# NVIDIA-RTX/RTXPT

Measured on AMD Instinct MI355X. Metric: Mrays/s at 4K 4spp 8-bounce bistro-like (extend + shadow rays / wall time of pt_render), higher is better.
Workload: dtype f32; 1 GPU; C3 bistro-like street canyon, 2808008 triangles, 64 materials, 32 textures 1024^2, 7368 emissive-triangle + env-quad lights, 3840x2160, 4 spp, 8 bounces, NEE 5 candidates + RR, lp types binary16 (reference default), environment cube 2048 BC6H (reference default on D3D12); BVH builder=PLOC + parallel re-insertion + cost-driven wide nodes, built on device, buildMs 77.8 (host part 0.0), 275780 wide n; parallelism=pixel-tile shard x1 + 1 gather, gather=none (1 GPU), transport=none, rehearsal=False

## Files before the change

### rtxpt_amd/csrc/pt_api.hip

```cpp
#include <cstring>
#include <rocprim/rocprim.hpp>
#include "pt_context.h"
#ifdef MI355PT_TEST_HOOKS
#include "../../include/mi355pt_testhooks.h"
#endif
#include "pt_denoiser.h"
#include <dlfcn.h>
#include <algorithm>
#include <cmath>
#include <cstdio>
#include <chrono>

using namespace ptk;

static_assert(sizeof(::PTMaterialData) == sizeof(ptk::PTMaterialData), "material ABI");
static_assert(sizeof(::PathTracerCameraData) == sizeof(ptk::PathTracerCameraData), "camera ABI");
static_assert(sizeof(::PtSettings) == sizeof(ptk::PtSettings), "settings ABI");
static_assert(sizeof(::PtGeometryDesc) == sizeof(ptk::GeometryDesc), "geometry ABI");
static_assert(sizeof(::PtInstanceDesc) == sizeof(ptk::InstanceDesc), "instance ABI");
static_assert(sizeof(::PolymorphicLightInfo) == sizeof(ptk::PolymorphicLightInfo), "light ABI");

namespace {

void build_mips(HostTexture& t) {
// ... 354 lines not shown
    return PT_OK;
}
int bake_env_cube(pt_context* c) {
    ptk::EnvCube& e = c->envCube; memset(&e, 0, sizeof(e)); e.dim = c->envCubeDim; e.mipLevels = ptk::env_cube_mip_levels(e.dim);
    size_t total = 0; for (uint l = 0; l < e.mipLevels; l++) { e.mipOffset[l] = (uint)total; total += 6ull * (e.dim >> l) * (e.dim >> l); }
    PT_CHECK_HIP(c, c->dEnvCube.resize(total));
    std::vector<ptk::EnvDirectionalLight> dirLights = c->envDirLights;
    if (!c->sceneDirLights.empty()) {
        PtEnvMapSceneParams prm; memset(&prm, 0, sizeof(prm)); memcpy(prm.Transform, c->envToWorld.m, 48); prm.Enabled = 1.f;
        std::vector<ptk::EnvDirectionalLight> conv(c->sceneDirLights.size());
        if (pt_env_bake_lights(reinterpret_cast<const PtEnvDirectionalLight*>(c->sceneDirLights.data()), (uint32_t)conv.size(), &prm, e.dim, reinterpret_cast<PtEnvDirectionalLight*>(conv.data())) != PT_OK) return fail(c, PT_ERROR_INVALID_ARGUMENT, "scene directional lights");
        for (auto& l : conv) if (dirLights.size() < 16u) dirLights.push_back(l);
    }
    PT_CHECK_HIP(c, c->dEnvDirLights.upload(dirLights, c->stream));
    if (c->skyEnabled) {
        ptk::ProceduralSkyContext h = c->sky; h.Transmittance.texels = c->dSkyTex[0].p; h.Scatter.texels = c->dSkyTex[1].p; h.Irradiance.texels = c->dSkyTex[2].p; h.Clouds.texels = c->dSkyTex[3].p;
        PT_CHECK_HIP(c, c->dSky.resize(1)); PT_CHECK_HIP(c, hipMemcpyAsync(c->dSky.p, &h, sizeof(h), hipMemcpyHostToDevice, c->stream)); PT_CHECK_HIP(c, hipStreamSynchronize(c->stream));
        PT_CHECK_HIP(c, c->dSkyLowRes.resize(6ull * (e.dim / 2u) * (e.dim / 2u)));
    }
    refresh_scene_view(c);
    launch_env_cube_bake(c->dsc, c->dEnvDirLights.p, (uint)dirLights.size(), c->dEnvCube.p, c->dsc.envCube, c->stream);
    if (c->envCompression) {
        PT_CHECK_HIP(c, c->dEnvCubeSource.resize(total));
        PT_CHECK_HIP(c, hipMemcpyAsync(c->dEnvCubeSource.p, c->dEnvCube.p, sizeof(ptk::uint2) * total, hipMemcpyDeviceToDevice, c->stream));
        launch_env_cube_compress(c->dEnvCube.p, c->dsc.envCube, c->envCompression, c->stream);
    } else c->dEnvCubeSource.free();
    refresh_scene_view(c);
    PT_CHECK_HIP(c, hipGetLastError());
    c->envCubeDirty = false; c->lightsDirty = true;
    return PT_OK;
}
}

int prepare(pt_context* c) {
    if (c->texDirty) { int r = upload_textures(c); if (r != PT_OK) return r; refresh_scene_view(c); c->lightsDirty = true; c->envCubeDirty = true; }
    if (c->envEnabled && c->envCubeDirty) { int r = bake_env_cube(c); if (r != PT_OK) return r; }
    if (c->geomDirty) { int r = finalize_geometry(c); if (r != PT_OK) return r; }
    if (c->lightsDirty) { int r = bake_lights(c); if (r != PT_OK) return r; }
    else if (c->weightsDirty && !c->lights.empty()) {
        launch_light_weights(c->dLights.p, c->dLightsEx.p, (uint)c->lights.size(), c->dLightW.p, c->lightBoost, c->stream);
        int r = build_light_proxies(c, c->dLightW.p, nullptr, 0u, 0.f); if (r != PT_OK) return r;
        refresh_scene_view(c);
    }
    c->weightsDirty = false;
    return PT_OK;
}

int neeat_exchange_feedback(pt_context* c) {
    pt_context::NeeAt& st = c->neeat;
    if (c->shardCount == 1 || !c->comm || !st.feedbackFilled || st.W != c->width || st.H != c->height) return PT_OK;
    hipStream_t s = c->stream;
    if (st.xW != c->width || st.xH != c->height) {
        std::vector<uint> others; for (uint r = 0; r < c->shardCount; r++) if (r != c->shardRank) others.insert(others.end(), c->shardPixels[r].begin(), c->shardPixels[r].end());
        PT_CHECK_HIP(c, st.xPixels.upload(others, s)); PT_CHECK_HIP(c, st.xRecv.resize(3 * others.size())); PT_CHECK_HIP(c, st.xSend.resize(3 * c->owned.size())); PT_CHECK_HIP(c, hipStreamSynchronize(s));
        st.xW = c->width; st.xH = c->height;
    }
    const size_t n = c->owned.size();
    launch_pack_feedback(st.fbW.p, st.fbC.p, st.depth.p, c->dOwned.p, (uint)n, c->width, st.xSend.p, s);
    PT_CHECK_NCCL(c, g_rccl.GroupStart());
    size_t off = 0; ncclResult_t bad = ncclSuccess;
    for (uint r = 0; r < c->shardCount && bad == ncclSuccess; r++) {
        if (r == c->shardRank) continue;
        const size_t m = c->shardPixels[r].size();
        if (n) bad = g_rccl.Send(st.xSend.p, 3 * n, ncclFloat, (int)r, c->comm, s);
        if (m && bad == ncclSuccess) bad = g_rccl.Recv(st.xRecv.p + 3 * off, 3 * m, ncclFloat, (int)r, c->comm, s);
        off += m;
    }
    ncclResult_t ge = g_rccl.GroupEnd();
    if (bad != ncclSuccess || ge != ncclSuccess) return fail(c, PT_ERROR_HIP, std::string("NEE-AT feedback exchange: ") + g_rccl.GetErrorString(bad != ncclSuccess ? bad : ge));
    launch_unpack_feedback(st.fbW.p, st.fbC.p, st.depth.p, st.xPixels.p, (uint)off, c->width, st.xRecv.p, s);
    return PT_OK;
}
int neeat_frame(pt_context* c, int phases, const float* depth, const ptk::uint2* motion) {
    pt_context::NeeAt& st = c->neeat;
    const uint N = (uint)c->lights.size();
    if (!N || !c->numProxies) {
        c->localResX = c->localResY = c->localJitterX = c->localJitterY = c->localMaxLight = 0; c->localRatio = 0.f; c->feedbackRequired = false; st.feedbackFilled = st.lastFeedbackAvailable = false; st.frameOpen = false;
        refresh_scene_view(c); return PT_OK;
    }
    NeeAtFrame F; memset(&F, 0, sizeof(F));
    F.W = c->width; F.H = c->height; F.BW = (F.W + 1) / 2; F.BH = (F.H + 1) / 2; F.tilesX = (F.W + 7) / 8 + 1; F.tilesY = (F.H + 7) / 8 + 1;
    const size_t px = (size_t)F.W * F.H, bpx = (size_t)F.BW * F.BH, tiles = (size_t)F.tilesX * F.tilesY;
    if (phases & NEEAT_BEGIN) {
        if (st.historicTotalLightCount && st.historicTotalLightCount != N) st.feedbackFilled = st.lastFeedbackAvailable = false;
        if (st.W != F.W || st.H != F.H) {
            st.W = F.W; st.H = F.H; st.feedbackFilled = false; st.lastFeedbackAvailable = false;
            PT_CHECK_HIP(c, st.fbW.resize(px)); PT_CHECK_HIP(c, st.fbC.resize(px)); PT_CHECK_HIP(c, st.scW.resize(px)); PT_CHECK_HIP(c, st.scC.resize(px)); PT_CHECK_HIP(c, st.snapW.resize(px)); PT_CHECK_HIP(c, st.snapC.resize(px));
            PT_CHECK_HIP(c, st.blW.resize(bpx)); PT_CHECK_HIP(c, st.blC.resize(bpx)); PT_CHECK_HIP(c, st.local.resize(tiles * RTXPT_LIGHTING_LOCAL_PROXY_COUNT));
            PT_CHECK_HIP(c, hipMemsetAsync(st.fbW.p, 0, 4 * px, c->stream)); PT_CHECK_HIP(c, hipMemsetAsync(st.fbC.p, 0xFF, 4 * px, c->stream));
            PT_CHECK_HIP(c, st.depth.resize(px)); PT_CHECK_HIP(c, st.histDepth.resize(px));
            PT_CHECK_HIP(c, hipMemsetAsync(st.depth.p, 0, 4 * px, c->stream)); PT_CHECK_HIP(c, hipMemsetAsync(st.histDepth.p, 0, 4 * px, c->stream));
        }
        st.prevJitter[0] = st.jitter[0]; st.prevJitter[1] = st.jitter[1];
        neeat_advance_jitter(st.updateCounter, st.jitterF, st.jitter);
        st.updateCounter++;
        st.frameLocalAvailable = st.lastFeedbackAvailable; st.frameFeedbackAvailable = st.feedbackFilled;
        st.framePrevLightCount = st.historicTotalLightCount; st.historicTotalLightCount = N;
        st.frameOpen = true;
    }
    if (!st.frameOpen || st.W != F.W || st.H != F.H) return fail(c, PT_ERROR_NOT_READY, "NEE-AT: UpdateEnd without UpdateBegin of this frame size");
    const bool lastFrameLocalSamplesAvailable = st.frameLocalAvailable, lastFrameFeedbackAvailable = st.frameFeedbackAvailable;
    F.jitterX = st.jitter[0]; F.jitterY = st.jitter[1]; F.jitterPrevX = st.prevJitter[0]; F.jitterPrevY = st.prevJitter[1];
    F.updateCounter = st.updateCounter; F.dropoff = st.dropoff; F.totalLightCount = N; F.historicTotalLightCount = st.framePrevLightCount;
    F.lastFrameFeedbackAvailable = lastFrameFeedbackAvailable ? 1u : 0u; F.lastFrameLocalSamplesAvailable = (lastFrameLocalSamplesAvailable && lastFrameFeedbackAvailable) ? 1u : 0u;
    F.fbW = st.fbW.p; F.fbC = st.fbC.p; F.scW = st.scW.p; F.scC = st.scC.p; F.blW = st.blW.p; F.blC = st.blC.p; F.local = st.local.p;
    F.depth = depth ? depth : st.depth.p; F.motion = motion; F.historyDepth = st.histDepth.p; F.depthDisocclusionThreshold = 1.5f;
    const uint totalMaxFeedbackCount = lastFrameFeedbackAvailable ? ((F.W + 7) / 8) * ((F.H + 7) / 8) * 64u : 0u;
    if (phases & NEEAT_BEGIN) {
        PT_CHECK_HIP(c, st.counters.resize(N + 1)); PT_CHECK_HIP(c, hipMemsetAsync(st.counters.p, 0, 4 * (size_t)(N + 1), c->stream)); F.perLightCounters = st.counters.p;
        if (lastFrameFeedbackAvailable) launch_neeat_begin(F, st.snapW.p, st.snapC.p, st.preFilter, totalMaxFeedbackCount, c->stream);
        PT_CHECK_HIP(c, st.curW.resize(N + 1)); PT_CHECK_HIP(c, st.histW.resize(N));
        launch_neeat_boost_weights(c->dLightW.p, (lastFrameFeedbackAvailable && st.intensityDeltaMul > 0) ? st.histW.p : nullptr, st.nHist, N, st.intensityDeltaMul, st.curW.p, c->stream);
        int r = build_light_proxies(c, st.curW.p, lastFrameFeedbackAvailable ? st.counters.p : nullptr, totalMaxFeedbackCount, lastFrameFeedbackAvailable ? st.globalFeedbackWeight : 0.f); if (r != PT_OK) return r;
        PT_CHECK_HIP(c, hipMemcpyAsync(st.histW.p, st.curW.p, 4 * (size_t)N, hipMemcpyDeviceToDevice, c->stream)); st.nHist = N;
        st.lastFeedbackAvailable = lastFrameFeedbackAvailable;
    }
    if (!(phases & NEEAT_END)) { PT_CHECK_HIP(c, hipStreamSynchronize(c->stream)); return PT_OK; }
    F.perLightCounters = st.counters.p;
    F.samplingProxyCount = c->numProxies; F.proxies = c->dProxyIndices.p;
    launch_neeat_end(F, c->stream);
    if (!depth) PT_CHECK_HIP(c, hipMemsetAsync(st.depth.p, 0, 4 * px, c->stream));
    st.exportDepth = depth == nullptr;
    st.feedbackFilled = true; st.frameOpen = false;
    c->localResX = F.tilesX; c->localResY = F.tilesY; c->localJitterX = st.jitter[0]; c->localJitterY = st.jitter[1]; c->localMaxLight = 0;
    c->localRatio = lastFrameFeedbackAvailable ? st.localRatio : 0.f; c->sscThreshold = st.sscThreshold; c->feedbackRequired = true;
    refresh_scene_view(c);
    PT_CHECK_HIP(c, hipStreamSynchronize(c->stream));
    return PT_OK;
}

extern "C" {

int32_t pt_create(const PtDeviceDesc* desc, pt_context** out) {
    if (!out) return PT_ERROR_INVALID_ARGUMENT;
    *out = nullptr;
    int ndev = 0;
    if (hipGetDeviceCount(&ndev) != hipSuccess || ndev <= 0) return PT_ERROR_NO_DEVICE;
    int dev = desc ? desc->deviceOrdinal : 0;
    if (dev < 0 || dev >= ndev) return PT_ERROR_INVALID_ARGUMENT;
    if (hipSetDevice(dev) != hipSuccess) return PT_ERROR_HIP;
    pt_context* c = new pt_context();
    c->device = dev; c->shardRank = desc ? desc->shardRank : 0; c->shardCount = (desc && desc->shardCount) ? desc->shardCount : 1;
    if (c->shardRank >= c->shardCount) { delete c; return PT_ERROR_INVALID_ARGUMENT; }
    if (hipStreamCreateWithFlags(&c->stream, hipStreamNonBlocking) != hipSuccess) { delete c; return PT_ERROR_HIP; }
    c->streams[0] = c->stream;
    for (uint b = 1; b < PT_PIPELINE_BATCHES; b++) if (hipStreamCreateWithFlags(&c->streams[b], hipStreamNonBlocking) != hipSuccess) { delete c; return PT_ERROR_HIP; }
    if (hipHostMalloc(&c->hostCounters, PT_PIPELINE_BATCHES * sizeof(WaveCounters), hipHostMallocDefault) != hipSuccess) { delete c; return PT_ERROR_HIP; }
    c->serialKernels = desc && (desc->flags & PT_DEVICE_SERIAL_KERNELS);
    c->bvhBuilder = (desc && (desc->flags & PT_DEVICE_PREFER_FAST_BUILD)) ? BVH_BUILDER_PLOC : ((desc && (desc->flags & PT_DEVICE_HOST_SAH_BUILDER)) ? BVH_BUILDER_SAH : BVH_BUILDER_PLOC_OPT);
    { const char* e = getenv("MI355PT_BVH_BUILDER");
      if (e && !strcmp(e, "karras")) c->bvhBuilder = BVH_BUILDER_KARRAS; else if (e && !strcmp(e, "ploc")) c->bvhBuilder = BVH_BUILDER_PLOC; else if (e && !strcmp(e, "sah")) c->bvhBuilder = BVH_BUILDER_SAH; else if (e && (!strcmp(e, "ploc_opt") || !strcmp(e, "device"))) c->bvhBuilder = BVH_BUILDER_PLOC_OPT; }
    { const char* e = getenv("MI355PT_TAIL_PATHS"); if (e) c->tailBelow = (uint)strtoul(e, nullptr, 10); }
    { const char* e = getenv("MI355PT_COMPACT_POOL"); if (e) c->compactPool = atoi(e) != 0; }
    { const char* e = getenv("MI355PT_FUSED_TRAVERSAL"); if (e) c->fusedTraversal = (uint)strtoul(e, nullptr, 10); }
    { const char* e = getenv("MI355PT_TAIL_DEFER"); if (e) c->tailDefer = (uint)strtoul(e, nullptr, 10); }
    memset(&c->dsc, 0, sizeof(c->dsc)); memset(&c->cam, 0, sizeof(c->cam)); memset(&c->bvh, 0, sizeof(c->bvh));
    pt_default_settings(reinterpret_cast<::PtSettings*>(&c->S));
    const float I[12] = {1, 0, 0, 0, 0, 1, 0, 0, 0, 0, 1, 0}; memcpy(c->envToWorld.m, I, 48); memcpy(c->envToLocal.m, I, 48); c->envColorMul = ptk::make_float3(1.0f / ptk::kEnvMapRadianceScale);
    if (c->dCounters.resize(PT_PIPELINE_BATCHES) != hipSuccess) { delete c; return PT_ERROR_HIP; }
    *out = c;
    return PT_OK;
}
int32_t pt_destroy(pt_context* c) {
    if (!c) return PT_ERROR_INVALID_ARGUMENT;
    (void)hipSetDevice(c->device); (void)hipStreamSynchronize(c->stream);
    if (c->comm && g_rccl.lib) { (void)g_rccl.CommDestroy(c->comm); c->comm = nullptr; }
    c->dSpHeader.free(); c->dSpThroughput.free(); c->dSpPlanes.free(); c->dSpRadiance.free(); c->dSpMotion.free(); c->dSpDepth.free(); c->dSpHitT.free(); c->dSpMark.free(); c->dSpNewL.free(); c->dSpScratch.free(); c->dSpGatherSend.free(); c->dSpGatherRecv.free(); c->dSpGatherPixels.free();
    c->dDnRRDiff.free(); c->dDnRRSpec.free(); c->dDnRRSpecMV.free(); c->dDnRRNormal.free(); c->dDnMotion.free(); c->dDnViewZ.free(); c->dDnRoughness.free(); c->dDnNormal.free(); c->dDnDiff.free(); c->dDnSpec.free(); c->dDnDisocclusion.free(); c->dDnHistoryClamp.free();
    relax_free(c); taa_free(c); bloom_free(c); taau_free(c);
    c->neeat.free(); c->dLocalTable.free(); c->dFbWeight.free(); c->dFbCand.free(); c->dSq3.free();
    c->dGatherSend.free(); c->dGatherRecv.free(); c->dGatherPixels.free(); c->dLightW.free(); c->dProxyOffsets.free(); if (c->dScanTemp) (void)hipFree(c->dScanTemp);
    if (c->bvhAllocated) bvh_free(c->bvh);
    c->dIndices.free(); c->dNormals.free(); c->dTangents.free(); c->dProxyCounters.free(); c->dProxyIndices.free(); c->dEnvLookup.free(); c->dOwned.free(); c->dQueue[0].free(); c->dQueue[1].free();
    c->dPrevPositions.free(); c->dPrevInstances.free(); c->dEmissiveList.free(); c->dEmissiveOffsets.free(); c->dPositions.free(); c->dUvs.free(); c->dGeometries.free(); c->dInstances.free(); c->dSubInstances.free(); c->dSubInstToInstGeom.free();
    c->dPrimInfo.free(); c->dShadeTris.free(); c->dAlphaPlanes.free(); c->dAlphaPool.free(); c->dMaterials.free(); c->dTexInfos.free(); c->dTexels.free(); c->dEnvCube.free(); c->dEnvCubeSource.free(); c->dEnvImageCube.free(); c->dEnvDirLights.free(); c->dLights.free(); c->dLightsEx.free(); c->dS0.free(); c->dS1.free(); c->dS2.free(); c->dS3.free(); c->dS4.free();
    c->dHit.free(); c->dS0b.free(); c->dS1b.free(); c->dS3b.free(); c->dS4b.free(); c->dHitb.free(); c->dSq0.free(); c->dSq1.free(); c->dSq2.free(); c->dAccum.free(); c->dScratch4.free(); c->dCounters.free(); c->dTravSpill.free(); c->dTaskQ.free(); c->dTravCounts.free(); c->dResolveList.free(); c->dBestKey.free(); c->dResolveListSh.free(); c->dBestKeySh.free(); c->dTaskQSh.free();
    for (uint b = 1; b < PT_PIPELINE_BATCHES; b++) (void)hipStreamDestroy(c->streams[b]);
    (void)hipStreamDestroy(c->stream); (void)hipHostFree(c->hostCounters);
    delete c;
    return PT_OK;
}
const char* pt_get_last_error(pt_context* c) { return c ? c->lastError.c_str() : "null context"; }

int32_t pt_set_geometry(pt_context* c, const PtGeometryBuffers* b, const PtGeometryDesc* geoms, uint32_t nGeoms, const PtMeshDesc* meshes, uint32_t nMeshes) {
    if (!c || !b || !geoms || !meshes) return fail(c, PT_ERROR_INVALID_ARGUMENT, "null argument");
    if (!b->indices || !b->positions) return fail(c, PT_ERROR_INVALID_ARGUMENT, "indices and positions are required");
    for (uint32_t g = 0; g < nGeoms; g++) {
        if ((size_t)geoms[g].indexOffset + geoms[g].numIndices > b->numIndices || (size_t)geoms[g].vertexOffset + geoms[g].numVertices > b->numVertices || geoms[g].numIndices % 3)
            return fail(c, PT_ERROR_INVALID_ARGUMENT, "geometry range outside the supplied streams");
        if ((geoms[g].flags & PT_GEOM_HAS_UV) && !b->uvs) return fail(c, PT_ERROR_INVALID_ARGUMENT, "geometry has uv flag but no uv stream");
        if ((geoms[g].flags & PT_GEOM_HAS_NORMAL) && !b->normals) return fail(c, PT_ERROR_INVALID_ARGUMENT, "geometry has normal flag but no normal stream");
        if ((geoms[g].flags & PT_GEOM_HAS_TANGENT) && !b->tangents) return fail(c, PT_ERROR_INVALID_ARGUMENT, "geometry has tangent flag but no tangent stream");
        const uint32_t* idx = b->indices + geoms[g].indexOffset;
        for (uint32_t k = 0; k < geoms[g].numIndices; k++) if (idx[k] >= geoms[g].numVertices) return fail(c, PT_ERROR_INVALID_ARGUMENT, "index outside the geometry's vertex range");
    }
    for (uint32_t m = 0; m < nMeshes; m++)
        if ((size_t)meshes[m].firstGeometry + meshes[m].numGeometries > nGeoms) return fail(c, PT_ERROR_INVALID_ARGUMENT, "mesh references geometries outside the supplied array");
    uint nv = b->numVertices;
    c->indices.assign(b->indices, b->indices + b->numIndices);
    c->positions.assign(b->positions, b->positions + 3 * (size_t)nv);
    c->uvs.assign(nv, ptk::make_float2(0, 0)); if (b->uvs) memcpy(c->uvs.data(), b->uvs, 8 * (size_t)nv);
    c->normals.assign(nv, 0); if (b->normals) memcpy(c->normals.data(), b->normals, 4 * (size_t)nv);
    c->tangents.assign(nv, 0); if (b->tangents) memcpy(c->tangents.data(), b->tangents, 4 * (size_t)nv);
    c->geometries.resize(nGeoms); memcpy(c->geometries.data(), geoms, sizeof(GeometryDesc) * nGeoms);
    c->meshes.resize(nMeshes); memcpy(c->meshes.data(), meshes, sizeof(MeshDesc) * nMeshes);
    c->geomDirty = true;
    relax_drop_history(c); taa_drop_history(c); taau_drop_history(c);
    return PT_OK;
}
int32_t pt_set_instances(pt_context* c, const PtInstanceDesc* inst, uint32_t n) {
    if (!c || (!inst && n)) return fail(c, PT_ERROR_INVALID_ARGUMENT, "null argument");
    c->instances.resize(n); if (n) memcpy(c->instances.data(), inst, sizeof(InstanceDesc) * n);
    c->geomDirty = true;
    return PT_OK;
}
int32_t pt_set_materials(pt_context* c, const ::PTMaterialData* mats, uint32_t nMats, const PtTextureDesc* tex, uint32_t nTex) {
    if (!c || (!mats && nMats) || (!tex && nTex)) return fail(c, PT_ERROR_INVALID_ARGUMENT, "null argument");
    c->materials.resize(nMats); if (nMats) memcpy(c->materials.data(), mats, 128 * (size_t)nMats);
    c->textures.clear();
    for (uint32_t i = 0; i < nTex; i++) {
        const PtTextureDesc& d = tex[i];
        if (!d.pixels || !d.width || !d.height || d.format > 2) return fail(c, PT_ERROR_INVALID_ARGUMENT, "bad texture descriptor");
        if (d.width > 32768u || d.height > 32768u) return fail(c, PT_ERROR_UNSUPPORTED, "textures above 32768 texels per side are not supported (16 mip levels)");
        HostTexture t; t.w = d.width; t.h = d.height; t.mips.resize(1); t.mips[0].resize((size_t)d.width * d.height);
        for (size_t k = 0; k < (size_t)d.width * d.height; k++) {
            ptk::float4 v;
            if (d.format == PT_TEX_RGBA32F) { const float* p = (const float*)d.pixels + 4 * k; v = ptk::make_float4(p[0], p[1], p[2], p[3]); }
            else {
                const uint8_t* p = (const uint8_t*)d.pixels + 4 * k;
                v = ptk::make_float4((float)p[0] / 255.0f, (float)p[1] / 255.0f, (float)p[2] / 255.0f, (float)p[3] / 255.0f);
                if (d.format == PT_TEX_RGBA8_SRGB) { v.x = srgb_to_linear(v.x); v.y = srgb_to_linear(v.y); v.z = srgb_to_linear(v.z); }
            }
            t.mips[0][k] = v;
        }
        build_mips(t);
        c->textures.push_back(std::move(t));
    }
    for (uint32_t m = 0; m < nMats; m++) {
        const ptk::PTMaterialData& mm = c->materials[m];
        auto chk = [&](uint flag, uint word) { return !(mm.Flags & flag) || (word & 0xFFFFu) < nTex; };
        if (!chk(PTMaterialFlags_UseBaseOrDiffuseTexture, mm.BaseOrDiffuseTextureIndex) || !chk(PTMaterialFlags_UseEmissiveTexture, mm.EmissiveTextureIndex) ||
            !chk(PTMaterialFlags_UseNormalTexture, mm.NormalTextureIndex) || !chk(PTMaterialFlags_UseMetalRoughOrSpecularTexture, mm.MetalRoughOrSpecularTextureIndex) ||
            !chk(PTMaterialFlags_UseTransmissionTexture, mm.TransmissionTextureIndex))
            return fail(c, PT_ERROR_INVALID_ARGUMENT, "material references a missing texture");
    }
    c->texDirty = true; c->geomDirty = true;
    return PT_OK;
}
static void set_env_params(pt_context* c, const PtEnvMapSceneParams* params) {
    if (params) {
        memcpy(c->envToWorld.m, params->Transform, 48);
        memset(&c->envToLocal, 0, sizeof(float3x4));
        for (int r = 0; r < 3; r++) for (int k = 0; k < 3; k++) c->envToLocal.m[r * 4 + k] = c->envToWorld.m[k * 4 + r];
        c->envColorMul = ptk::make_float3(params->ColorMultiplier[0], params->ColorMultiplier[1], params->ColorMultiplier[2]);
    } else {
        const float I[12] = {1, 0, 0, 0, 0, 1, 0, 0, 0, 0, 1, 0}; memcpy(c->envToWorld.m, I, 48); memcpy(c->envToLocal.m, I, 48);
        c->envColorMul = ptk::make_float3(1.0f / ptk::kEnvMapRadianceScale);
    }
}
static bool env_has_image(const pt_context* c) { return c->envTex.w != 0u || c->envImageCubeDim != 0u; }
int32_t pt_set_environment(pt_context* c, const float* rgb, uint32_t w, uint32_t h, const PtEnvMapSceneParams* params) {
    if (!c) return PT_ERROR_INVALID_ARGUMENT;
    c->envImageCubeDim = 0; c->dEnvImageCube.free();
    c->envEnabled = (w != 0 && h != 0 && rgb && (!params || params->Enabled != 0.f));
    if (!c->envEnabled) { c->envTex.w = c->envTex.h = 0; c->envTex.mips.clear(); if (c->skyEnabled && (!params || params->Enabled != 0.f)) c->envEnabled = true; }
    else {
        HostTexture& t = c->envTex; t.w = w; t.h = h; t.mips.clear(); t.mips.resize(1); t.mips[0].resize((size_t)w * h);
        for (size_t i = 0; i < (size_t)w * h; i++) t.mips[0][i] = ptk::make_float4(rgb[3 * i], rgb[3 * i + 1], rgb[3 * i + 2], 1.f);
        t.mipLevels = 1;
    }
    set_env_params(c, params);
    c->texDirty = true; c->lightsDirty = true; c->envCubeDirty = true;
    return PT_OK;
}
int32_t pt_set_environment_cube(pt_context* c, const float* rgbaFaces, uint32_t dim, const PtEnvMapSceneParams* params) {
    if (!c) return PT_ERROR_INVALID_ARGUMENT;
    if (dim > 16384u) return fail(c, PT_ERROR_INVALID_ARGUMENT, "cube-map source: at most 16384 texels per side");
    c->envTex.w = c->envTex.h = 0; c->envTex.mips.clear();
    c->envEnabled = (dim != 0 && rgbaFaces && (!params || params->Enabled != 0.f));
    if (!c->envEnabled) { c->envImageCubeDim = 0; c->dEnvImageCube.free(); if (c->skyEnabled && (!params || params->Enabled != 0.f)) c->envEnabled = true; }
    else {
        const size_t n = 6ull * dim * dim; std::vector<ptk::uint2> h(n);
        for (size_t i = 0; i < n; i++) h[i] = ptk::env_pack_rgba16f(ptk::make_float4(rgbaFaces[4 * i], rgbaFaces[4 * i + 1], rgbaFaces[4 * i + 2], rgbaFaces[4 * i + 3]));
        PT_CHECK_HIP(c, c->dEnvImageCube.resize(n)); PT_CHECK_HIP(c, hipMemcpy(c->dEnvImageCube.p, h.data(), n * sizeof(ptk::uint2), hipMemcpyHostToDevice));
        c->envImageCubeDim = dim;
    }
    set_env_params(c, params);
    c->texDirty = true; c->lightsDirty = true; c->envCubeDirty = true;
    return PT_OK;
}
int32_t pt_set_procedural_sky(pt_context* c, const PtProceduralSkyConstants* consts, const PtProceduralSkyTextures* tex) {
    if (!c) return PT_ERROR_INVALID_ARGUMENT;
    static_assert(sizeof(PtProceduralSkyConstants) == sizeof(ptk::ProceduralSkyConstants), "ProceduralSkyConstants layout");
    if (!consts) {
        if (c->skyEnabled) { c->skyEnabled = false; if (!env_has_image(c)) c->envEnabled = false; c->envCubeDirty = true; c->lightsDirty = true; c->texDirty = true; }
        return PT_OK;
    }
    if (tex) {
        const PtSkyTexture* t[4] = {&tex->transmittance, &tex->scattering, &tex->irradiance, &tex->clouds}; ptk::SkyTexture* dst[4] = {&c->sky.Transmittance, &c->sky.Scatter, &c->sky.Irradiance, &c->sky.Clouds};
        for (int i = 0; i < 4; i++) {
            if (!t[i]->rgba || !t[i]->width || !t[i]->height || !t[i]->depth || t[i]->width > 4096u || t[i]->height > 4096u || t[i]->depth > 4096u) return fail(c, PT_ERROR_INVALID_ARGUMENT, "procedural sky: every look-up texture needs RGBA float texels and sizes in [1, 4096]");
            if ((i == 0 || i == 2) && t[i]->depth != 1u) return fail(c, PT_ERROR_INVALID_ARGUMENT, "procedural sky: the transmittance and irradiance textures are 2-D (depth 1)");
        }
        for (int i = 0; i < 4; i++) {
            const size_t n = (size_t)t[i]->width * t[i]->height * t[i]->depth;
            PT_CHECK_HIP(c, c->dSkyTex[i].resize(n)); PT_CHECK_HIP(c, hipMemcpy(c->dSkyTex[i].p, t[i]->rgba, n * sizeof(ptk::float4), hipMemcpyHostToDevice));
// ... 913 lines not shown
```

### rtxpt_amd/csrc/pt_context.h

```cpp
#pragma once
#include "../../include/mi355pt.h"
#include "pt_wavefront.h"
#include "pt_stableplanes_launch.h"
#include "pt_denoiser.h"
#include "pt_build.h"
#include <rccl/rccl.h>
#include <string>
#include <vector>

#pragma GCC visibility push(hidden)

using namespace ptk;

template <typename T> struct DevBuf {
    T* p = nullptr; size_t n = 0;
    hipError_t resize(size_t count) {
        if (count <= n && p) return hipSuccess;
        if (p) (void)hipFree(p);
        p = nullptr; n = 0;
        hipError_t e = hipMalloc(&p, sizeof(T) * (count ? count : 1));
        if (e == hipSuccess) n = count ? count : 1;
        return e;
    }
    hipError_t upload(const T* src, size_t count, hipStream_t st) {
        hipError_t e = resize(count); if (e != hipSuccess) return e;
        if (!count) return hipSuccess;
        return hipMemcpyAsync(p, src, sizeof(T) * count, hipMemcpyHostToDevice, st);
    }
    hipError_t upload(const std::vector<T>& v, hipStream_t st) { return upload(v.data(), v.size(), st); }
    void free() { if (p) (void)hipFree(p); p = nullptr; n = 0; }
};

struct HostTexture { uint w, h, mipLevels; std::vector<std::vector<ptk::float4>> mips; };

static const uint TILE = 32;
static const uint TASK_QUEUE_CAPACITY = 1u << 22;
#ifndef PT_SHARD_TILE_GROUP
#define PT_SHARD_TILE_GROUP 1
#endif
#ifndef PT_PIPELINE_FULL_AT
#define PT_PIPELINE_FULL_AT (1u << 21)
#endif
#ifndef PT_PIPELINE_MID_BATCHES
#define PT_PIPELINE_MID_BATCHES 2
#endif
#ifndef PT_CLASSIFY_FROM
#define PT_CLASSIFY_FROM 65536u
#endif
#ifndef PT_SP_FILL_CLASSES
#define PT_SP_FILL_CLASSES 1
#endif
#ifndef PT_SP_FILL_RANGED
#define PT_SP_FILL_RANGED 1
#endif
#ifndef PT_TAIL_PATHS
#define PT_TAIL_PATHS 4096u
#endif
#ifndef PT_FUSED_TRAVERSAL
#define PT_FUSED_TRAVERSAL 1u
#endif
#ifndef PT_FUSED_BELOW
#define PT_FUSED_BELOW (12u << 20)
#endif
#ifndef PT_COMPACT_POOL
#define PT_COMPACT_POOL 1
#endif
#ifndef PT_FREE_RUN_BELOW
#define PT_FREE_RUN_BELOW (1u << 22)
#endif
#ifndef PT_PIPELINE_BATCHES
#define PT_PIPELINE_BATCHES 4
#endif

#pragma GCC visibility pop
struct pt_context {
    int device = 0; hipStream_t stream = nullptr; uint shardRank = 0, shardCount = 1;
    hipStream_t streams[PT_PIPELINE_BATCHES] = {}; WaveCounters* hostCounters = nullptr; bool serialKernels = false;
    uint tailBelow = PT_TAIL_PATHS, tailDefer = 0, fusedTraversal = PT_FUSED_TRAVERSAL; bool compactPool = PT_COMPACT_POOL != 0;
    std::string lastError;
    std::vector<uint> indices; std::vector<float> positions; std::vector<ptk::float2> uvs; std::vector<uint> normals, tangents;
    std::vector<GeometryDesc> geometries; std::vector<MeshDesc> meshes; std::vector<InstanceDesc> instances;
    std::vector<ptk::PTMaterialData> materials; std::vector<HostTexture> textures; HostTexture envTex; bool envEnabled = false;
    float3x4 envToWorld, envToLocal; ptk::float3 envColorMul;
    uint envCubeDim = 2048; std::vector<ptk::EnvDirectionalLight> envDirLights, sceneDirLights; bool envCubeDirty = true;
    ptk::EnvCube envCube;
    std::vector<PolymorphicLightInfoFull> analyticLights;
    std::vector<SubInstanceData> subInstances; std::vector<ptk::uint2> subInstToInstGeom; std::vector<ptk::uint2> primInfo;
    std::vector<uint> subInstFirstPrim;
    std::vector<ptk::PolymorphicLightInfo> lights; std::vector<ptk::PolymorphicLightInfoEx> lightsEx; std::vector<uint> envLookup;
    uint envLookupDim = 0; uint numProxies = 0, envLightsBaked = 0;
    DevBuf<float> dLightW; DevBuf<uint> dProxyOffsets; void* dScanTemp = nullptr; size_t scanTempBytes = 0;
    DevBuf<uint> dIndices, dNormals, dTangents, dProxyCounters, dProxyIndices, dEnvLookup, dOwned, dQueue[2], dEmissiveList, dEmissiveOffsets;
    DevBuf<float> dPrevPositions; DevBuf<InstanceDesc> dPrevInstances; bool motionHistory = false, prevAllStale = false;
    std::vector<uint32_t> prevStaleRanges;
    DevBuf<float> dPositions; DevBuf<ptk::float2> dUvs; DevBuf<GeometryDesc> dGeometries; DevBuf<InstanceDesc> dInstances;
    DevBuf<SubInstanceData> dSubInstances;
    DevBuf<ptk::AlphaPlane> dAlphaPlanes; DevBuf<unsigned char> dAlphaPool; DevBuf<ptk::ShadeTri> dShadeTris;
    DevBuf<ptk::uint2> dSubInstToInstGeom, dPrimInfo; DevBuf<ptk::PTMaterialData> dMaterials; DevBuf<TexInfo> dTexInfos; DevBuf<ptk::float4> dTexels;
    bool skyEnabled = false; ptk::ProceduralSkyContext sky; DevBuf<ptk::float4> dSkyTex[4]; DevBuf<ptk::ProceduralSkyContext> dSky;
    DevBuf<ptk::uint2> dSkyLowRes;
    DevBuf<ptk::uint2> dEnvImageCube; uint envImageCubeDim = 0;
    DevBuf<ptk::uint2> dEnvCube, dEnvCubeSource; DevBuf<ptk::EnvDirectionalLight> dEnvDirLights; uint envCompression = 0;
    DevBuf<ptk::PolymorphicLightInfo> dLights; DevBuf<ptk::PolymorphicLightInfoEx> dLightsEx;
    DevBuf<uint> dLocalTable; uint localResX = 0, localResY = 0, localJitterX = 0, localJitterY = 0, localMaxLight = 0;
    float localRatio = 0.f, sscThreshold = 0.f; bool feedbackRequired = false;
    DevBuf<float> dFbWeight; DevBuf<uint> dFbCand; DevBuf<ptk::float4> dSq3; uint fbSamples = 0;
    ptk::LightFrustumBoost lightBoost = {}; bool weightsDirty = false;
    struct NeeAt {
        bool enabled = false; float globalFeedbackWeight = 0.75f, localRatio = 0.65f, sscThreshold = 0.3f, dropoff = 0.005f, intensityDeltaMul = 64.0f;
        bool preFilter = true;
        uint updateCounter = 0; float jitterF[2] = {0, 0}; uint jitter[2] = {0, 0}, prevJitter[2] = {0, 0};
        bool feedbackFilled = false, lastFeedbackAvailable = false; uint historicTotalLightCount = 0, W = 0, H = 0, nHist = 0;
        bool frameOpen = false, frameFeedbackAvailable = false, frameLocalAvailable = false, exportDepth = true; uint framePrevLightCount = 0;
        DevBuf<float> fbW, scW, blW, snapW, curW, histW; DevBuf<uint> fbC, scC, blC, snapC, local, counters;
        DevBuf<float> depth, histDepth; bool haveClip = false; float clipZ[4] = {0, 0, 0, 0}, clipW[4] = {0, 0, 0, 0};
        DevBuf<uint> xSend, xRecv; DevBuf<uint> xPixels; uint xW = 0, xH = 0;
        void reset() {
            W = H = 0; updateCounter = 0; jitterF[0] = jitterF[1] = 0; jitter[0] = jitter[1] = prevJitter[0] = prevJitter[1] = 0;
            feedbackFilled = lastFeedbackAvailable = false; frameOpen = false; exportDepth = true; historicTotalLightCount = 0; nHist = 0;
        }
        void free() {
            fbW.free(); scW.free(); blW.free(); snapW.free(); curW.free(); histW.free(); fbC.free(); scC.free(); blC.free(); snapC.free();
            local.free(); counters.free(); xSend.free(); xRecv.free(); xPixels.free(); depth.free(); histDepth.free();
        }
    } neeat;
    DevBuf<ptk::uint4> dS0, dS1, dS2, dS3, dS4, dHit, dS0b, dS1b, dS3b, dS4b, dHitb; DevBuf<ptk::float4> dSq0, dSq1, dSq2, dAccum, dScratch4;
    DevBuf<WaveCounters> dCounters; DevBuf<ptk::uint2> dTravSpill; DevBuf<ptk::TravTask> dTaskQ; DevBuf<uint> dTravCounts, dResolveList;
    DevBuf<unsigned long long> dBestKey;
    DevBuf<ptk::TravTask> dTaskQSh; DevBuf<uint> dResolveListSh; DevBuf<unsigned long long> dBestKeySh;
    std::vector<TexInfo> texInfos; TexInfo envTexInfo;
    BvhBuildBuffers bvh; bool bvhAllocated = false; uint numTris = 0; uint bvhBuilder = BVH_BUILDER_SAH;
    DeviceScene dsc;
    ptk::PtSettings S; ptk::PathTracerCameraData cam; uint width = 0, height = 0, accumCount = 0; std::vector<uint> owned;
    std::vector<std::vector<uint>> shardPixels;
    std::vector<float> hostRadiance; bool countersEnabled = false;
    bool geomDirty = true, lightsDirty = true, texDirty = true;
    double buildMs = 0, refitMs = 0, lightBakeMs = 0;
    uint poolCapacity = 0; size_t shadowCapacity = 0;
    DevBuf<uint> dSpHeader, dSpThroughput; DevBuf<ptk::StablePlane> dSpPlanes; DevBuf<ptk::uint2> dSpRadiance, dSpMotion;
    DevBuf<float> dSpDepth, dSpHitT; uint spW = 0, spH = 0; bool spGathered = false;
    DevBuf<ptk::uint4> dSpMark; DevBuf<ptk::float4> dSpNewL;
    DevBuf<float> dSpScratch; DevBuf<uint> dSpGatherSend, dSpGatherRecv, dSpGatherPixels; uint spGatherW = 0, spGatherH = 0;
    DevBuf<uint> dDnRRDiff, dDnRRSpec, dDnRRSpecMV; DevBuf<ptk::uint2> dDnRRNormal, dDnMotion; DevBuf<float> dDnViewZ, dDnRoughness;
    DevBuf<ptk::float4> dDnNormal, dDnDiff, dDnSpec;
    DevBuf<unsigned char> dDnDisocclusion, dDnHistoryClamp; uint dnW = 0, dnH = 0;
    uint spSampleBase = 0;
    DevBuf<ptk::float4> dRxHist[3][2][5], dRxOut[3][2], dRxGuide, dRxPing[2], dRxPong[2];
    uint rxW = 0, rxH = 0, rxSide[3] = {0, 0, 0}; bool rxHistory[3] = {false, false, false}, rxDenoised[3] = {false, false, false}; int dnPreparedPlane = -1;
    uint spFrameSerial = 0, rxFrameSerial[3] = {0, 0, 0};
    bool rxTiming = false; std::vector<float> rxPassMs; std::vector<hipEvent_t> rxEvents;
    DevBuf<ptk::float4> dTaa[2]; uint taaW = 0, taaH = 0, taaSide = 0, taaFrameSerial = 0, dnNrdSerial = 0; bool taaHistory = false, taaResolved = false;
    hipEvent_t taaEvents[2] = {nullptr, nullptr};
    DevBuf<ptk::float4> dBloom, dBloomQ[2]; uint bloomW = 0, bloomH = 0; bool bloomReady = false;
    hipEvent_t bloomEvents[2] = {nullptr, nullptr};
    DevBuf<ptk::float4> dTaau[2], dTaauBloom, dTaauBloomQ[2]; uint taauW = 0, taauH = 0, taauRenderW = 0, taauRenderH = 0, taauSide = 0, taauFrameSerial = 0;
    bool taauHistory = false, taauResolved = false, taauBloomReady = false;
    hipEvent_t taauEvents[2] = {nullptr, nullptr}, taauBloomEvents[2] = {nullptr, nullptr};
    ncclComm_t comm = nullptr; uint commRank = 0, commWorld = 0; DevBuf<ptk::float4> dGatherSend, dGatherRecv; DevBuf<uint> dGatherPixels;
    std::vector<size_t> gatherCounts; uint gatherW = 0, gatherH = 0;
};

#pragma GCC visibility push(hidden)

inline int fail(pt_context* c, int code, const std::string& msg) { if (c) c->lastError = msg; return code; }
#define PT_CHECK_HIP(c, expr) \
    do { hipError_t e_ = (expr); if (e_ != hipSuccess) return fail(c, PT_ERROR_HIP, std::string(#expr) + ": " + hipGetErrorString(e_)); } while (0)

int prepare(pt_context* c);
int neeat_exchange_feedback(pt_context* c);
enum { NEEAT_BEGIN = 1, NEEAT_END = 2, NEEAT_BOTH = 3 };
int neeat_frame(pt_context* c, int phases = NEEAT_BOTH, const float* depth = nullptr, const ptk::uint2* motion = nullptr);
inline int32_t dn_ready(pt_context* c) {
    if (!c->spW || c->spW != c->width || c->spH != c->height) return fail(c, PT_ERROR_NOT_READY, "no stable planes of this frame size yet: pt_build_stable_planes, pt_fill_stable_planes");
    if (c->shardCount > 1 && !c->spGathered) return fail(c, PT_ERROR_NOT_READY, "the denoiser passes read the whole frame's planes: pt_gather_stable_planes / pt_unpack_stable_planes first");
    return PT_OK;
}
inline ptk::DenoiserBuffers dn_buffers(pt_context* c) {
    ptk::DenoiserBuffers D;
    D.RRDiffuseAlbedo = c->dDnRRDiff.p; D.RRSpecAlbedo = c->dDnRRSpec.p; D.RRNormalsAndRoughness = c->dDnRRNormal.p; D.RRSpecMotionVectors = c->dDnRRSpecMV.p;
    D.ViewZ = c->dDnViewZ.p; D.MotionVectors = c->dDnMotion.p; D.NormalRoughness = c->dDnNormal.p; D.DiffRadianceHitDist = c->dDnDiff.p; D.SpecRadianceHitDist = c->dDnSpec.p;
    D.Roughness = c->dDnRoughness.p; D.DisocclusionThresholdMix = c->dDnDisocclusion.p; D.CombinedHistoryClampRelax = c->dDnHistoryClamp.p;
    return D;
}
void relax_drop_history(pt_context* c);
void relax_free(pt_context* c);
void taa_drop_history(pt_context* c);
void taa_free(pt_context* c);
int32_t taa_resolved_ready(pt_context* c);
void bloom_drop(pt_context* c);
void bloom_free(pt_context* c);
void taau_drop_history(pt_context* c);
void taau_free(pt_context* c);
StablePlanesContext sp_context(pt_context* c, const PtStablePlanesParams* params);
void add_frame_stats(PtFrameStats& t, const PtFrameStats& o);

#pragma GCC visibility pop
```

### rtxpt_amd/csrc/pt_frame.hip

```cpp
#include "pt_context.h"
#include <cstdio>
#include <cstdlib>
#include <cstring>

StablePlanesContext sp_context(pt_context* c, const PtStablePlanesParams* params) {
    ptk::StablePlanesParams prm;
    if (params) memcpy(&prm, params, sizeof(prm));
    else { memset(&prm, 0, sizeof(prm)); prm.activeStablePlaneCount = cStablePlaneCount; }
    StablePlanesContext sp; sp.C = ptk::SP_make_consts(prm, c->width, c->height, c->S.bounceCount);
    sp.B.Header = c->dSpHeader.p; sp.B.Planes = c->dSpPlanes.p; sp.B.StableRadiance = c->dSpRadiance.p; sp.B.Depth = c->dSpDepth.p;
    sp.B.SpecularHitT = c->dSpHitT.p; sp.B.MotionVectors = c->dSpMotion.p; sp.B.Throughput = c->dSpThroughput.p;
    return sp;
}

void add_frame_stats(PtFrameStats& t, const PtFrameStats& o) {
    t.extendRays += o.extendRays; t.shadowRays += o.shadowRays; t.hits += o.hits;
    t.nodeVisitsExtend += o.nodeVisitsExtend; t.triTestsExtend += o.triTestsExtend; t.nodeVisitsShadow += o.nodeVisitsShadow;
    t.triTestsShadow += o.triTestsShadow; t.leafVisitsExtend += o.leafVisitsExtend; t.waveItersExtend += o.waveItersExtend;
    t.leafVisitsShadow += o.leafVisitsShadow; t.waveItersShadow += o.waveItersShadow;
    for (int q = 0; q < 4; q++) t.extendPhaseCycles[q] += o.extendPhaseCycles[q];
    t.leafBlocksExtend += o.leafBlocksExtend; if (o.waveItersMaxExtend > t.waveItersMaxExtend) t.waveItersMaxExtend = o.waveItersMaxExtend;
    for (int q = 0; q < 16; q++) t.extendRayIterHist[q] += o.extendRayIterHist[q];
    for (uint q = 0; q < o.longRayCount && q < 32u && t.longRayCount < 32u; q++) { memcpy(t.longRays[t.longRayCount], o.longRays[q], 32); t.longRayCount++; }
    for (int q = 0; q < 8; q++) t.extendEvents[q] += o.extendEvents[q];
    t.gpuMilliseconds += o.gpuMilliseconds; t.extendKernelMs += o.extendKernelMs; t.shadeKernelMs += o.shadeKernelMs; t.shadowKernelMs += o.shadowKernelMs;
    t.extendLaunches += o.extendLaunches; if (o.iterations > t.iterations) t.iterations = o.iterations;
    t.pathsTraced += o.pathsTraced; t.tailLaunches += o.tailLaunches;
}

namespace {


int ensure_pool(pt_context* c, uint n, uint shadowPerPath) {
    if (n <= c->poolCapacity && (size_t)n * shadowPerPath <= c->shadowCapacity) return PT_OK;
    if (n < c->poolCapacity) n = c->poolCapacity;
    const size_t ns = (size_t)n * shadowPerPath;
    if (ns > 0xF0000000ull) return fail(c, PT_ERROR_INVALID_ARGUMENT, "too many shadow-queue entries in one pt_render call (paths x NEEFullSamples)");
    PT_CHECK_HIP(c, c->dS0.resize(n)); PT_CHECK_HIP(c, c->dS1.resize(n)); PT_CHECK_HIP(c, c->dS2.resize(n)); PT_CHECK_HIP(c, c->dS3.resize(n));
    PT_CHECK_HIP(c, c->dS4.resize(n)); PT_CHECK_HIP(c, c->dHit.resize(n)); PT_CHECK_HIP(c, c->dQueue[0].resize(n)); PT_CHECK_HIP(c, c->dQueue[1].resize(n));
    PT_CHECK_HIP(c, c->dSq0.resize(ns)); PT_CHECK_HIP(c, c->dSq1.resize(ns)); PT_CHECK_HIP(c, c->dSq2.resize(ns));
    PT_CHECK_HIP(c, c->dBestKey.resize(ns)); PT_CHECK_HIP(c, c->dResolveList.resize(ns));
    PT_CHECK_HIP(c, c->dTaskQ.resize((size_t)PT_PIPELINE_BATCHES * 2 * TASK_QUEUE_CAPACITY));
    PT_CHECK_HIP(c, c->dTravCounts.resize(PT_PIPELINE_BATCHES * PASS_COUNTERS));
    c->poolCapacity = n; c->shadowCapacity = ns;
    return PT_OK;
}

struct Events {
    std::vector<hipEvent_t> ev;
    Events() = default; Events(const Events&) = delete; Events& operator=(const Events&) = delete;
    ~Events() { for (hipEvent_t e : ev) if (e) (void)hipEventDestroy(e); }
    hipError_t record(hipStream_t st) {
        hipEvent_t e = nullptr; const hipError_t r = hipEventCreate(&e); ev.push_back(e);
        return r != hipSuccess ? r : hipEventRecord(e, st);
    }
    size_t mark(hipStream_t st) { (void)record(st); return ev.size() - 1; }
    float ms(size_t a = 0, size_t b = 1) const { float m = 0; (void)hipEventElapsedTime(&m, ev[a], ev[b]); return m; }
};

struct Batch {
    uint pixFirst = 0, numPix = 0, total = 0, base = 0;
    hipStream_t st = nullptr; WaveCounters* wc = nullptr; WaveCounters* hwc = nullptr;
    PathPool pool; ShadowQueue sq; uint* queue[2] = {nullptr, nullptr}; DeviceScene sc; PathKernelContext k; TravAux aux;
    uint cur = 0, active = 0, iterations = 0; unsigned long long extendRays = 0, shadowRays = 0; bool waiting = false;
};
uint batch_count(const pt_context* c, uint paths) {
    if (c->serialKernels || paths < (1u << 20)) return 1u;
    return paths < PT_PIPELINE_FULL_AT ? (uint)PT_PIPELINE_MID_BATCHES : (uint)PT_PIPELINE_BATCHES;
}
void slice_batch(pt_context* c, const PathKernelContext& k, uint b, uint numBatches, uint pathsPerPixel, uint shadowPerPath,
                 const ShadowQueue& frameSq, uint maxBlocks, Batch& t) {
    const unsigned long long numOwned = c->owned.size();
    t.pixFirst = (uint)(numOwned * b / numBatches); t.numPix = (uint)(numOwned * (b + 1) / numBatches) - t.pixFirst;
    t.total = t.numPix * pathsPerPixel; t.base = t.pixFirst * pathsPerPixel;
    t.st = c->streams[b]; t.wc = c->dCounters.p + b; t.hwc = c->hostCounters + b;
    t.pool = PathPool{c->dS0.p + t.base, c->dS1.p + t.base, c->dS2.p + t.base, c->dS3.p + t.base, c->dS4.p + t.base, c->dHit.p + t.base};
    const size_t sbase = (size_t)t.base * shadowPerPath;
    t.sq = frameSq; t.sq.q0 += sbase; t.sq.q1 += sbase; t.sq.q2 += sbase; if (t.sq.q3) t.sq.q3 += sbase;
    t.queue[0] = c->dQueue[0].p + t.base; t.queue[1] = c->dQueue[1].p + t.base;
    t.sc = c->dsc; t.sc.travSpill = c->dsc.travSpill + (size_t)b * T8_MAX_BLOCKS * T8_GROUPS_PER_BLOCK * T8_SPILL_DEPTH;
    t.k = k; t.k.sc = t.sc;
    t.aux.taskQ[0] = c->dTaskQ.p + (size_t)(2 * b) * TASK_QUEUE_CAPACITY; t.aux.taskQ[1] = t.aux.taskQ[0] + TASK_QUEUE_CAPACITY;
    t.aux.counts = c->dTravCounts.p + PASS_COUNTERS * b; t.aux.taskCap = TASK_QUEUE_CAPACITY; t.aux.maxBlocks = maxBlocks;
    t.aux.bestKey = c->dBestKey.p + sbase; t.aux.resolveList = c->dResolveList.p + sbase; t.aux.primToSlot = c->bvh.primToSlot;
    memset(t.hwc, 0, sizeof(WaveCounters));
}
PathKernelContext kernel_context(const pt_context* c) { PathKernelContext k; k.sc = c->dsc; k.S = c->S; k.cam = c->cam; return k; }
ShadowQueue frame_shadow_queue(const pt_context* c, uint group) {
    return ShadowQueue{c->dSq0.p, c->dSq1.p, c->dSq2.p, group, nullptr, nullptr, nullptr, 0u, 0u, 0u};
}
TravAux shadow_aux(const Batch& t) { TravAux a = t.aux; a.counts = t.aux.counts + PASS_SHADOW_OFFSET; return a; }

uint nested_dielectric_allowance(const ptk::PtSettings& S) { return S.nestedDielectricsQuality == 2 ? 16u : (S.nestedDielectricsQuality == 1 ? 4u : 0u); }

bool composed_frame(const pt_context* c, uint shadowGroup) { return !c->serialKernels && !c->countersEnabled && !shadowGroup && c->dsc.rootIsValid; }

PtFrameStats batch_stats(const Batch& t, uint shadowGroup) {
    const WaveCounters& h = *t.hwc;
    PtFrameStats s; memset(&s, 0, sizeof(s));
    s.extendRays = t.extendRays + h.tailExtendRays; s.shadowRays = shadowGroup ? h.shadowValid : t.shadowRays + h.tailShadowRays; s.hits = h.hits;
    s.nodeVisitsExtend = h.nodeVisitsExt; s.triTestsExtend = h.triTestsExt; s.nodeVisitsShadow = h.nodeVisitsSh; s.triTestsShadow = h.triTestsSh;
    s.leafVisitsExtend = h.leafVisitsExt; s.waveItersExtend = h.itersExt; s.leafVisitsShadow = h.leafVisitsSh; s.waveItersShadow = h.itersSh;
    for (int q = 0; q < 4; q++) s.extendPhaseCycles[q] = h.phaseCycExt[q];
    s.leafBlocksExtend = h.leafBlocksExt; s.waveItersMaxExtend = h.itersMaxExt;
    for (int q = 0; q < 8; q++) s.extendEvents[q] = h.eventsExt[q];
    for (int q = 0; q < 16; q++) s.extendRayIterHist[q] = h.rayIterHistExt[q];
    s.longRayCount = h.longRayCount < 32u ? h.longRayCount : 32u; memcpy(s.longRays, h.longRays, 32 * (size_t)s.longRayCount);
    s.extendLaunches = s.iterations = t.iterations; s.pathsTraced = t.total;
    return s;
}

template <typename B> int32_t check_frame_end(pt_context* c, const B* batches, uint numBatches, const char* stillAlive) {
    for (uint b = 0; b < numBatches; b++)
        if (batches[b].hwc->overflow)
            return fail(c, PT_ERROR_HIP, "BVH8 traversal: stack tail or straggler task queue overflow (raise T8_SPILL_DEPTH / TASK_QUEUE_CAPACITY)");
    for (uint b = 0; b < numBatches; b++) if (batches[b].active) return fail(c, PT_ERROR_HIP, stillAlive);
    return PT_OK;
}
template <typename B> int32_t drain_frame(pt_context* c, B* batches, uint numBatches, Events& frame) {
    for (uint b = 0; b < numBatches; b++)
        PT_CHECK_HIP(c, hipMemcpyAsync(batches[b].hwc, batches[b].wc, sizeof(WaveCounters), hipMemcpyDeviceToHost, batches[b].st));
    for (uint b = 0; b < numBatches; b++) PT_CHECK_HIP(c, hipStreamSynchronize(batches[b].st));
    PT_CHECK_HIP(c, frame.record(c->stream));
    PT_CHECK_HIP(c, hipStreamSynchronize(c->stream));
    PT_CHECK_HIP(c, hipGetLastError());
    return PT_OK;
}


struct RenderBatch : Batch {
    uint bound = 0;
    uint tailLaunches = 0; bool afterTail = false, inTail = false;
    uint pendingShadow = 0; TravAux auxSh;
    PathPool poolSet[2]; uint set = 0; bool compact = false;
    bool timed = false; Events marks; size_t t0 = 0, t1 = 0;
    struct Span { size_t a, b; int kind; uint items; }; std::vector<Span> spans;
    size_t mark() { return timed ? marks.mark(st) : 0; }
    void span(size_t a, size_t b, int kind, uint items) { if (timed) spans.push_back({a, b, kind, items}); }
};

struct RenderFrame {
    pt_context* c; uint first, count, total, shadowGroup, shadowPerPath; bool feedback;
    uint numBatches = 0; RenderBatch B[PT_PIPELINE_BATCHES];
    uint maxIter = 0, tailBelow = 0, wavefrontPasses = 0; bool fused = false, passLog = false;

    bool live(const RenderBatch& t) const { return t.active && t.bound < maxIter; }
    int32_t setup(const PathKernelContext& k) {
        numBatches = batch_count(c, total);
        static const uint batchesOverride = []() { const char* e = getenv("MI355PT_BATCHES"); return e ? (uint)strtoul(e, nullptr, 10) : 0u; }();
        static const uint blocksOverride = []() { const char* e = getenv("MI355PT_MAX_BLOCKS"); return e ? (uint)strtoul(e, nullptr, 10) : 0u; }();
        if (batchesOverride && !c->serialKernels) numBatches = batchesOverride < (uint)PT_PIPELINE_BATCHES ? batchesOverride : (uint)PT_PIPELINE_BATCHES;
        uint maxBlocks = (numBatches >= 3u) ? (total < (6u << 20) ? 256u * 7u / 2u : (total < (24u << 20) ? 256u * 35u / 8u : 256u * 7u)) : 0u;
        if (blocksOverride) maxBlocks = blocksOverride < 2u ? 2u : (blocksOverride < T8_MAX_BLOCKS ? blocksOverride : (uint)T8_MAX_BLOCKS);
        ShadowQueue sq = frame_shadow_queue(c, shadowGroup);
        if (feedback) {
            sq.q3 = c->dSq3.p; sq.fbTotalWeight = c->neeat.enabled ? c->neeat.fbW.p : c->dFbWeight.p;
            sq.fbCandidates = c->neeat.enabled ? c->neeat.fbC.p : c->dFbCand.p;
            sq.fbWidth = c->width; sq.fbPlane = c->width * c->height; sq.fbSampleFirst = first;
        }
        passLog = getenv("MI355PT_PASS_LOG") != nullptr;
        for (uint b = 0; b < numBatches; b++) {
            RenderBatch& t = B[b];
            slice_batch(c, k, b, numBatches, count, shadowPerPath, sq, maxBlocks, t);
            t.timed = c->serialKernels || c->countersEnabled || passLog;
            t.hwc->extendCount[0] = t.active = t.total;
        }
        maxIter = c->S.bounceCount + 2 + nested_dielectric_allowance(c->S);
        const bool composed = composed_frame(c, shadowGroup);
        tailBelow = composed ? c->tailBelow : 0u;
        const bool fuse = composed && (c->fusedTraversal == 1u || (c->fusedTraversal == 2u && total < PT_FUSED_BELOW));
        if (fuse) { int32_t r = enable_fused(); if (r != PT_OK) return r; }
        const bool neeatShade = c->dsc.lights.LocalSamplingBuffer != nullptr || c->dsc.lights.TemporalFeedbackRequired != 0u;
        if (composed && c->compactPool && !neeatShade && !feedback) return enable_compact_pool();
        return PT_OK;
    }
    int32_t enable_fused() {
        PT_CHECK_HIP(c, c->dBestKeySh.resize(c->shadowCapacity)); PT_CHECK_HIP(c, c->dResolveListSh.resize(c->shadowCapacity));
        PT_CHECK_HIP(c, c->dTaskQSh.resize((size_t)PT_PIPELINE_BATCHES * 2 * TASK_QUEUE_CAPACITY));
        for (uint b = 0; b < numBatches; b++) {
            RenderBatch& t = B[b]; const size_t sbase = (size_t)t.base * shadowPerPath;
            t.auxSh = shadow_aux(t);
            t.auxSh.taskQ[0] = c->dTaskQSh.p + (size_t)(2 * b) * TASK_QUEUE_CAPACITY; t.auxSh.taskQ[1] = t.auxSh.taskQ[0] + TASK_QUEUE_CAPACITY;
            t.auxSh.bestKey = c->dBestKeySh.p + sbase; t.auxSh.resolveList = c->dResolveListSh.p + sbase;
        }
        fused = true;
        return PT_OK;
    }
    int32_t enable_compact_pool() {
        PT_CHECK_HIP(c, c->dS0b.resize(c->poolCapacity)); PT_CHECK_HIP(c, c->dS1b.resize(c->poolCapacity)); PT_CHECK_HIP(c, c->dS3b.resize(c->poolCapacity));
        PT_CHECK_HIP(c, c->dS4b.resize(c->poolCapacity)); PT_CHECK_HIP(c, c->dHitb.resize(c->poolCapacity));
        for (uint b = 0; b < numBatches; b++) {
            RenderBatch& t = B[b]; t.compact = true; t.set = 0; t.poolSet[0] = t.pool;
            t.poolSet[1] = PathPool{c->dS0b.p + t.base, c->dS1b.p + t.base, t.pool.s2, c->dS3b.p + t.base, c->dS4b.p + t.base, c->dHitb.p + t.base, nullptr};
        }
        return PT_OK;
    }
    int32_t start() {
        for (uint b = 0; b < numBatches; b++) {
            RenderBatch& t = B[b];
            t.t0 = t.mark();
            PT_CHECK_HIP(c, hipMemcpyAsync(t.wc, t.hwc, sizeof(WaveCounters), hipMemcpyHostToDevice, t.st));
            launch_generate(t.k, t.pool, c->dOwned.p + t.pixFirst, t.numPix, first, count, 0u, t.total, t.queue[0], nullptr, t.st);
        }
        return PT_OK;
    }
    int32_t queue_pass(RenderBatch& t) {
        const uint nxt = t.cur ^ 1u;
        launch_pass_reset(t.aux.counts, &t.wc->extendCount[nxt], fused ? nullptr : &t.wc->shadowCount, t.st);
        if (tailBelow && t.active <= tailBelow && !t.afterTail) return queue_tail(t);
        t.afterTail = false; t.bound++; wavefrontPasses++;
        const size_t e0 = t.mark();
        PathPool pin = t.pool, pout = PathPool{};
        if (t.compact) { pin = t.poolSet[t.set]; pin.home = t.queue[t.cur]; pout = t.poolSet[t.set ^ 1u]; t.set ^= 1u; }
        const uint* countIn = &t.wc->extendCount[t.cur];
        if (t.pendingShadow) {
            launch_trace_pair(t.sc, pin, t.queue[t.cur], countIn, t.active, t.sq, &t.wc->shadowCount, t.pendingShadow, t.wc, t.aux, t.auxSh, t.st);
            t.pendingShadow = 0;
        } else launch_extend(t.sc, pin, t.queue[t.cur], countIn, t.active, t.wc, c->countersEnabled, t.aux, t.st);
        const size_t e1 = t.mark(); t.span(e0, e1, 0, t.active);
        uint* classScratch = t.active >= PT_CLASSIFY_FROM ? reinterpret_cast<uint*>(t.aux.bestKey) : nullptr;
        launch_shade(t.k, pin, t.queue[t.cur], countIn, t.active, t.queue[nxt], &t.wc->extendCount[nxt], t.sq, t.wc, classScratch,
                     t.aux.counts + PASS_CLASS_OFFSET, t.st, pout);
        const size_t e2 = t.mark(); t.span(e1, e2, 1, t.active);
        t.extendRays += t.active;
        PT_CHECK_HIP(c, hipMemcpyAsync(t.hwc, t.wc, 16, hipMemcpyDeviceToHost, t.st));
        t.waiting = true;
        return PT_OK;
    }
    int32_t queue_tail(RenderBatch& t) {
        const uint nxt = t.cur ^ 1u;
        if (t.compact) {
            PathPool in = t.poolSet[t.set]; in.home = t.queue[t.cur];
            launch_uncompact(in, t.poolSet[t.set ^ 1u], &t.wc->extendCount[t.cur], t.active, t.st);
            t.pool = t.poolSet[t.set ^ 1u]; t.compact = false;
        }
        if (t.pendingShadow) {
            launch_shadow(t.sc, t.pool, t.sq, &t.wc->shadowCount, t.pendingShadow, t.wc, false, t.auxSh, t.st);
            PT_CHECK_HIP(c, hipMemsetAsync(&t.wc->shadowCount, 0, 4, t.st));
            t.pendingShadow = 0;
        }
        const size_t e0 = t.mark();
        launch_tail(t.k, t.pool, t.queue[t.cur], &t.wc->extendCount[t.cur], t.active, t.queue[nxt], &t.wc->extendCount[nxt], t.sq, t.wc, maxIter - t.bound,
                    c->tailDefer, t.aux.maxBlocks, t.st);
        const size_t e1 = t.mark(); t.span(e0, e1, 3, t.active);
        t.tailLaunches++; t.afterTail = true; t.inTail = true;
        PT_CHECK_HIP(c, hipMemcpyAsync(t.hwc, t.wc, 16, hipMemcpyDeviceToHost, t.st));
        t.waiting = true;
        return PT_OK;
    }
    int32_t finish_pass(RenderBatch& t, uint b) {
        t.waiting = false; t.inTail = false;
        const uint nxt = t.cur ^ 1u, nShadow = t.hwc->shadowCount;
        if (passLog) {
            uint pc[PASS_COUNTERS]; PT_CHECK_HIP(c, hipMemcpy(pc, t.aux.counts, sizeof(pc), hipMemcpyDeviceToHost));
            fprintf(stderr, "[pass log]   b%u pass %u: %u paths -> extend splits %u / %u / %u / %u sub-trees, %u rays resolved; %u visibility rays next\n",
                    b, t.iterations, t.active, pc[0], pc[1], pc[2], pc[3], pc[TRAV_RESOLVE], nShadow);
        }
        t.active = t.hwc->extendCount[nxt];
        if (fused && nShadow && live(t)) { t.pendingShadow = nShadow; t.shadowRays += nShadow; }
        else if (nShadow) {
            const size_t s0 = t.mark();
            launch_shadow(t.sc, t.pool, t.sq, &t.wc->shadowCount, nShadow, t.wc, c->countersEnabled, fused ? t.auxSh : shadow_aux(t), t.st);
            const size_t s1 = t.mark(); t.span(s0, s1, 2, nShadow);
            if (!shadowGroup) t.shadowRays += nShadow;
            if (fused) PT_CHECK_HIP(c, hipMemsetAsync(&t.wc->shadowCount, 0, 4, t.st));
        }
        t.cur = nxt; t.iterations++;
        return PT_OK;
    }
    int32_t lockstep() {
        static const uint freeRunBelow = []() {
            const char* e = getenv("MI355PT_FREE_RUN_BELOW"); return e ? (uint)strtoul(e, nullptr, 10) : (uint)PT_FREE_RUN_BELOW;
        }();
        for (;;) {
            bool freeRun = freeRunBelow != 0u && numBatches > 1u;
            for (uint b = 0; b < numBatches; b++) if (live(B[b]) && B[b].active >= freeRunBelow) freeRun = false;
            wavefrontPasses = 0;
            for (uint b = 0; b < numBatches; b++) {
                RenderBatch& t = B[b];
                if (t.waiting || !live(t)) continue;
                int32_t r = queue_pass(t); if (r != PT_OK) return r;
            }
            if (freeRun) return PT_OK;
            bool any = false;
            for (uint b = 0; b < numBatches; b++) {
                RenderBatch& t = B[b];
                if (!t.waiting) continue;
                if (t.inTail && wavefrontPasses && hipStreamQuery(t.st) == hipErrorNotReady) { any = true; continue; }
                PT_CHECK_HIP(c, hipStreamSynchronize(t.st));
                int32_t r = finish_pass(t, b); if (r != PT_OK) return r;
                if (live(t)) any = true;
            }
            if (!any) return PT_OK;
        }
    }
    int32_t free_run() {
        uint waiting = 0; for (uint b = 0; b < numBatches; b++) waiting += B[b].waiting ? 1u : 0u;
        while (waiting) {
            for (uint b = 0; b < numBatches; b++) {
                RenderBatch& t = B[b];
                if (!t.waiting || hipStreamQuery(t.st) == hipErrorNotReady) continue;
                PT_CHECK_HIP(c, hipStreamSynchronize(t.st));
                int32_t r = finish_pass(t, b); if (r != PT_OK) return r;
                waiting--;
                if (live(t)) { r = queue_pass(t); if (r != PT_OK) return r; waiting++; }
            }
        }
        return PT_OK;
    }
    void accumulate() {
        for (uint b = 0; b < numBatches; b++) {
            RenderBatch& t = B[b];
            launch_accumulate(t.pool, c->dOwned.p + t.pixFirst, t.numPix, count, c->dAccum.p, c->accumCount, c->width, t.st);
            t.t1 = t.mark();
        }
    }
    void harvest(PtFrameStats& stats, float frameMs) const {
        for (uint b = 0; b < numBatches; b++) {
            const RenderBatch& t = B[b];
            PtFrameStats s = batch_stats(t, shadowGroup);
            s.tailLaunches = t.tailLaunches;
            for (const RenderBatch::Span& sp : t.spans) {
                const float m = t.marks.ms(sp.a, sp.b);
                if (sp.kind == 0) s.extendKernelMs += m; else if (sp.kind == 1) s.shadeKernelMs += m; else if (sp.kind == 2) s.shadowKernelMs += m;
            }
            add_frame_stats(stats, s);
        }
        stats.gpuMilliseconds = frameMs;
    }
    void log_passes() const {
        static const char* const kinds[4] = {"extend", "shade", "shadow", "tail"};
        for (uint b = 0; b < numBatches; b++) {
            const RenderBatch& t = B[b]; const WaveCounters& h = *t.hwc;
            if (t.tailLaunches)
                fprintf(stderr, "[pass log] batch %u: %u tail launches traced %llu + %llu rays, handed back %llu extend stragglers, "
                        "%llu visibility stragglers, %llu paths at the bounce bound\n", b, t.tailLaunches, (unsigned long long)h.tailExtendRays,
                        (unsigned long long)h.tailShadowRays, (unsigned long long)h.tailHandedBack[0], (unsigned long long)h.tailHandedBack[1],
                        (unsigned long long)h.tailHandedBack[2]);
            if (!t.timed) continue;
            fprintf(stderr, "[pass log] batch %u of %u: %u paths, %u passes, %.3f ms from first to last event\n", b, numBatches, t.total, t.iterations,
                    t.marks.ms(t.t0, t.t1));
            for (const RenderBatch::Span& sp : t.spans)
                fprintf(stderr, "[pass log]   b%u %-6s %9u items  start %8.3f ms  %7.3f ms\n", b, kinds[sp.kind], sp.items, t.marks.ms(t.t0, sp.a),
                        t.marks.ms(sp.a, sp.b));
        }
    }
};

int32_t render_sample_by_sample(pt_context* c, uint32_t first, uint32_t count, PtFrameStats* stats) {
    PtFrameStats total; memset(&total, 0, sizeof(total));
    int32_t r = PT_OK;
    for (uint32_t s = 0; s < count && r == PT_OK; s++) {
        PtFrameStats one; r = pt_render(c, first + s, 1, &one);
        if (r == PT_OK) add_frame_stats(total, one);
    }
    if (stats) *stats = total;
    return r;
}
int32_t prepare_neeat_layers(pt_context* c, uint32_t count, bool feedback, uint shadowGroup) {
    if (c->localResX) {
        const uint TILE_PX = ptk::RTXPT_LIGHTING_SAMPLING_BUFFER_TILE_SIZE;
        if ((c->width - 1u + c->localJitterX) / TILE_PX >= c->localResX || (c->height - 1u + c->localJitterY) / TILE_PX >= c->localResY)
            return fail(c, PT_ERROR_INVALID_ARGUMENT, "local sampling table smaller than the frame");
        if (c->localMaxLight >= c->lights.size())
            return fail(c, PT_ERROR_INVALID_ARGUMENT, "local sampling table names a light index beyond the baked light table");
    }
    c->fbSamples = 0;
    if (!feedback) return PT_OK;
    if (shadowGroup)
        return fail(c, PT_ERROR_INVALID_ARGUMENT, "NEE-AT temporal feedback needs NEEFullSamples 1 (the reference's default): the feedback draw of one light "
                                                  "sample shifts the random numbers of the next");
    const size_t plane = (size_t)c->width * c->height;
    PT_CHECK_HIP(c, c->dSq3.resize(c->shadowCapacity));
    if (!c->neeat.enabled) {
        PT_CHECK_HIP(c, c->dFbWeight.resize(plane * count)); PT_CHECK_HIP(c, c->dFbCand.resize(plane * count));
// ... 226 lines not shown
```

### rtxpt_amd/csrc/pt_path.h

```cpp
#pragma once
#include "pt_bsdf.h"
#include "pt_rng.h"
#include "pt_scene.h"

#ifndef PT_SHADE_TRI
#define PT_SHADE_TRI 1
#endif
#ifndef PT_SHADE_NOINLINE
#define PT_SHADE_NOINLINE
#endif

namespace ptk {
#pragma clang force_cuda_host_device begin

static const float kMaxRayTravel = 1e15f;
static const float kSpecularRoughnessThreshold = 0.25f;

struct PathTracerCameraData {
    float3 PosW; float NearZ; float3 DirectionW; float PixelConeSpreadAngle; float3 CameraU; float FarZ;
    float3 CameraV; float FocalDistance; float3 CameraW; float AspectRatio; uint2 ViewportSize; float ApertureRadius; float _padding0;
    float2 Jitter; float _padding1, _padding2;
};
static_assert(sizeof(PathTracerCameraData) == 112, "PathTracerCameraData layout");
struct PtSettings {
// ... 14 lines not shown
        float distTerm = fabsf(getWidth());
        float normalTerm = fabsf(dot(rayDir, normal));
        if (moreDetailOnSlopes) normalTerm = sqrtf_(normalTerm);
        lambda += SafeLog2(distTerm / normalTerm);
        return lambda;
    }
};
struct InteriorList {
    static const uint kNoMaterial = 0xffffffffu, kMaterialMask = (1u << 28) - 1u, kNestedPriorityOffset = 28, kMaxNestedPriority = 15;
    uint slots[2];
    bool isEmpty() const { return slots[0] == 0; }
    uint getTopNestedPriority() const { return slots[0] >> kNestedPriorityOffset; }
    uint getTopMaterialID() const { return slots[0] != 0 ? (slots[0] & kMaterialMask) : kNoMaterial; }
    uint getNextMaterialID() const { return slots[1] != 0 ? (slots[1] & kMaterialMask) : kNoMaterial; }
    bool isTrueIntersection(uint nestedPriority) const { return nestedPriority == 0 || nestedPriority >= getTopNestedPriority(); }
    void handleIntersection(uint materialID, uint nestedPriority, bool entering) {
        if (nestedPriority == 0) nestedPriority = kMaxNestedPriority;
        uint slot = (nestedPriority << kNestedPriorityOffset) | (materialID & kMaterialMask);
        if (entering && slots[0] == 0) slots[0] = slot;
        else if (!entering && slots[0] != 0 && (slots[0] & kMaterialMask) == materialID) slots[0] = 0;
        else if (entering && slots[1] == 0) slots[1] = slot;
        else if (!entering && slots[1] != 0 && (slots[1] & kMaterialMask) == materialID) slots[1] = 0;
        if (slots[0] < slots[1]) { uint t = slots[0]; slots[0] = slots[1]; slots[1] = t; }
    }
};
enum : uint {
    PF_active = 1 << 0, PF_hit = 1 << 1, PF_transmission = 1 << 2, PF_specular = 1 << 3, PF_delta = 1 << 4,
    PF_insideDielectricVolume = 1 << 5, PF_terminateAtNextBounce = 1 << 6, PF_enableThreadReorder = 1 << 9, PF_deltaOnlyPath = 1 << 12,
};
enum { PC_DiffuseBounces = 0, PC_RejectedHits = 1 };
static const uint kVertexIndexBitCount = 10, kVertexIndexBitMask = (1u << 10) - 1u;

struct PathState {
    float3 origin; uint id; float3 dir; float sceneLength;
    uint pack23[2]; uint pack45[2];
    InteriorList interiorList; uint packedCounters; RayCone rayCone;
    uint pack0, pack1, flagsAndVertexIndex, sampleIndex;

    void SetFireflyFilterK_BsdfScatterPdf(float k, float pdf) { pack0 = (f32tof16(clampf(k, 0, HLF_MAX)) << 16) | f32tof16(clampf(pdf, 0, HLF_MAX)); }
    float GetFireflyFilterK() const { return f16tof32(pack0 >> 16); }
    float GetBsdfScatterPdf() const { return f16tof32(pack0 & 0xFFFFu); }
    void SetPackedMISInfo_ThpRuRuCorrection(uint mis, float c) { pack1 = (mis << 16) | f32tof16(clampf(c, 0, HLF_MAX)); }
    uint GetPackedMISInfo() const { return pack1 >> 16; }
    float GetThpRuRuCorrection() const { return f16tof32(pack1 & 0xFFFFu); }
    void SetThp(float3 thp) { thp = clamp3(thp, 0.f, HLF_MAX); pack23[0] = Fp32ToFp16NoClamp(make_float2(thp.x, thp.y)); pack23[1] = Fp32ToFp16NoClamp(make_float2(thp.z, 0.f)); }
    float3 GetThp() const { float2 a = Fp16ToFp32(pack23[0]), b = Fp16ToFp32(pack23[1]); return make_float3(a.x, a.y, b.x); }
    void SetL(float4 l) { pack45[0] = Fp32ToFp16NoClamp(make_float2(clampf(l.x, 0, HLF_MAX), clampf(l.y, 0, HLF_MAX))); pack45[1] = Fp32ToFp16NoClamp(make_float2(clampf(l.z, 0, HLF_MAX), clampf(l.w, 0, HLF_MAX))); }
    float4 GetL() const { float2 a = Fp16ToFp32(pack45[0]), b = Fp16ToFp32(pack45[1]); return make_float4(a.x, a.y, b.x, b.y); }
    bool hasFlag(uint f) const { return (flagsAndVertexIndex & (f << kVertexIndexBitCount)) != 0; }
    void setFlag(uint f, bool v = true) { uint bit = f << kVertexIndexBitCount; if (v) flagsAndVertexIndex |= bit; else flagsAndVertexIndex &= ~bit; }
    bool isActive() const { return hasFlag(PF_active); }
    void terminate() { setFlag(PF_active, false); }
    bool isTerminatingAtNextBounce() const { return hasFlag(PF_terminateAtNextBounce); }
    void clearScatterEventFlags() { flagsAndVertexIndex &= ~((PF_transmission | PF_specular | PF_delta) << kVertexIndexBitCount); }
    uint getCounter(uint type) const { return (packedCounters >> (type << 3)) & 0xff; }
    void incrementCounter(uint type) { packedCounters += (1u << (type << 3)); }
    uint getVertexIndex() const { return flagsAndVertexIndex & kVertexIndexBitMask; }
    void incrementVertexIndex() { flagsAndVertexIndex += 1; }
    void decrementVertexIndex() { flagsAndVertexIndex -= 1; }
};
struct NEEBSDFMISInfo {
    bool LightSamplingEnabled, LightSamplingIsSSC; uint CandidateSamples, FullSamples;
    static NEEBSDFMISInfo empty() { NEEBSDFMISInfo r; r.LightSamplingEnabled = false; r.LightSamplingIsSSC = false; r.CandidateSamples = 0; r.FullSamples = 0; return r; }
    static NEEBSDFMISInfo Unpack16bit(uint p) { NEEBSDFMISInfo r; r.LightSamplingEnabled = (p & (1u << 15)) != 0; r.LightSamplingIsSSC = (p & (1u << 13)) != 0; r.CandidateSamples = (p >> 6) & 0x3F; r.FullSamples = p & 0x3F; return r; }
    uint Pack16bit() const { return ((LightSamplingEnabled ? 1u : 0u) << 15) | ((LightSamplingIsSSC ? 1u : 0u) << 13) | ((CandidateSamples & 0x3F) << 6) | (FullSamples & 0x3F); }
};
struct LightSample {
    float3 Li; float Distance; float3 Direction; uint LightIndex; float SelectionPdf, SolidAnglePdf; bool LightSampleableByBSDF, FromLocalDistribution;
    bool Valid() const { return any_gt0(Li); }
};
struct SurfaceData { ShadingData shadingData; StandardBSDF bsdf; float interiorIoR; uint neeTriangleLightIndex; uint neeAnalyticLightIndex; };
struct ShadowRequest { bool valid; float3 origin, dir; float tmax; float3 radiance; uint fbLight; float fbWeight, fbRandom; uint rrFix; };
struct ShadowSink { float4* q0; float4* q1; float4* q2; uint* count; unsigned long long* valid; uint pathIndex; };

static inline float ComputeRayConeSpreadAngleExpansionByScatterPDF(float bsdfScatterPdf, float growthFactor) {
    return growthFactor * 2.0f * FastACos(fmaxf_(-1.0f, 1.0f - (1.0f / bsdfScatterPdf) / (2.0f * K_PI)));
}
template <class LP> static inline float ComputeNewScatterFireflyFilterK(float currentK, float bouncePDF, float lobeP) {
    const float minK = 0.00001f;
    float angle = (bouncePDF == 0) ? 0.f : ComputeRayConeSpreadAngleExpansionByScatterPDF(bouncePDF, 1.0f);
    const float k = 32;
    float p = k / (k + angle * angle);
    p *= FastSqrt(lobeP);
    return LP::r(fmaxf_(minK, currentK * p));
}
template <class LP> static inline float3 FireflyFilter(float3 signalIn, float threshold, float fireflyFilterK) {
    float t = LP::mul(threshold, fireflyFilterK);
    float maxR = LP::average3(signalIn);
    if (maxR > t) signalIn = LP::mul3(LP::div3(signalIn, maxR), t);
    return signalIn;
}
static inline float FireflyFilterShort(float signalAverage, float threshold, float fireflyFilterK) {
    float t = threshold * fireflyFilterK;
    return (signalAverage > t) ? (1.0f / signalAverage * t) : 1.0f;
}
static inline float ComputeLowGrazingAngleFalloff(float3 lightDirection, float3 n, float falloffFrom, float falloffRange) {
    return saturate((dot(lightDirection, n) - falloffFrom) / falloffRange);
}
static inline float GetPerceivedBrightness(float3 c) { return sqrtf_((0.299f * c.x * c.x + 0.587f * c.y * c.y) + 0.114f * c.z * c.z); }
static inline void ConvertSpecularGlossToMetalRough(float3 diffuseColor, float3 specularColor, float3& baseColor, float& metalness) {
    const float epsilon = 1e-6f, dielectricSpecular = 0.04f;
    float diffuseBrightness = GetPerceivedBrightness(diffuseColor), specularBrightness = GetPerceivedBrightness(specularColor);
    float oneMinusSpecularStrength = 1.0f - fmaxf_(specularColor.x, fmaxf_(specularColor.y, specularColor.z));
    metalness = 0.0f;
    if (!(specularBrightness < dielectricSpecular)) {
        float b = (diffuseBrightness * oneMinusSpecularStrength / (1.0f - dielectricSpecular) + specularBrightness) - 2.0f * dielectricSpecular;
        float c = dielectricSpecular - specularBrightness;
        float D = fmaxf_(b * b - 4.0f * dielectricSpecular * c, 0.0f);
        metalness = saturate((-b + sqrtf_(D)) / (2.0f * dielectricSpecular));
    }
    float3 baseColorFromDiffuse = diffuseColor * (oneMinusSpecularStrength / (1.0f - dielectricSpecular) / fmaxf_(1.0f - metalness, epsilon));
    float3 baseColorFromSpecular = (specularColor - make_float3(dielectricSpecular * (1.0f - metalness))) * (1.0f / fmaxf_(metalness, epsilon));
    baseColor = saturate3(lerp3(baseColorFromDiffuse, baseColorFromSpecular, metalness * metalness));
}
static inline float computeRayConeTriangleLODValue(const float3 v[3], const float2 t[3], const float3x4& M) {
    float2 tx10 = t[1] - t[0], tx20 = t[2] - t[0];
    float Ta = fabsf(tx10.x * tx20.y - tx20.x * tx10.y);
    float3 edge01 = xform_vector(M, v[1] - v[0]);
    float3 edge02 = xform_vector(M, v[2] - v[0]);
    float Pa = length(cross(edge01, edge02));
    return 0.5f * RayCone::SafeLog2(Ta / Pa);
}

static inline float TriangleCurvatureApprox_GradN(const float3 vertexPositions[3], const float3 vertexNormals[3], const float3x4& transform) {
    const float eps = 1e-8f;
    float3 e10 = xform_vector(transform, vertexPositions[1] - vertexPositions[0]);
    float e10Len = length(e10);
    if (e10Len < eps) return 0.0f;
    float3 e1 = e10 / e10Len;
    float3 e20 = xform_vector(transform, vertexPositions[2] - vertexPositions[0]);
    float u2 = dot(e20, e1);
    float3 t = e20 - e1 * u2;
    float tLen = length(t);
    if (tLen < eps) return 0.0f;
    float3 e2 = t / tLen;
    float u1 = e10Len;
    float v2 = dot(e20, e2);
    float3 dn1 = vertexNormals[1] - vertexNormals[0], dn2 = vertexNormals[2] - vertexNormals[0];
    float3 a = dn1 / fmaxf_(u1, eps);
    float denomV = fabsf(v2) < eps ? (v2 >= 0.0f ? eps : -eps) : v2;
    float3 b = (dn2 - a * u2) / denomV;
    return sqrtf_(dot(a, a) + dot(b, b));
}
struct MVBlockInputs { float curvatureWS, projectionTerm; };

template <bool LP16> struct PathKernelContextT {
    typedef LPOps<LP16> LP;
    DeviceScene sc; PtSettings S; PathTracerCameraData cam;

    bool HasFinishedSurfaceBounces(uint vertexIndex, uint diffuseBounces) const {
        if (S.bounceCount < vertexIndex) return true;
        return diffuseBounces > S.diffuseBounceCount;
    }
    void computeCameraRay(uint px, uint py, uint sampleIndex, float3& o, float3& d) const {
        SampleGeneratorVertexBase vb = SampleGeneratorVertexBase::make((px << 16) | py, 0, sampleIndex);
        SampleSequenceGenerator sg = SampleSequenceGenerator::make(vb);
        float2 r0 = sampleNext2D(sg);
        float2 subPixelOffset = make_float2(cam.Jitter.x + (r0.x - 0.5f) * S.perPixelJitterAAScale, cam.Jitter.y + (r0.y - 0.5f) * S.perPixelJitterAAScale);
        float2 dof = sampleNext2D(sg);
        float2 pp = make_float2(((float)px + 0.5f + -subPixelOffset.x) / (float)cam.ViewportSize.x, ((float)py + 0.5f + subPixelOffset.y) / (float)cam.ViewportSize.y);
        float2 ndc = make_float2(2.f * pp.x + -1.f, -2.f * pp.y + 1.f);
        float3 org = cam.PosW;
        float3 dir = (ndc.x * cam.CameraU + ndc.y * cam.CameraV) + cam.CameraW;
        float2 ap = sample_disk(dof);
        float3 rayTarget = org + dir;
        org = org + cam.ApertureRadius * (ap.x * normalize(cam.CameraU) + ap.y * normalize(cam.CameraV));
        dir = normalize(rayTarget - org);
        float invCos = 1.f / dot(normalize(cam.CameraW), dir);
        float tMin = cam.NearZ * invCos;
        o = org + dir * tMin; d = dir;
    }
    void ExportDepth(const PathState& path, float3 virtualWorldPos) const {
        sc.lights.DepthExport[(path.id & 0xFFFFu) * sc.lights.DepthWidth + (path.id >> 16)] = LightTable_ClipDepth(sc.lights, virtualWorldPos);
    }
    PathState generate(uint px, uint py, uint sampleIndex) const {
        PathState p; __builtin_memset(&p, 0, sizeof(p));
        p.id = (px << 16) | py; p.sampleIndex = sampleIndex;
        p.SetThp(make_float3(1.f));
        p.setFlag(PF_active); p.setFlag(PF_deltaOnlyPath, true);
        p.rayCone = RayCone::make(0, cam.PixelConeSpreadAngle);
        p.SetL(make_float4(0, 0, 0, 0));
        p.SetFireflyFilterK_BsdfScatterPdf(1.0f, 0.0f);
        p.SetPackedMISInfo_ThpRuRuCorrection(NEEBSDFMISInfo::empty().Pack16bit(), 1.0f);
        if (HasFinishedSurfaceBounces(p.getVertexIndex() + 1, p.getCounter(PC_DiffuseBounces))) p.setFlag(PF_terminateAtNextBounce);
        SampleGeneratorVertexBase vb = SampleGeneratorVertexBase::make((px << 16) | py, 0, sampleIndex);
        SampleSequenceGenerator sg = SampleSequenceGenerator::make(vb);
        float2 r0 = sampleNext2D(sg);
        float2 subPixelOffset = make_float2(cam.Jitter.x + (r0.x - 0.5f) * S.perPixelJitterAAScale, cam.Jitter.y + (r0.y - 0.5f) * S.perPixelJitterAAScale);
        float2 dof = sampleNext2D(sg);
        float2 pp = make_float2(((float)px + 0.5f + -subPixelOffset.x) / (float)cam.ViewportSize.x, ((float)py + 0.5f + subPixelOffset.y) / (float)cam.ViewportSize.y);
        float2 ndc = make_float2(2.f * pp.x + -1.f, -2.f * pp.y + 1.f);
        float3 org = cam.PosW;
        float3 dir = (ndc.x * cam.CameraU + ndc.y * cam.CameraV) + cam.CameraW;
        float2 ap = sample_disk(dof);
        float3 rayTarget = org + dir;
        org = org + cam.ApertureRadius * (ap.x * normalize(cam.CameraU) + ap.y * normalize(cam.CameraV));
        dir = normalize(rayTarget - org);
        float invCos = 1.f / dot(normalize(cam.CameraW), dir);
        float tMin = cam.NearZ * invCos;
        p.origin = org + dir * tMin; p.dir = dir;
        return p;
    }

    PT_SHADE_NOINLINE float4 sampleTexture(uint textureIndexAndInfo, float lambdaNoDims, float2 uv) const {
        uint textureIndex = textureIndexAndInfo & 0xFFFFu, baseLOD = textureIndexAndInfo >> 24, mipLevels = (textureIndexAndInfo >> 16) & 0xFFu;
        float lambda = 0.5f * (float)baseLOD + lambdaNoDims;
        lambda = fminf_(lambda, fmaxf_((float)mipLevels - 5.0f, 0.0f));
        return sample_trilinear(sc, sc.textures[textureIndex], uv, lambda);
    }
    static void computeTangentSpace(ShadingData& sd, float4 tangentW, bool ignoreTangent) {
        float3 t3 = xyz(tangentW);
        float NdotT = dot(t3, sd.N);
        bool nonParallel = fabsf(NdotT) < 0.9999f;
        bool nonZero = dot(t3, t3) > 0.f;
        bool valid = tangentW.w != 0.f && nonZero && nonParallel;
        if (!ignoreTangent && valid) { sd.T = normalize(t3 - sd.N * NdotT); sd.B = cross(sd.N, sd.T) * tangentW.w; }
        else { sd.T = perp_stark(sd.N); sd.B = cross(sd.N, sd.T); }
    }
    static void adjustShadingNormal(ShadingData& sd, float4 tangentW, bool recompute, bool ignoreTangent) {
        float3 Ng = sd.faceNCorrected;
        float signN = dot(sd.N, Ng) >= 0.f ? 1.f : -1.f;
        float3 Ns = signN * sd.N;
        const float kCosThetaThreshold = 0.1f;
        float cosTheta = dot(sd.V, Ns);
        if (cosTheta <= kCosThetaThreshold) {
            float t = saturate(cosTheta * (1.f / kCosThetaThreshold));
            sd.N = signN * normalize(lerp3(Ng, Ns, t));
        }
        if (cosTheta <= kCosThetaThreshold || recompute) computeTangentSpace(sd, tangentW, ignoreTangent);
    }
    float3 prevPosW(uint prim, float bu, float bv) const {
        const uint2 pinfo = sc.primInfo[prim];
        const uint2 ig = sc.subInstToInstGeom[pinfo.x];
        const GeometryDesc& g = sc.geometries[ig.y];
        const float3x4& M = (sc.prevInstances ? sc.prevInstances : sc.instances)[ig.x].transform;
        const float* P = sc.prevPositions ? sc.prevPositions : sc.positions;
        const float3 bary = make_float3(1.0f - (bu + bv), bu, bv);
        const uint* idx = sc.indices + g.indexOffset + pinfo.y * 3;
        const uint vi[3] = {g.vertexOffset + idx[0], g.vertexOffset + idx[1], g.vertexOffset + idx[2]};
        float3 vp[3];
        for (int k = 0; k < 3; k++) vp[k] = make_float3(P[3 * vi[k]], P[3 * vi[k] + 1], P[3 * vi[k] + 2]);
        const float3 objPos = (vp[0] * bary.x + vp[1] * bary.y) + vp[2] * bary.z;
        return xform_point(M, objPos);
    }
    template <bool LEAN = false>
    SurfaceData loadSurface(uint prim, float bu, float bv, float3 rayDir, RayCone rayCone, MVBlockInputs* mvBlock = nullptr) const {
#if PT_SHADE_TRI
        const uint4* rec = reinterpret_cast<const uint4*>(sc.shadeTris + prim);
        const uint4 r0 = rec[0], r1 = rec[1], r2 = rec[2], r3 = rec[3], r4 = rec[4], r5 = rec[5], r6 = rec[6], r7 = rec[7];
        const uint subInst = r0.y, triangleIndex = r0.z, materialIndex = r0.w & 0xFFFFu;
        struct { uint flags; } g; g.flags = r0.w >> 16;
        const float3x4& M = sc.instances[r0.x].transform;
        float3 bary = make_float3(1.0f - (bu + bv), bu, bv);
        float3 vp[3] = {make_float3(asfloat(r1.x), asfloat(r1.y), asfloat(r1.z)), make_float3(asfloat(r1.w), asfloat(r2.x), asfloat(r2.y)), make_float3(asfloat(r2.z), asfloat(r2.w), asfloat(r3.x))};
        float2 vt[3] = {make_float2(0, 0), make_float2(0, 0), make_float2(0, 0)};
        float3 objPos = (vp[0] * bary.x + vp[1] * bary.y) + vp[2] * bary.z;
        float2 texcoord = make_float2(0, 0);
        if (g.flags & GEOM_HAS_UV) {
            vt[0] = make_float2(asfloat(r3.y), asfloat(r3.z)); vt[1] = make_float2(asfloat(r3.w), asfloat(r4.x)); vt[2] = make_float2(asfloat(r4.y), asfloat(r4.z));
            texcoord = (vt[0] * bary.x + vt[1] * bary.y) + vt[2] * bary.z;
        }
        float3 objFlatN = SafeNormalize(cross(vp[1] - vp[0], vp[2] - vp[0]));
        if (mvBlock) mvBlock->curvatureWS = 0.0f;
        float3 geometryNormal = make_float3(0.f);
        if (!LEAN && (g.flags & GEOM_HAS_NORMAL)) {
            const float3 n[3] = {make_float3(asfloat(r4.w), asfloat(r5.x), asfloat(r5.y)), make_float3(asfloat(r5.z), asfloat(r5.w), asfloat(r6.x)), make_float3(asfloat(r6.y), asfloat(r6.z), asfloat(r6.w))};
            if (mvBlock) mvBlock->curvatureWS = TriangleCurvatureApprox_GradN(vp, n, M);
            geometryNormal = (n[0] * bary.x + n[1] * bary.y) + n[2] * bary.z;
            geometryNormal = SafeNormalize(xform_direction4(M, geometryNormal));
        }
        float4 tangent = make_float4(0, 0, 0, 0);
        if (!LEAN && (g.flags & GEOM_HAS_TANGENT)) {
            const uint pg[3] = {r7.x, r7.y, r7.z};
            float4 tg[3];
#else
        uint2 pinfo = sc.primInfo[prim];
        uint subInst = pinfo.x, triangleIndex = pinfo.y;
        uint2 ig = sc.subInstToInstGeom[subInst];
        const InstanceDesc& inst = sc.instances[ig.x];
        const uint materialIndex = sc.subInstances[subInst].GlobalGeometryIndex_PTMaterialDataIndex & 0xFFFFu;
        const GeometryDesc& g = sc.geometries[ig.y];
        const float3x4& M = inst.transform;
        float3 bary = make_float3(1.0f - (bu + bv), bu, bv);
        const uint* idx = sc.indices + g.indexOffset + triangleIndex * 3;
        uint vi[3] = {g.vertexOffset + idx[0], g.vertexOffset + idx[1], g.vertexOffset + idx[2]};
        float3 vp[3]; float2 vt[3] = {make_float2(0, 0), make_float2(0, 0), make_float2(0, 0)};
        for (int k = 0; k < 3; k++) vp[k] = make_float3(sc.positions[3 * vi[k]], sc.positions[3 * vi[k] + 1], sc.positions[3 * vi[k] + 2]);
        float3 objPos = (vp[0] * bary.x + vp[1] * bary.y) + vp[2] * bary.z;
        float2 texcoord = make_float2(0, 0);
        if (g.flags & GEOM_HAS_UV) {
            for (int k = 0; k < 3; k++) vt[k] = sc.uvs[vi[k]];
            texcoord = (vt[0] * bary.x + vt[1] * bary.y) + vt[2] * bary.z;
        }
        float3 objFlatN = SafeNormalize(cross(vp[1] - vp[0], vp[2] - vp[0]));
        if (mvBlock) mvBlock->curvatureWS = 0.0f;
        float3 geometryNormal = make_float3(0.f);
        if (!LEAN && (g.flags & GEOM_HAS_NORMAL)) {
            float3 n[3];
            for (int k = 0; k < 3; k++) {
                n[k] = normalize(Unpack_RGB8_SNORM(sc.normals[vi[k]]));
                if (dot(n[k], objFlatN) < 0.f) n[k] = -n[k];
            }
            if (mvBlock) mvBlock->curvatureWS = TriangleCurvatureApprox_GradN(vp, n, M);
            geometryNormal = (n[0] * bary.x + n[1] * bary.y) + n[2] * bary.z;
            geometryNormal = SafeNormalize(xform_direction4(M, geometryNormal));
        }
        float4 tangent = make_float4(0, 0, 0, 0);
        if (!LEAN && (g.flags & GEOM_HAS_TANGENT)) {
            float4 tg[3];
            const uint pg[3] = {sc.tangents[vi[0]], sc.tangents[vi[1]], sc.tangents[vi[2]]};
#endif
            for (int k = 0; k < 3; k++) tg[k] = Unpack_RGBA8_SNORM(pg[k]);
            float3 t3 = (xyz(tg[0]) * bary.x + xyz(tg[1]) * bary.y) + xyz(tg[2]) * bary.z;
            t3 = SafeNormalize(xform_direction4(M, t3));
            tangent = make_float4(t3, tg[0].w);
        }
        float3 flatNormal = SafeNormalize(xform_direction4(M, objFlatN));
        bool frontFacing = dot(-rayDir, flatNormal) >= 0.0f;
        if (LEAN || !(g.flags & GEOM_HAS_NORMAL)) geometryNormal = flatNormal;
        float3 posW = xform_point(M, objPos);
        float coneTexLODValue = computeRayConeTriangleLODValue(vp, vt, M);
        float lambda = rayCone.computeLOD(coneTexLODValue, rayDir, flatNormal, true) + S.texLODBias;

        ShadingData sd; __builtin_memset(&sd, 0, sizeof(sd));
        sd.posW = posW; sd.V = -rayDir; sd.N = geometryNormal;
        const PTMaterialData& material = sc.materials[materialIndex];
        const uint mflags = material.Flags;
        float4 texBase = make_float4(1, 1, 1, 1), texEmissive = make_float4(1, 1, 1, 1), texNormal = make_float4(0.5f, 0.5f, 1.0f, 0.f),
               texMR = make_float4(1, 1, 1, 1), texTrans = make_float4(1, 1, 1, 1);
        bool hasUV = (g.flags & GEOM_HAS_UV) != 0;
        if (!LEAN && hasUV && (mflags & PTMaterialFlags_UseBaseOrDiffuseTexture)) texBase = sampleTexture(material.BaseOrDiffuseTextureIndex, lambda, texcoord);
        if (!LEAN && hasUV && (mflags & PTMaterialFlags_UseNormalTexture)) texNormal = sampleTexture(material.NormalTextureIndex, lambda, texcoord);
        if (!LEAN && hasUV && (mflags & PTMaterialFlags_UseMetalRoughOrSpecularTexture)) texMR = sampleTexture(material.MetalRoughOrSpecularTextureIndex, lambda, texcoord);
        if (hasUV && (mflags & PTMaterialFlags_UseEmissiveTexture)) texEmissive = sampleTexture(material.EmissiveTextureIndex, lambda, texcoord);
        if (!LEAN && hasUV && (mflags & PTMaterialFlags_UseTransmissionTexture)) texTrans = sampleTexture(material.TransmissionTextureIndex, lambda, texcoord);

        float3 emissiveColor = LP::r3(material.EmissiveColor);
        if (mflags & PTMaterialFlags_UseEmissiveTexture) emissiveColor = LP::mul3(emissiveColor, LP::r3(xyz(texEmissive)));
        float matIoR = LP::r(material.IoR);
        sd.faceNCorrected = frontFacing ? flatNormal : -flatNormal;
        sd.frontFacing = frontFacing;
        bool thin = (mflags & PTMaterialFlags_ThinSurface) != 0;
        sd.materialID = materialIndex;
        sd.mtl = MaterialHeader::make();
        { uint pr = 1 + (mflags >> PTMaterialFlags_NestedPriorityShift); sd.mtl.setNestedPriority(pr < InteriorList::kMaxNestedPriority ? pr : InteriorList::kMaxNestedPriority); }
        sd.mtl.setThinSurface(thin);
        sd.mtl.setActiveLobes(Lobe_All);
        sd.IoR = 1.f;
        StandardBSDFData bd; __builtin_memset(&bd, 0, sizeof(bd));
        if (!LEAN) {
        float3 mGeometryNormal = normalize(geometryNormal), mShadingNormal = mGeometryNormal;
        float3 baseColor = LP::r3(material.BaseOrDiffuseColor * xyz(texBase));
        float roughness = LP::r(material.Roughness * texMR.y);
// ... 339 lines not shown
```

### rtxpt_amd/csrc/pt_wavefront.h

```cpp
#pragma once
#include "pt_path.h"
#include "pt_neeat.h"
#include "pt_tonemap.h"
#include <hip/hip_runtime.h>

namespace ptk {

struct PathPool { uint4* s0; uint4* s1; uint4* s2; uint4* s3; uint4* s4; uint4* hit;
    const uint* home; };
struct ShadowQueue { float4* q0; float4* q1; float4* q2; uint group;
    float4* q3; float* fbTotalWeight; uint* fbCandidates; uint fbWidth, fbPlane, fbSampleFirst; };
struct WaveCounters {
    uint extendCount[2]; uint shadowCount; uint overflow;
    unsigned long long hits, nodeVisitsExt, triTestsExt, nodeVisitsSh, triTestsSh, leafVisitsExt, itersExt, leafVisitsSh, itersSh, phaseCycExt[4], leafBlocksExt, eventsExt[8], itersMaxExt, rayIterHistExt[16]; uint longRayCount, _padLong; float longRays[32][8];
    unsigned long long shadowValid;
    unsigned long long tailExtendRays, tailShadowRays;
    unsigned long long tailHandedBack[3];
};

static const uint TRAV_COUNTERS = 5, TRAV_RESOLVE = 4, PASS_COUNTERS = 16, PASS_SHADOW_OFFSET = 5, PASS_CLASS_OFFSET = 10;
struct TravAux { TravTask* taskQ[2]; uint* counts; uint taskCap; unsigned long long* bestKey; uint* resolveList; const uint* primToSlot; uint maxBlocks; };

void launch_generate(const PathKernelContext& k, PathPool pool, const uint* ownedPixels, uint numOwned, uint sampleFirst, uint spp, uint first, uint n, uint* queue, uint* countPtr, hipStream_t st);
void launch_extend(const DeviceScene& sc, PathPool pool, const uint* queue, const uint* countPtr, uint count, WaveCounters* wc, bool counters, TravAux aux, hipStream_t st, bool ranged = false);
void launch_shade(const PathKernelContext& k, PathPool pool, const uint* queueIn, const uint* countInPtr, uint countIn, uint* queueOut, uint* countOutPtr,
                  ShadowQueue sq, WaveCounters* wc, uint* classScratch, uint* classCount, hipStream_t st, PathPool outPool = PathPool{});
void launch_uncompact(PathPool in, PathPool out, const uint* countPtr, uint count, hipStream_t st);
void launch_classify(PathPool pool, const uint* queueIn, const uint* countInPtr, uint countIn, uint* classScratch, uint* classCount, hipStream_t st);
void launch_shadow(const DeviceScene& sc, PathPool pool, ShadowQueue sq, const uint* countPtr, uint count, WaveCounters* wc, bool counters, TravAux aux, hipStream_t st);
void launch_trace_pair(const DeviceScene& sc, PathPool pool, const uint* queue, const uint* extCountPtr, uint extCount, ShadowQueue sq, uint* shCountPtr, uint shCount, WaveCounters* wc, TravAux auxE, TravAux auxS, hipStream_t st);
void launch_tail(const PathKernelContext& k, PathPool pool, const uint* queueIn, const uint* countInPtr, uint countIn, uint* queueOut, uint* countOutPtr, ShadowQueue sq, WaveCounters* wc, uint maxBounces, uint deferIters , uint maxBlocks, hipStream_t st);
void launch_pass_reset(uint* passCounters, uint* nextCount, uint* shadowCount, hipStream_t st);
void launch_accumulate(PathPool pool, const uint* ownedPixels, uint numOwned, uint spp, float4* accum, uint accumCountBase, uint width, hipStream_t st);
void launch_trace_probe(const DeviceScene& sc, const float4* rays, uint n, float4* outClosest, uint* outVisible, uint* overflow, hipStream_t st);
void launch_pack(const float4* accum, const uint* ownedPixels, uint numOwned, uint width, float4* dst, hipStream_t st);
void launch_unpack(float4* accum, const uint* pixels, uint num, uint width, const float4* src, hipStream_t st);
void launch_pack_feedback(const float* fbW, const uint* fbC, const float* depth, const uint* pixels, uint num, uint width, uint* dst, hipStream_t st);
void launch_unpack_feedback(float* fbW, uint* fbC, float* depth, const uint* pixels, uint num, uint width, const uint* src, hipStream_t st);
void launch_env_cube_bake(const DeviceScene& sc, const EnvDirectionalLight* lights, uint nLights, uint2* texels, const EnvCube& cube, hipStream_t st);
void launch_env_cube_compress(uint2* texels, const EnvCube& cube, uint quality, hipStream_t st);
void launch_env_importance(const DeviceScene& sc, uint dim, uint sx, uint sy, float4* out, hipStream_t st);
void launch_bake_emissive(const DeviceScene& sc, const uint* subInstList, const uint* subInstTriOffset, uint numEmissiveSubInst, uint totalTris, uint lightBase,
                          PolymorphicLightInfo* lights, PolymorphicLightInfoEx* lightsEx, hipStream_t st);
void launch_light_weights(const PolymorphicLightInfo* lights, const PolymorphicLightInfoEx* lightsEx, uint n, float* w, const LightFrustumBoost& boost, hipStream_t st);
void launch_light_proxy_counts(const float* w, uint n, float* sum, uint budget, bool uniform, uint maxPerLight, uint* counts, const uint* usage, uint totalMaxFeedbackCount, float globalFeedbackUseWeight, hipStream_t st);
void launch_neeat_boost_weights(const float* base, const float* hist, uint nHist, uint n, float mul, float* cur, hipStream_t st);
void launch_neeat_begin(const NeeAtFrame& F, float* snapW, uint* snapC, bool preFilter, uint totalThreads, hipStream_t st);
void launch_neeat_end(const NeeAtFrame& F, hipStream_t st);
void launch_light_proxy_fill(const uint* counts, const uint* offsets, uint n, uint* proxies, uint capacity, hipStream_t st);
void launch_tonemap(const float4* accum, uint num, const ToneMapParams& p, uint* outRgba8, hipStream_t st);
void launch_average_log_luminance(const float4* accum, uint W, uint H, float* scratch, float** result, hipStream_t st);
void launch_probe(const PathKernelContext& k, int kind, const void* dIn, void* dOut, uint n, hipStream_t st);

}
```

### rtxpt_amd/csrc/pt_wavefront.hip

```cpp
#include "pt_wavefront.h"
#include "pt_traverse8.h"
#include "pt_traverse8p.h"
#include "pt_wavefront_device.h"
#include <cstdlib>
#define T8_TRAVERSE traverse8_pairs

namespace ptk {

#ifndef PT_SAMPLE_MINOR
#define PT_SAMPLE_MINOR 1
#endif
#ifndef T8_CHUNKS_PER_WAVE_MIN
#define T8_CHUNKS_PER_WAVE_MIN 1
#endif
#ifndef T8_SHORT_TAIL_BELOW
#define T8_SHORT_TAIL_BELOW 32768u
#endif
#ifndef T8_TASK_BLOCKS_N
#define T8_TASK_BLOCKS_N 512
#endif

__global__ void __launch_bounds__(256) k_generate(PathKernelContext k, PathPool pool, const uint* __restrict__ ownedPixels, uint numOwned, uint sampleFirst, uint spp, uint first, uint n, uint* __restrict__ queue, uint* countPtr) {
    const uint t = blockIdx.x * 256u + threadIdx.x;
    if (t >= n) return;
    const uint i = first + t;
#if PT_SAMPLE_MINOR
    uint kpx = i / spp, s = i - kpx * spp, px = ownedPixels[kpx];
#else
    uint s = i / numOwned, px = ownedPixels[i - s * numOwned];
#endif
    PathState p = k.generate(px >> 16, px & 0xFFFFu, sampleFirst + s);
    store_path(pool, i, p);
    queue[t] = i;
    if (countPtr && t == 0u) atomicAdd(countPtr, n);
}

template <bool COUNT, bool RANGED>
__device__ __forceinline__ void t8_extend_body(const DeviceScene& sc, const PathPool& pool, const uint* __restrict__ queue, const uint count, WaveCounters* wc, const TravAux& aux, const uint rpc,
                                               uint2* stack, uint* rayBuf, float2* mineUV, const uint vBlock, const uint vGrid) {
    Traverse8Counters ctr; t8_counters_init(ctr);
    auto fetch = [&](uint i, float3& o, float3& d, float& tmin, float& tmax, uint& startRef, float& bestT0, uint& bestPrim0) -> uint {
        uint p = pool.home ? i : queue[i];
        uint4 a = pool.s0[p], b = pool.s1[p];
        o = make_float3(asfloat(a.x), asfloat(a.y), asfloat(a.z)); d = make_float3(asfloat(b.x), asfloat(b.y), asfloat(b.z));
        tmin = 0.0f; tmax = kMaxRayTravel; startRef = 0u; bestT0 = kMaxRayTravel; bestPrim0 = 0xFFFFFFFFu;
        if (RANGED) { const uint4 r = pool.hit[p]; tmin = asfloat(r.x); tmax = asfloat(r.y); bestT0 = tmax; }
        return p;
    };
    auto commit = [&](uint p, const HitInfo& h) { pool.hit[p] = make_uint4(asuint(h.t), h.prim, asuint(h.u), asuint(h.v)); };
    auto publish = [&](uint p, float bestT, uint bestPrim) { aux.bestKey[p] = t8_hit_key(bestT, bestPrim); aux.resolveList[atomicAdd(&aux.counts[TRAV_RESOLVE], 1u)] = p; };
    if (COUNT) { ctr.rayIterHist = wc->rayIterHistExt; ctr.longRayCount = &wc->longRayCount; ctr.longRays = &wc->longRays[0][0]; }
    T8_TRAVERSE<false, COUNT, !RANGED, false, true>(sc, count, rpc, stack, rayBuf, mineUV, fetch, commit, publish, TravTaskOut{aux.taskQ[0], &aux.counts[0], aux.taskCap}, ctr, &wc->overflow, vBlock, vGrid);
    if (COUNT) { wave_add64(ctr.nodeVisits, &wc->nodeVisitsExt); wave_add64(ctr.triTests, &wc->triTestsExt); wave_add64(ctr.leafVisits, &wc->leafVisitsExt); wave_add64(ctr.iters, &wc->itersExt); wave_add64(ctr.leafBlocks, &wc->leafBlocksExt); if ((threadIdx.x & 63u) == 0u) atomicMax(&wc->itersMaxExt, (unsigned long long)ctr.iters);
                 if ((threadIdx.x & 63u) == 0u) for (int q = 0; q < 4; q++) atomicAdd(&wc->phaseCycExt[q], ctr.cyc[q]);
                 for (int q = 0; q < 8; q++) wave_add64(ctr.ev[q], &wc->eventsExt[q]); }
}
template <bool COUNT, bool RANGED = false>
__global__ void __launch_bounds__(T8_BLOCK, T8_EXTEND_MIN_BLOCKS) k_extend(DeviceScene sc, PathPool pool, const uint* __restrict__ queue, const uint* __restrict__ countPtr, WaveCounters* wc, TravAux aux, uint rpc) {
    __shared__ uint2 stack[T8_GROUPS_PER_BLOCK * BVH8_STACK_STRIDE];
    __shared__ uint rayBuf[T8_RAYBUF_WORDS];
    __shared__ float2 mineUV[T8_BLOCK];
    t8_extend_body<COUNT, RANGED>(sc, pool, queue, *countPtr, wc, aux, rpc, stack, rayBuf, mineUV, blockIdx.x, gridDim.x);
}

#ifndef T8_TASK_SPREAD
#define T8_TASK_SPREAD 1
#endif
__device__ __forceinline__ uint t8_tasks_per_chunk(uint count) { return (!T8_TASK_SPREAD || count > T8_GROUPS_PER_WAVE * 4u * T8_TASK_BLOCKS_N || T8_GROUPS_PER_WAVE > T8_CHUNK) ? T8_CHUNK : T8_GROUPS_PER_WAVE; }
template <int STAGE, bool FINAL>
__device__ __forceinline__ void t8_extend_tasks_body(const DeviceScene& sc, const PathPool& pool, WaveCounters* wc, const TravAux& aux, uint2* stack, uint* rayBuf, const uint vBlock, const uint vGrid) {
    constexpr int IN = STAGE & 1;
    uint count = aux.counts[STAGE]; if (count > aux.taskCap) count = aux.taskCap;
    if (count == 0u) return;
    const TravTask* tasks = aux.taskQ[IN];
    const uint real = t8_tasks_per_chunk(count), per = (count + real - 1u) / real;
    Traverse8Counters ctr; t8_counters_init(ctr);
    auto fetch = [&](uint i, float3& o, float3& d, float& tmin, float& tmax, uint& startRef, float& bestT0, uint& bestPrim0) -> uint {
        const uint lane = i % T8_CHUNK, j = lane * per + i / T8_CHUNK;
        const bool pad = lane >= real || j >= count;
        TravTask t = tasks[pad ? 0u : j];
        if (pad) t.tbits = 0x7F800000u;
        uint4 a = pool.s0[t.tag], b = pool.s1[t.tag];
        o = make_float3(asfloat(a.x), asfloat(a.y), asfloat(a.z)); d = make_float3(asfloat(b.x), asfloat(b.y), asfloat(b.z));
        unsigned long long key = aux.bestKey[t.tag];
        tmin = 0.0f; tmax = kMaxRayTravel; bestT0 = __uint_as_float((uint)(key >> 32)); bestPrim0 = (uint)key;
        startRef = (__uint_as_float(t.tbits) <= bestT0) ? t.ref : BVH_EMPTY;
        return t.tag;
    };
    auto commit = [&](uint p, const HitInfo& h) { atomicMin(&aux.bestKey[p], t8_hit_key(h.t, h.prim)); };
    auto publish = [&](uint p, float bestT, uint bestPrim) { if (bestPrim != 0xFFFFFFFFu) atomicMin(&aux.bestKey[p], t8_hit_key(bestT, bestPrim)); };
    T8_TRAVERSE<false, false, true, true, !FINAL>(sc, per * T8_CHUNK, T8_CHUNK, stack, rayBuf, nullptr, fetch, commit, publish, TravTaskOut{aux.taskQ[IN ^ 1], &aux.counts[FINAL ? STAGE : STAGE + 1], FINAL ? 0u : aux.taskCap}, ctr, &wc->overflow, vBlock, vGrid);
}
template <int STAGE, bool FINAL = (STAGE == 3)>
__global__ void __launch_bounds__(T8_BLOCK, T8_EXTEND_MIN_BLOCKS) k_extend_tasks(DeviceScene sc, PathPool pool, WaveCounters* wc, TravAux aux) {
    __shared__ uint2 stack[T8_GROUPS_PER_BLOCK * BVH8_STACK_STRIDE];
    __shared__ uint rayBuf[T8_TASKBUF_WORDS];
    t8_extend_tasks_body<STAGE, FINAL>(sc, pool, wc, aux, stack, rayBuf, blockIdx.x, gridDim.x);
}

__device__ __forceinline__ void t8_resolve_extend_body(const DeviceScene& sc, const PathPool& pool, const TravAux& aux, const uint vBlock, const uint vGrid) {
    const uint n = aux.counts[TRAV_RESOLVE];
    for (uint i = vBlock * 256u + threadIdx.x; i < n; i += vGrid * 256u) {
        uint p = aux.resolveList[i];
        unsigned long long key = aux.bestKey[p];
        uint prim = (uint)key;
        uint4 out = make_uint4((uint)(key >> 32), prim, 0u, 0u);
        if (prim != 0xFFFFFFFFu) {
            uint4 a = pool.s0[p], b = pool.s1[p];
            float3 o = make_float3(asfloat(a.x), asfloat(a.y), asfloat(a.z)), d = make_float3(asfloat(b.x), asfloat(b.y), asfloat(b.z));
            float t, u = 0.f, v = 0.f;
            const TriRecord tr = sc.tris[aux.primToSlot[prim]]; (void)intersect_tri_wt(tri_v0(tr), tri_v1(tr), tri_v2(tr), o, d, 0.0f, kMaxRayTravel, t, u, v);
            out.z = asuint(u); out.w = asuint(v);
        }
        pool.hit[p] = out;
    }
}
__global__ void __launch_bounds__(256) k_resolve_extend(DeviceScene sc, PathPool pool, TravAux aux) { t8_resolve_extend_body(sc, pool, aux, blockIdx.x, gridDim.x); }

#ifndef PT_SHADE_BLOCK
#define PT_SHADE_BLOCK 256
#endif
#ifndef PT_SHADE_MIN_BLOCKS
#define PT_SHADE_MIN_BLOCKS 1
#endif
#ifndef PT_SHADE_PROBE
#define PT_SHADE_PROBE 0
#endif
#ifndef PT_SHADE_CLASSES
#define PT_SHADE_CLASSES 1
#endif

#define PT_CLASSIFY_ITEMS 4u
__global__ void __launch_bounds__(1024) k_classify(PathPool pool, const uint* __restrict__ queueIn, const uint* __restrict__ countInPtr, uint* __restrict__ classQ, uint* __restrict__ classCount) {
    __shared__ uint waveCnt[PT_CLASSIFY_ITEMS][16][3]; __shared__ uint blockBase[3];
    const uint count = *countInPtr, wave = threadIdx.x >> 6, lane = threadIdx.x & 63u;
    uint p[PT_CLASSIFY_ITEMS], cls[PT_CLASSIFY_ITEMS]; unsigned long long mine[PT_CLASSIFY_ITEMS];
#pragma unroll
    for (uint j = 0; j < PT_CLASSIFY_ITEMS; j++) {
        const uint i = (blockIdx.x * PT_CLASSIFY_ITEMS + j) * 1024u + threadIdx.x;
        p[j] = 0u; cls[j] = 3u;
        if (i < count) {
            p[j] = pool.home ? i : queueIn[i];
            const uint prim = reinterpret_cast<const uint*>(pool.hit)[4u * (size_t)p[j] + 1u], flags = reinterpret_cast<const uint*>(pool.s4)[4u * (size_t)p[j] + 2u];
            cls[j] = (prim == 0xFFFFFFFFu) ? 2u : (((flags >> kVertexIndexBitCount) & PF_terminateAtNextBounce) ? 1u : 0u);
        }
        const unsigned long long m0 = __builtin_amdgcn_ballot_w64(cls[j] == 0u), m1 = __builtin_amdgcn_ballot_w64(cls[j] == 1u), m2 = __builtin_amdgcn_ballot_w64(cls[j] == 2u);
        if (lane == 0u) { waveCnt[j][wave][0] = (uint)__popcll(m0); waveCnt[j][wave][1] = (uint)__popcll(m1); waveCnt[j][wave][2] = (uint)__popcll(m2); }
        mine[j] = cls[j] == 0u ? m0 : (cls[j] == 1u ? m1 : m2);
    }
    __syncthreads();
    if (threadIdx.x < 3u) {
        uint tot = 0;
        for (uint j = 0; j < PT_CLASSIFY_ITEMS; j++) for (uint w = 0; w < 16u; w++) { const uint c = waveCnt[j][w][threadIdx.x]; waveCnt[j][w][threadIdx.x] = tot; tot += c; }
        blockBase[threadIdx.x] = tot ? atomicAdd(&classCount[threadIdx.x], tot) : 0u;
    }
    __syncthreads();
#pragma unroll
    for (uint j = 0; j < PT_CLASSIFY_ITEMS; j++) {
        if (cls[j] > 2u) continue;
        const uint rank = blockBase[cls[j]] + waveCnt[j][wave][cls[j]] + (uint)__popcll(mine[j] & ((1ull << lane) - 1ull));
        classQ[cls[j] == 0u ? rank : (cls[j] == 1u ? count - 1u - rank : count + rank)] = p[j];
    }
}

template <bool MULTI, class PKC, bool NEEAT, bool COMPACT = false>
__global__ void __launch_bounds__(PT_SHADE_BLOCK, PT_SHADE_MIN_BLOCKS) k_shade(PKC k, PathPool pool, const uint* __restrict__ queueIn, const uint* __restrict__ countInPtr,
                                               uint* __restrict__ queueOut, uint* countOutPtr, ShadowQueue sq, WaveCounters* wc, const uint* __restrict__ classCount, PathPool outPool) {
    static_assert(!COMPACT || !PT_SHADE_PROBE, "the PT_SHADE_PROBE timing builds do not know the compacted pool: take the COMPACT launch out of launch_shade and run with MI355PT_COMPACT_POOL=0");
    const uint count = *countInPtr;
    uint i = blockIdx.x * (uint)PT_SHADE_BLOCK + threadIdx.x;
    bool inRange = i < count;
    bool alive = false; bool isHit = false; uint p = 0, hp = 0;
    ShadowRequest req; req.valid = false;
    PathState cpath;
    if (COMPACT) __builtin_memset(&cpath, 0, sizeof(cpath));
    if (inRange) {
        if (classCount) {
            const uint nGo = classCount[0], nEnd = classCount[1];
            p = queueIn[i < nGo ? i : (i < nGo + nEnd ? count - 1u - (i - nGo) : count + (i - nGo - nEnd))];
        } else p = COMPACT ? i : queueIn[i];
        hp = COMPACT ? pool.home[p] : p;
        uint4 hr = pool.hit[p];
        HitInfo h; h.t = asfloat(hr.x); h.prim = hr.y; h.u = asfloat(hr.z); h.v = asfloat(hr.w);
#if PT_SHADE_PROBE
        PathState path = load_path(pool, p);
#if PT_SHADE_PROBE == 1
        if (h.prim != 0xFFFFFFFFu) { isHit = true; path.sceneLength += h.t; } path.terminate();
#elif PT_SHADE_PROBE == 2
        if (h.prim != 0xFFFFFFFFu) { isHit = true; SurfaceData sfd = k.loadSurface(h.prim, h.u, h.v, path.dir, path.rayCone); path.origin = sfd.shadingData.posW + sfd.shadingData.N * sfd.bsdf.data.roughness + sfd.bsdf.data.diffuse + sfd.shadingData.T; } path.terminate();
#endif
        store_path(pool, p, path);
        alive = path.isActive();
#else
        if (COMPACT) {
            const PathCompactIO io{pool, p, hp};
            if (h.prim == 0xFFFFFFFFu) { cpath = io.load_all(); k.template HandleMiss<NEEAT>(cpath, cpath.dir, kMaxRayTravel); }
            else { isHit = true; cpath = io.load_first(); k.template HandleHit<false, NEEAT>(cpath, h, req, nullptr, io); }
            alive = cpath.isActive();
            pool.s2[hp] = make_uint4(cpath.pack23[0], cpath.pack23[1], cpath.pack45[0], cpath.pack45[1]);
        }
        else if (h.prim == 0xFFFFFFFFu) { PathState path = load_path(pool, p); k.template HandleMiss<NEEAT>(path, path.dir, kMaxRayTravel); store_path(pool, p, path); alive = path.isActive(); }
        else {
            isHit = true;
            const PathPoolIO io{pool, p};
            PathState path = io.load_first();
            if (MULTI) { ShadowSink sink{sq.q0, sq.q1, sq.q2, &wc->shadowCount, &wc->shadowValid, p}; k.template HandleHit<true, NEEAT>(path, h, req, &sink, io); }
            else k.template HandleHit<false, NEEAT>(path, h, req, nullptr, io);
            alive = path.isActive();
#ifdef PT_SHADE_PHASE_PROBE
            for (int q = 1; q < 6; q++) wave_add64(io.tk[q] ? (unsigned long long)(uint)(io.tk[q] - io.tk[q - 1 - (io.tk[q - 1] ? 0 : 1)]) : 0ull, &wc->eventsExt[q - 1]);
#endif
        }
#endif
    }
    __shared__ uint sCnt[PT_SHADE_BLOCK / 64][2]; __shared__ uint sBase[2];
    const uint wave = threadIdx.x >> 6, lane = threadIdx.x & 63u;
    const unsigned long long mAlive = __builtin_amdgcn_ballot_w64(alive), mReq = __builtin_amdgcn_ballot_w64(!MULTI && req.valid);
    if (lane == 0u) { sCnt[wave][0] = (uint)__popcll(mAlive); sCnt[wave][1] = (uint)__popcll(mReq); }
    __syncthreads();
    if (threadIdx.x < 2u) {
        uint tot = 0; for (uint w = 0; w < (uint)(PT_SHADE_BLOCK / 64); w++) { const uint c = sCnt[w][threadIdx.x]; sCnt[w][threadIdx.x] = tot; tot += c; }
        sBase[threadIdx.x] = tot ? atomicAdd(threadIdx.x == 0u ? countOutPtr : &wc->shadowCount, tot) : 0u;
    }
    __syncthreads();
    const unsigned long long below = (1ull << lane) - 1ull;
    if (alive) {
        const uint slot = sBase[0] + sCnt[wave][0] + (uint)__popcll(mAlive & below);
        queueOut[slot] = hp;
        if (COMPACT) {
            outPool.s0[slot] = make_uint4(asuint(cpath.origin.x), asuint(cpath.origin.y), asuint(cpath.origin.z), cpath.id);
            outPool.s1[slot] = make_uint4(asuint(cpath.dir.x), asuint(cpath.dir.y), asuint(cpath.dir.z), asuint(cpath.sceneLength));
            outPool.s3[slot] = make_uint4(cpath.interiorList.slots[0], cpath.interiorList.slots[1], cpath.packedCounters, cpath.rayCone.widthSpreadAngleFP16);
            outPool.s4[slot] = make_uint4(cpath.pack0, cpath.pack1, cpath.flagsAndVertexIndex, cpath.sampleIndex);
        }
    }
    if (!MULTI && req.valid) {
        const uint sslot = sBase[1] + sCnt[wave][1] + (uint)__popcll(mReq & below);
        sq.q0[sslot] = make_float4(req.origin.x, req.origin.y, req.origin.z, req.tmax);
        sq.q1[sslot] = make_float4(req.dir.x, req.dir.y, req.dir.z, asfloat(hp));
        sq.q2[sslot] = make_float4(req.radiance.x, req.radiance.y, req.radiance.z, 0.f);
        if (NEEAT && sq.q3) sq.q3[sslot] = make_float4(req.fbWeight, req.fbRandom, asfloat(req.fbLight), asfloat(req.rrFix));
    }
    if (classCount) { if (blockIdx.x == 0u && threadIdx.x == 0u) atomicAdd(&wc->hits, (unsigned long long)classCount[0] + classCount[1]); }
    else wave_add64(isHit ? 1ull : 0ull, &wc->hits);
}

__device__ __forceinline__ void shadow_mark_visible(ShadowQueue sq, uint i) { reinterpret_cast<float*>(sq.q2 + i)[3] = 1.0f; }
template <bool GROUPED>
__device__ __forceinline__ void shadow_visible(PathPool pool, ShadowQueue sq, uint i) {
    if (GROUPED) { shadow_mark_visible(sq, i); return; }
    float4 r = sq.q2[i];
    uint p = asuint(sq.q1[i].w);
    uint4 c = pool.s2[p];
    uint pack45[2] = {c.z, c.w};
    PathKernelContext::ResolveShadow(pack45, make_float3(r.x, r.y, r.z));
    c.z = pack45[0]; c.w = pack45[1];
    pool.s2[p] = c;
    if (sq.q3) {
        const float4 f = sq.q3[i];
        const uint light = asuint(f.z), fix = asuint(f.w);
        if (light != RTXPT_INVALID_LIGHT_INDEX) {
            uint4 e = pool.s4[p];
            const uint id = pool.s0[p].w, slot = (e.w - sq.fbSampleFirst) * sq.fbPlane + (id & 0xFFFFu) * sq.fbWidth + (id >> 16);
            float total = sq.fbTotalWeight[slot]; uint cand = sq.fbCandidates[slot];
            LightFeedbackReservoir_Add(total, cand, f.y, light & ~LFR_SCREEN_SPACE_COHERENT_FLAG, f.x, (light & LFR_SCREEN_SPACE_COHERENT_FLAG) != 0u);
            sq.fbTotalWeight[slot] = total; sq.fbCandidates[slot] = cand;
            if (fix & 1u) {
                const uint bit = (uint)PF_terminateAtNextBounce << kVertexIndexBitCount;
                if (fix & 2u) e.z |= bit; else { e.z &= ~bit; e.y = (e.y & 0xFFFF0000u) | (fix >> 16); }
                pool.s4[p] = e;
            }
        }
    }
}

template <bool COUNT>
__device__ __forceinline__ void t8_shadow_body(const DeviceScene& sc, const ShadowQueue& sq, const uint count, WaveCounters* wc, const TravAux& aux, const uint rpc,
                                               uint2* stack, uint* rayBuf, const uint vBlock, const uint vGrid) {
    Traverse8Counters ctr; t8_counters_init(ctr);
    auto fetch = [&](uint i, float3& o, float3& d, float& tmin, float& tmax, uint& startRef, float& bestT0, uint& bestPrim0) -> uint {
        float4 a = sq.q0[i], b = sq.q1[i];
        o = make_float3(a.x, a.y, a.z); d = make_float3(b.x, b.y, b.z); tmin = 0.0f; tmax = a.w; startRef = 0u; bestT0 = a.w; bestPrim0 = 0xFFFFFFFFu;
        return i;
    };
    auto commit = [&](uint i, const HitInfo& h) { if (h.prim == 0xFFFFFFFFu) shadow_mark_visible(sq, i); };
    auto publish = [&](uint i, float, uint) { aux.bestKey[i] = 0ull; aux.resolveList[atomicAdd(&aux.counts[TRAV_RESOLVE], 1u)] = i; };
    T8_TRAVERSE<true, COUNT, false, false, true>(sc, count, rpc, stack, rayBuf, nullptr, fetch, commit, publish, TravTaskOut{aux.taskQ[0], &aux.counts[0], aux.taskCap}, ctr, &wc->overflow, vBlock, vGrid);
    if (COUNT) { wave_add64(ctr.nodeVisits, &wc->nodeVisitsSh); wave_add64(ctr.triTests, &wc->triTestsSh); wave_add64(ctr.leafVisits, &wc->leafVisitsSh); wave_add64(ctr.iters, &wc->itersSh); }
}
template <bool COUNT>
__global__ void __launch_bounds__(T8_BLOCK, COUNT ? 1 : T8_SHADOW_MIN_WAVES) k_shadow(DeviceScene sc, ShadowQueue sq, const uint* __restrict__ countPtr, WaveCounters* wc, TravAux aux, uint rpc) {
    __shared__ uint2 stack[T8_GROUPS_PER_BLOCK * BVH8_STACK_STRIDE];
    __shared__ uint rayBuf[T8_RAYBUF_WORDS];
    t8_shadow_body<COUNT>(sc, sq, *countPtr, wc, aux, rpc, stack, rayBuf, blockIdx.x, gridDim.x);
}

template <int STAGE, bool FINAL>
__device__ __forceinline__ void t8_shadow_tasks_body(const DeviceScene& sc, const ShadowQueue& sq, WaveCounters* wc, const TravAux& aux, uint2* stack, uint* rayBuf, const uint vBlock, const uint vGrid) {
    constexpr int IN = STAGE & 1;
    uint count = aux.counts[STAGE]; if (count > aux.taskCap) count = aux.taskCap;
    if (count == 0u) return;
    const TravTask* tasks = aux.taskQ[IN];
    const uint real = t8_tasks_per_chunk(count), per = (count + real - 1u) / real;
    Traverse8Counters ctr; t8_counters_init(ctr);
    auto fetch = [&](uint i, float3& o, float3& d, float& tmin, float& tmax, uint& startRef, float& bestT0, uint& bestPrim0) -> uint {
        const uint lane = i % T8_CHUNK, j = lane * per + i / T8_CHUNK;
        const bool pad = lane >= real || j >= count;
        TravTask t = tasks[pad ? 0u : j];
        float4 a = sq.q0[t.tag], b = sq.q1[t.tag];
        o = make_float3(a.x, a.y, a.z); d = make_float3(b.x, b.y, b.z); tmin = 0.0f; tmax = a.w; bestT0 = a.w; bestPrim0 = 0xFFFFFFFFu;
        startRef = (!pad && aux.bestKey[t.tag] == 0ull) ? t.ref : BVH_EMPTY;
        return t.tag;
    };
    auto commit = [&](uint i, const HitInfo& h) { if (h.prim != 0xFFFFFFFFu) aux.bestKey[i] = 1ull; };
    auto publish = [&](uint, float, uint) {};
    T8_TRAVERSE<true, false, false, true, !FINAL>(sc, per * T8_CHUNK, T8_CHUNK, stack, rayBuf, nullptr, fetch, commit, publish, TravTaskOut{aux.taskQ[IN ^ 1], &aux.counts[FINAL ? STAGE : STAGE + 1], FINAL ? 0u : aux.taskCap}, ctr, &wc->overflow, vBlock, vGrid);
}
template <int STAGE, bool FINAL = (STAGE == 3)>
__global__ void __launch_bounds__(T8_BLOCK) k_shadow_tasks(DeviceScene sc, ShadowQueue sq, WaveCounters* wc, TravAux aux) {
    __shared__ uint2 stack[T8_GROUPS_PER_BLOCK * BVH8_STACK_STRIDE];
    __shared__ uint rayBuf[T8_TASKBUF_WORDS];
    t8_shadow_tasks_body<STAGE, FINAL>(sc, sq, wc, aux, stack, rayBuf, blockIdx.x, gridDim.x);
}

template <bool GROUPED>
__device__ __forceinline__ void t8_resolve_shadow_body(const PathPool& pool, const ShadowQueue& sq, const TravAux& aux, const uint count, const uint vBlock, const uint vGrid) {
    const uint n = aux.counts[TRAV_RESOLVE];
    for (uint k = vBlock * 256u + threadIdx.x; k < n; k += vGrid * 256u) {
        uint i = aux.resolveList[k];
        if (aux.bestKey[i] == 0ull) shadow_visible<GROUPED>(pool, sq, i);
    }
    if (GROUPED) return;
    for (uint i = vBlock * 256u + threadIdx.x; i < count; i += vGrid * 256u)
        if (reinterpret_cast<const float*>(sq.q2 + i)[3] == 1.0f) shadow_visible<false>(pool, sq, i);
}
template <bool GROUPED>
__global__ void __launch_bounds__(256) k_resolve_shadow(PathPool pool, ShadowQueue sq, TravAux aux, uint count) { t8_resolve_shadow_body<GROUPED>(pool, sq, aux, count, blockIdx.x, gridDim.x); }

__global__ void __launch_bounds__(T8_BLOCK, T8_EXTEND_MIN_BLOCKS) k_trace_pair(DeviceScene sc, PathPool pool, const uint* __restrict__ queue, const uint* __restrict__ extCountPtr, ShadowQueue sq, const uint* __restrict__ shCountPtr,
                                                                              WaveCounters* wc, TravAux auxE, TravAux auxS, uint rpcE, uint rpcS, uint blocksE) {
    __shared__ uint2 stack[T8_GROUPS_PER_BLOCK * BVH8_STACK_STRIDE];
    __shared__ uint rayBuf[T8_RAYBUF_WORDS];
    __shared__ float2 mineUV[T8_BLOCK];
    if (blockIdx.x < blocksE) t8_extend_body<false, false>(sc, pool, queue, *extCountPtr, wc, auxE, rpcE, stack, rayBuf, mineUV, blockIdx.x, blocksE);
    else t8_shadow_body<false>(sc, sq, *shCountPtr, wc, auxS, rpcS, stack, rayBuf, blockIdx.x - blocksE, gridDim.x - blocksE);
}
template <int STAGE, bool FINAL = (STAGE == 3)>
// ... 185 lines not shown
}

#ifdef MI355PT_TEST_HOOKS
__global__ void __launch_bounds__(64) k_probe(PathKernelContext k, int kind, const float* __restrict__ in, float* __restrict__ out, uint n) {
    uint i = blockIdx.x * 64u + threadIdx.x; if (i >= n) return;
    switch (kind) {
    case 0: { const float* p = in + 3 * i; int fn = (int)p[0]; float x = p[1], y = p[2]; float r;
        switch (fn) { case 0: r = dm_sin(x); break; case 1: r = dm_cos(x); break; case 2: r = dm_exp2(x); break; case 3: r = dm_log2(x); break;
                      case 4: r = dm_atan2(y, x); break; case 5: r = dm_pow(x, y); break; case 6: r = FastACos(x); break; default: r = FastSqrt(x); break; }
        out[i] = r; } break;
    case 1: { float x = in[i]; uint hbits = f32tof16(x); out[2 * i] = asfloat(hbits); out[2 * i + 1] = f16tof32(hbits); } break;
    case 2: { const uint* p = reinterpret_cast<const uint*>(in) + 6 * i;
        SampleGeneratorVertexBase vb = SampleGeneratorVertexBase::make(p[0], p[1], p[2]);
        uint cnt = p[5] > 8 ? 8 : p[5];
        if (p[4] == 0) { float4 v = SampleSequenceGenerator::Generate(cnt, vb, p[3]); out[8 * i] = v.x; out[8 * i + 1] = v.y; out[8 * i + 2] = v.z; out[8 * i + 3] = v.w; }
        else if (p[4] == 1) { float4 v = UniformSampleSequenceGenerator::Generate(cnt, vb, p[3]); out[8 * i] = v.x; out[8 * i + 1] = v.y; out[8 * i + 2] = v.z; out[8 * i + 3] = v.w; }
        else if (p[4] == 2) { UniformSampleSequenceGenerator g = UniformSampleSequenceGenerator::make(vb, p[3]); for (uint j = 0; j < cnt; j++) out[8 * i + j] = sampleNext1D(g); }
        else { SampleSequenceGenerator g = SampleSequenceGenerator::make(vb, p[3], p[4] == 4); for (uint j = 0; j < cnt; j++) out[8 * i + j] = sampleNext1D(g); } } break;
    case 3: { const float* p = in + 24 * i;
        ShadingData sd; __builtin_memset(&sd, 0, sizeof(sd));
        sd.N = make_float3(0, 0, 1); sd.T = make_float3(1, 0, 0); sd.B = make_float3(0, 1, 0); sd.V = make_float3(p[16], p[17], p[18]);
        sd.faceNCorrected = sd.N; sd.vertexN = sd.N; sd.frontFacing = true; sd.mtl = MaterialHeader::make(); sd.mtl.setActiveLobes(Lobe_All); sd.mtl.setThinSurface(p[14] != 0.f);
        StandardBSDF b; b.diffuseModel = (int)p[15];
        b.data.diffuse = make_float3(p[0], p[1], p[2]); b.data.specular = make_float3(p[3], p[4], p[5]); b.data.roughness = p[6]; b.data.metallic = p[7];
        b.data.transmission = make_float3(p[8], p[9], p[10]); b.data.diffuseTransmission = p[11]; b.data.specularTransmission = p[12]; b.data.eta = p[13];
        float* o = out + 10 * i;
        if (p[22] == 0.f) { float3 wo = make_float3(p[19], p[20], p[21]); float4 e = b.eval(sd, wo); o[0] = e.x; o[1] = e.y; o[2] = e.z; o[3] = e.w; o[4] = b.evalPdf(sd, wo); o[5] = (float)b.getLobes(); o[6] = o[7] = o[8] = o[9] = 0.f; }
        else { BSDFSample s; __builtin_memset(&s, 0, sizeof(s)); bool v = b.sample(sd, make_float4(p[19], p[20], p[21], 0), s);
               o[0] = s.wo.x; o[1] = s.wo.y; o[2] = s.wo.z; o[3] = s.pdf; o[4] = s.weight.x; o[5] = s.weight.y; o[6] = s.weight.z; o[7] = (float)s.lobe; o[8] = s.lobeP; o[9] = v ? 1.f : 0.f; } } break;
    case 4: { const uint* p = reinterpret_cast<const uint*>(in) + 3 * i;
        PathState ps = k.generate(p[0], p[1], p[2]);
        out[6 * i] = ps.origin.x; out[6 * i + 1] = ps.origin.y; out[6 * i + 2] = ps.origin.z; out[6 * i + 3] = ps.dir.x; out[6 * i + 4] = ps.dir.y; out[6 * i + 5] = ps.dir.z; } break;
    case 5: { const float* a = in + 9 * i + 1; int fn = (int)in[9 * i]; float* o = out + 4 * i; o[0] = o[1] = o[2] = o[3] = 0.f;
        switch (fn) {
        case 0: o[0] = evalFresnelSchlick(a[0], a[1], a[2]); break;
        case 1: { float3 r = evalFresnelSchlick(make_float3(a[0], a[1], a[2]), a[3], a[4]); o[0] = r.x; o[1] = r.y; o[2] = r.z; } break;
        case 2: { float ct = 0.f; o[0] = evalFresnelDielectric(a[0], a[1], ct); o[1] = ct; } break;
        case 3: o[0] = evalNdfGGX(a[0], a[1]); break;
        case 4: o[0] = evalPdfGGX_BVNDF(a[0], make_float3(a[1], a[2], a[3]), make_float3(a[4], a[5], a[6])); break;
        case 5: { float3 r = sampleGGX_BVNDF(a[0], make_float3(a[1], a[2], a[3]), make_float2(a[4], a[5])); o[0] = r.x; o[1] = r.y; o[2] = r.z; } break;
        case 6: o[0] = evalLambdaGGX(a[0], a[1]); break;
        case 7: o[0] = evalMaskingSmithGGXCorrelated(a[0], a[1], a[2]); break;
        case 8: { float2 r = ndir_to_oct_equal_area_unorm(make_float3(a[0], a[1], a[2])); o[0] = r.x; o[1] = r.y; } break;
        case 9: { float3 r = oct_to_ndir_equal_area_unorm(make_float2(a[0], a[1])); o[0] = r.x; o[1] = r.y; o[2] = r.z; } break;
        case 10: { float2 r = sample_disk(make_float2(a[0], a[1])); o[0] = r.x; o[1] = r.y; } break;
        case 11: { float2 r = sample_disk_concentric(make_float2(a[0], a[1])); o[0] = r.x; o[1] = r.y; } break;
        case 12: { float pdf = 0.f; float3 r = sample_cosine_hemisphere_concentric(make_float2(a[0], a[1]), pdf); o[0] = r.x; o[1] = r.y; o[2] = r.z; o[3] = pdf; } break;
        case 13: { float3 r = perp_stark(make_float3(a[0], a[1], a[2])); o[0] = r.x; o[1] = r.y; o[2] = r.z; } break;
        case 14: { float3 r = ComputeRayOrigin(make_float3(a[0], a[1], a[2]), make_float3(a[3], a[4], a[5])); o[0] = r.x; o[1] = r.y; o[2] = r.z; } break;
        case 15: o[0] = FastSqrt(a[0]); break;
        case 16: o[0] = FastACos(a[0]); break;
        case 17: o[0] = ComputeRayConeSpreadAngleExpansionByScatterPDF(a[0], a[1]); break;
        case 18: o[0] = ComputeNewScatterFireflyFilterK<LPOps<false>>(a[0], a[1], a[2]); break;
        case 19: { float3 r = FireflyFilter<LPOps<false>>(make_float3(a[0], a[1], a[2]), a[3], a[4]); o[0] = r.x; o[1] = r.y; o[2] = r.z; } break;
        case 20: o[0] = FireflyFilterShort(a[0], a[1], a[2]); break;
        case 21: o[0] = ComputeLowGrazingAngleFalloff(make_float3(a[0], a[1], a[2]), make_float3(a[3], a[4], a[5]), a[6], a[7]); break;
        default: break;
        } } break;
    case 6: { const uint* a = reinterpret_cast<const uint*>(in) + 19 * i + 1; const uint lk = reinterpret_cast<const uint*>(in)[19 * i]; uint* o = reinterpret_cast<uint*>(out) + 12 * i;
        for (int q = 0; q < 12; q++) o[q] = 0u;
        const float3x4 I = {{1, 0, 0, 0, 0, 1, 0, 0, 0, 0, 1, 0}};
        auto info = [&](const uint* w) { PolymorphicLightInfoFull li; __builtin_memset(&li, 0, sizeof(li));
            li.Base.Center = make_float3(asfloat(w[0]), asfloat(w[1]), asfloat(w[2])); li.Base.ColorTypeAndFlags = w[3]; li.Base.Direction1 = w[4]; li.Base.Direction2 = w[5]; li.Base.Scalars = w[6]; li.Base.LogRadiance = w[7];
            li.Extended.IesProfileIndex = w[8]; li.Extended.PrimaryAxis = w[9]; li.Extended.CosConeAngleAndSoftness = w[10]; li.Extended.UniqueID = w[11]; return li; };
        if (lk == 0u) { PolymorphicLightInfo b; __builtin_memset(&b, 0, sizeof(b)); PackLightColor(make_float3(asfloat(a[0]), asfloat(a[1]), asfloat(a[2])), b); float3 c = UnpackLightColor(b);
            o[0] = b.ColorTypeAndFlags; o[1] = b.LogRadiance; o[2] = asuint(c.x); o[3] = asuint(c.y); o[4] = asuint(c.z); }
        else if (lk == 1u) { TriangleLight t; t.base = make_float3(asfloat(a[0]), asfloat(a[1]), asfloat(a[2])); t.edge1 = make_float3(asfloat(a[3]), asfloat(a[4]), asfloat(a[5])); t.edge2 = make_float3(asfloat(a[6]), asfloat(a[7]), asfloat(a[8]));
            t.radiance = make_float3(asfloat(a[9]), asfloat(a[10]), asfloat(a[11])); t.normal = make_float3(0.f); t.surfaceArea = 0;
            PolymorphicLightInfoFull li = t.Store(7u);
            o[0] = asuint(li.Base.Center.x); o[1] = asuint(li.Base.Center.y); o[2] = asuint(li.Base.Center.z); o[3] = li.Base.ColorTypeAndFlags; o[4] = li.Base.Direction1; o[5] = li.Base.Direction2; o[6] = li.Base.Scalars; o[7] = li.Base.LogRadiance;
            o[8] = li.Extended.IesProfileIndex; o[9] = li.Extended.PrimaryAxis; o[10] = li.Extended.CosConeAngleAndSoftness; o[11] = li.Extended.UniqueID; }
        else if (lk == 2u) { PolymorphicLightInfoFull li = info(a);
            PolymorphicLightSample sm = PolymorphicLight_CalcSample(li, make_float2(asfloat(a[12]), asfloat(a[13])), make_float3(asfloat(a[14]), asfloat(a[15]), asfloat(a[16])), I);
            o[0] = asuint(sm.Position.x); o[1] = asuint(sm.Position.y); o[2] = asuint(sm.Position.z); o[3] = asuint(sm.Normal.x); o[4] = asuint(sm.Normal.y); o[5] = asuint(sm.Normal.z);
            o[6] = asuint(sm.Radiance.x); o[7] = asuint(sm.Radiance.y); o[8] = asuint(sm.Radiance.z); o[9] = asuint(sm.SolidAnglePdf); o[10] = sm.LightSampleableByBSDF ? 1u : 0u; o[11] = asuint(PolymorphicLight_GetPower(li)); }
        else if (lk == 3u) { TriangleLight t = TriangleLight::Create(info(a));
            o[0] = asuint(t.CalcSolidAnglePdfForMIS(make_float3(asfloat(a[12]), asfloat(a[13]), asfloat(a[14])), make_float3(asfloat(a[15]), asfloat(a[16]), asfloat(a[17])))); }
        else { uint pk = NDirToOctUnorm32(make_float3(asfloat(a[0]), asfloat(a[1]), asfloat(a[2]))); float3 d = OctToNDirUnorm32(pk); o[0] = pk; o[1] = asuint(d.x); o[2] = asuint(d.y); o[3] = asuint(d.z); }
        } break;
    case 8: { const float* a = in + 8 * i; uint* o = reinterpret_cast<uint*>(out) + 45 * i;
        RayCone rc = RayCone::make(a[6], a[7]);
        auto emit = [&](const SurfaceData& q) {
            const ShadingData& s = q.shadingData; const StandardBSDFData& b = q.bsdf.data;
            auto put3 = [&](float3 v) { *o++ = asuint(v.x); *o++ = asuint(v.y); *o++ = asuint(v.z); };
            put3(s.posW); put3(s.faceNCorrected); put3(s.V); put3(s.N); put3(s.T); put3(s.B); put3(s.vertexN);
            *o++ = s.frontFacing ? 1u : 0u; *o++ = s.mtl.packedData; *o++ = s.materialID; *o++ = asuint(s.IoR); *o++ = asuint(s.shadowNoLFadeout); put3(s.emission);
            put3(b.diffuse); *o++ = asuint(b.roughness); put3(b.specular); *o++ = asuint(b.metallic); put3(b.transmission);
            *o++ = asuint(b.diffuseTransmission); *o++ = asuint(b.specularTransmission); *o++ = asuint(b.eta); *o++ = asuint(q.interiorIoR); *o++ = q.neeTriangleLightIndex; };
        if (k.S.useFp16Types) { PathKernelContextT<true> k16; __builtin_memcpy(&k16, &k, sizeof(k16)); emit(k16.loadSurface(asuint(a[0]), a[1], a[2], make_float3(a[3], a[4], a[5]), rc)); }
        else emit(k.loadSurface(asuint(a[0]), a[1], a[2], make_float3(a[3], a[4], a[5]), rc));
        } break;
    case 7: { const float* a = in + 4 * i; const int op = (int)a[0]; typedef LPOps<true> H; float r = 0.f;
        switch (op) { case 0: r = H::r(a[1]); break; case 1: r = H::add(H::r(a[1]), H::r(a[2])); break; case 2: r = H::sub(H::r(a[1]), H::r(a[2])); break; case 3: r = H::mul(H::r(a[1]), H::r(a[2])); break;
                      case 4: r = H::div(H::r(a[1]), H::r(a[2])); break; case 5: r = H::lerp(H::r(a[1]), H::r(a[2]), H::r(a[3])); break;
                      case 7: r = H::r(a[1] * a[2]); break; case 8: r = H::r(H::r(a[1]) * a[2]); break; case 9: r = H::r(a[1] + a[2]); break; case 10: r = H::r(a[1] / a[2]); break;
                      default: r = H::average3(make_float3(H::r(a[1]), H::r(a[2]), H::r(a[3]))); break; }
        out[i] = r; } break;
    case 10: { const uint* a = reinterpret_cast<const uint*>(in) + 3 * i; uint* o = reinterpret_cast<uint*>(out) + 2 * i;
        const uint slot = k.sc.primToSlot[a[0]]; const TriRecord tr = k.sc.tris[slot];
        const bool solid = !(tr.flags & 1u) || alpha_test_slot(k.sc, slot, asfloat(a[1]), asfloat(a[2]));
        o[0] = solid ? 1u : 0u; o[1] = (!(tr.flags & 1u) || (!(tr.flags & 2u) && solid)) ? 1u : 0u; } break;
    case 9: { const float* a = in + 4 * i; float* o = out + 3 * i;
        float3 r = k.sc.envEnabled ? env_eval_local(k.sc, make_float3(a[0], a[1], a[2]), a[3]) : make_float3(0.f);
        o[0] = r.x; o[1] = r.y; o[2] = r.z; } break;
    default: break;
    }
}
#endif

#ifndef T8_ADAPTIVE_CHUNKS
#define T8_ADAPTIVE_CHUNKS 1
#endif
static inline uint rays_per_chunk(uint count) {
    if (!T8_ADAPTIVE_CHUNKS) return T8_CHUNK;
    const uint resident = 256u * 4u * 8u;
    const uint step = T8_GROUPS_PER_WAVE;
    uint r = ((count + resident - 1u) / resident + step - 1u) / step * step;
    return r < step ? (step > T8_CHUNK ? T8_CHUNK : step) : (r > T8_CHUNK ? T8_CHUNK : r);
}
static inline uint grid_for(uint count, uint block, uint maxBlocks) { uint g = (count + block - 1) / block; if (g < 1) g = 1; if (g > maxBlocks) g = maxBlocks; return g; }

__global__ void __launch_bounds__(256) k_tonemap(const float4* __restrict__ accum, uint num, ToneMapParams p, uint* __restrict__ out) {
    uint i = blockIdx.x * 256u + threadIdx.x;
    if (i < num) out[i] = tm_pixel(p, accum[i]);
}
void launch_tonemap(const float4* accum, uint num, const ToneMapParams& p, uint* outRgba8, hipStream_t st) {
    hipLaunchKernelGGL(k_tonemap, dim3((num + 255) / 256), dim3(256), 0, st, accum, num, p, outRgba8);
}
__global__ void __launch_bounds__(256) k_log_luminance(const float4* __restrict__ accum, uint W, uint H, uint LW, uint LH, float* __restrict__ out) {
    uint i = blockIdx.x * 256u + threadIdx.x;
    if (i < LW * LH) out[i] = tm_log_luminance_texel(accum, W, H, LW, LH, i % LW, i / LW);
}
__global__ void __launch_bounds__(256) k_luminance_mip(const float* __restrict__ src, uint w, uint h, uint ow, uint oh, float* __restrict__ dst) {
    uint i = blockIdx.x * 256u + threadIdx.x;
    if (i < ow * oh) dst[i] = tm_mip_texel(src, w, h, i % ow, i / ow);
}
void launch_average_log_luminance(const float4* accum, uint W, uint H, float* scratch, float** result, hipStream_t st) {
    uint w = tm_pow2_floor(W), h = tm_pow2_floor(H);
    float* a = scratch; float* b = scratch + (size_t)w * h;
    hipLaunchKernelGGL(k_log_luminance, dim3((w * h + 255) / 256), dim3(256), 0, st, accum, W, H, w, h, a);
    while (w > 1u || h > 1u) {
        uint ow = w > 1u ? w / 2u : 1u, oh = h > 1u ? h / 2u : 1u;
        hipLaunchKernelGGL(k_luminance_mip, dim3((ow * oh + 255) / 256), dim3(256), 0, st, a, w, h, ow, oh, b);
        float* t = a; a = b; b = t; w = ow; h = oh;
    }
    *result = a;
}
void launch_generate(const PathKernelContext& k, PathPool pool, const uint* ownedPixels, uint numOwned, uint sampleFirst, uint spp, uint first, uint n, uint* queue, uint* countPtr, hipStream_t st) {
    if (n) hipLaunchKernelGGL(k_generate, dim3((n + 255) / 256), dim3(256), 0, st, k, pool, ownedPixels, numOwned, sampleFirst, spp, first, n, queue, countPtr);
}
static const uint T8_TASK_BLOCKS = T8_TASK_BLOCKS_N, T8_RESOLVE_BLOCKS = 256;
static const uint T8_SWEEP_BLOCKS = 2048;
static inline uint shadow_resolve_grid(uint count) { const uint g = grid_for(count, 256u, T8_SWEEP_BLOCKS); return g < T8_RESOLVE_BLOCKS ? T8_RESOLVE_BLOCKS : g; }
void launch_extend(const DeviceScene& sc, PathPool pool, const uint* queue, const uint* countPtr, uint count, WaveCounters* wc, bool counters, TravAux aux, hipStream_t st, bool ranged) {
    const uint rpc = rays_per_chunk(count);
    uint g = grid_for(count, (T8_BLOCK / 64u) * rpc * T8_CHUNKS_PER_WAVE_MIN, (aux.maxBlocks && aux.maxBlocks < T8_MAX_BLOCKS) ? aux.maxBlocks : T8_MAX_BLOCKS);
    if (ranged) { if (counters) hipLaunchKernelGGL((k_extend<true, true>), dim3(g), dim3(T8_BLOCK), 0, st, sc, pool, queue, countPtr, wc, aux, rpc);
                  else hipLaunchKernelGGL((k_extend<false, true>), dim3(g), dim3(T8_BLOCK), 0, st, sc, pool, queue, countPtr, wc, aux, rpc); }
    else if (counters) hipLaunchKernelGGL((k_extend<true>), dim3(g), dim3(T8_BLOCK), 0, st, sc, pool, queue, countPtr, wc, aux, rpc);
    else hipLaunchKernelGGL((k_extend<false>), dim3(g), dim3(T8_BLOCK), 0, st, sc, pool, queue, countPtr, wc, aux, rpc);
    if (count <= T8_SHORT_TAIL_BELOW) {
        hipLaunchKernelGGL((k_extend_tasks<0>), dim3(T8_TASK_BLOCKS), dim3(T8_BLOCK), 0, st, sc, pool, wc, aux);
        hipLaunchKernelGGL((k_extend_tasks<1, true>), dim3(T8_TASK_BLOCKS), dim3(T8_BLOCK), 0, st, sc, pool, wc, aux);
        hipLaunchKernelGGL(k_resolve_extend, dim3(T8_RESOLVE_BLOCKS), dim3(256), 0, st, sc, pool, aux);
        return;
    }
    hipLaunchKernelGGL((k_extend_tasks<0>), dim3(T8_TASK_BLOCKS), dim3(T8_BLOCK), 0, st, sc, pool, wc, aux);
    hipLaunchKernelGGL((k_extend_tasks<1>), dim3(T8_TASK_BLOCKS), dim3(T8_BLOCK), 0, st, sc, pool, wc, aux);
    hipLaunchKernelGGL((k_extend_tasks<2>), dim3(T8_TASK_BLOCKS), dim3(T8_BLOCK), 0, st, sc, pool, wc, aux);
    hipLaunchKernelGGL((k_extend_tasks<3>), dim3(T8_TASK_BLOCKS), dim3(T8_BLOCK), 0, st, sc, pool, wc, aux);
    hipLaunchKernelGGL(k_resolve_extend, dim3(T8_RESOLVE_BLOCKS), dim3(256), 0, st, sc, pool, aux);
}
void launch_trace_pair(const DeviceScene& sc, PathPool pool, const uint* queue, const uint* extCountPtr, uint extCount, ShadowQueue sq, uint* shCountPtr, uint shCount, WaveCounters* wc, TravAux auxE, TravAux auxS, hipStream_t st) {
    const uint rpc = rays_per_chunk(extCount + shCount);
    const uint bound = (auxE.maxBlocks && auxE.maxBlocks < T8_MAX_BLOCKS) ? auxE.maxBlocks : T8_MAX_BLOCKS;
    uint gE = grid_for(extCount, (T8_BLOCK / 64u) * rpc * T8_CHUNKS_PER_WAVE_MIN, bound), gS = grid_for(shCount, (T8_BLOCK / 64u) * rpc * T8_CHUNKS_PER_WAVE_MIN, bound);
    if (gE + gS > bound) {
        uint s = (uint)(((unsigned long long)bound * shCount + (extCount + shCount) / 2u) / (extCount + shCount)); if (s < 1u) s = 1u; if (s > bound - 1u) s = bound - 1u;
        if (s > gS) s = gS;
        uint e = bound - s; if (e > gE) { e = gE; s = (bound - e < gS) ? bound - e : gS; }
        gE = e; gS = s;
    }
    hipLaunchKernelGGL(k_trace_pair, dim3(gE + gS), dim3(T8_BLOCK), 0, st, sc, pool, queue, extCountPtr, sq, shCountPtr, wc, auxE, auxS, rpc, rpc, gE);
    const dim3 tg(2u * T8_TASK_BLOCKS), tb(T8_BLOCK);
    if (extCount <= T8_SHORT_TAIL_BELOW && shCount <= T8_SHORT_TAIL_BELOW) {
        hipLaunchKernelGGL((k_tasks_pair<0>), tg, tb, 0, st, sc, pool, sq, wc, auxE, auxS);
        hipLaunchKernelGGL((k_tasks_pair<1, true>), tg, tb, 0, st, sc, pool, sq, wc, auxE, auxS);
    } else {
        hipLaunchKernelGGL((k_tasks_pair<0>), tg, tb, 0, st, sc, pool, sq, wc, auxE, auxS);
        hipLaunchKernelGGL((k_tasks_pair<1>), tg, tb, 0, st, sc, pool, sq, wc, auxE, auxS);
        hipLaunchKernelGGL((k_tasks_pair<2>), tg, tb, 0, st, sc, pool, sq, wc, auxE, auxS);
        hipLaunchKernelGGL((k_tasks_pair<3>), tg, tb, 0, st, sc, pool, sq, wc, auxE, auxS);
    }
    hipLaunchKernelGGL(k_resolve_pair, dim3(T8_RESOLVE_BLOCKS + shadow_resolve_grid(shCount)), dim3(256), 0, st, sc, pool, sq, auxE, auxS, shCountPtr, shCount, T8_RESOLVE_BLOCKS);
}
void launch_classify(PathPool pool, const uint* queueIn, const uint* countInPtr, uint countIn, uint* classScratch, uint* classCount, hipStream_t st) {
    hipLaunchKernelGGL(k_classify, dim3((countIn + 1024u * PT_CLASSIFY_ITEMS - 1u) / (1024u * PT_CLASSIFY_ITEMS)), dim3(1024), 0, st, pool, queueIn, countInPtr, classScratch, classCount);
}
void launch_shade(const PathKernelContext& k, PathPool pool, const uint* queueIn, const uint* countInPtr, uint countIn, uint* queueOut, uint* countOutPtr, ShadowQueue sq, WaveCounters* wc,
                  uint* classScratch, uint* classCount, hipStream_t st, PathPool outPool) {
    const dim3 g((countIn + PT_SHADE_BLOCK - 1) / PT_SHADE_BLOCK), b(PT_SHADE_BLOCK);
    if (PT_SHADE_CLASSES && classScratch) {
        hipLaunchKernelGGL(k_classify, dim3((countIn + 1024u * PT_CLASSIFY_ITEMS - 1u) / (1024u * PT_CLASSIFY_ITEMS)), dim3(1024), 0, st, pool, queueIn, countInPtr, classScratch, classCount);
        queueIn = classScratch;
    } else classCount = nullptr;
    const bool neeat = k.sc.lights.LocalSamplingBuffer != nullptr || k.sc.lights.TemporalFeedbackRequired != 0u;
#define PT_LAUNCH_SHADE(MULTI, PKC, CTX) do { if (neeat) hipLaunchKernelGGL((k_shade<MULTI, PKC, true>), g, b, 0, st, CTX, pool, queueIn, countInPtr, queueOut, countOutPtr, sq, wc, classCount, outPool); \
                                              else if (pool.home && !MULTI) hipLaunchKernelGGL((k_shade<false, PKC, false, true>), g, b, 0, st, CTX, pool, queueIn, countInPtr, queueOut, countOutPtr, sq, wc, classCount, outPool); \
                                              else hipLaunchKernelGGL((k_shade<MULTI, PKC, false>), g, b, 0, st, CTX, pool, queueIn, countInPtr, queueOut, countOutPtr, sq, wc, classCount, outPool); } while (0)
    if (k.S.useFp16Types) {
        static_assert(sizeof(PathKernelContextT<true>) == sizeof(PathKernelContext), "the two lp builds share one context layout");
        PathKernelContextT<true> k16; __builtin_memcpy(&k16, &k, sizeof(k16));
        if (sq.group) PT_LAUNCH_SHADE(true, PathKernelContextT<true>, k16); else PT_LAUNCH_SHADE(false, PathKernelContextT<true>, k16);
    } else {
        if (sq.group) PT_LAUNCH_SHADE(true, PathKernelContext, k); else PT_LAUNCH_SHADE(false, PathKernelContext, k);
    }
#undef PT_LAUNCH_SHADE
}
void launch_shadow(const DeviceScene& sc, PathPool pool, ShadowQueue sq, const uint* countPtr, uint count, WaveCounters* wc, bool counters, TravAux aux, hipStream_t st) {
    const uint rpc = rays_per_chunk(count);
    uint g = grid_for(count, (T8_BLOCK / 64u) * rpc * T8_CHUNKS_PER_WAVE_MIN, (aux.maxBlocks && aux.maxBlocks < T8_MAX_BLOCKS) ? aux.maxBlocks : T8_MAX_BLOCKS);
    if (counters && !sq.group) hipLaunchKernelGGL((k_shadow<true>), dim3(g), dim3(T8_BLOCK), 0, st, sc, sq, countPtr, wc, aux, rpc);
    else hipLaunchKernelGGL((k_shadow<false>), dim3(g), dim3(T8_BLOCK), 0, st, sc, sq, countPtr, wc, aux, rpc);
    hipLaunchKernelGGL((k_shadow_tasks<0>), dim3(T8_TASK_BLOCKS), dim3(T8_BLOCK), 0, st, sc, sq, wc, aux);
    if (count <= T8_SHORT_TAIL_BELOW) hipLaunchKernelGGL((k_shadow_tasks<1, true>), dim3(T8_TASK_BLOCKS), dim3(T8_BLOCK), 0, st, sc, sq, wc, aux);
    else {
    hipLaunchKernelGGL((k_shadow_tasks<1>), dim3(T8_TASK_BLOCKS), dim3(T8_BLOCK), 0, st, sc, sq, wc, aux);
    hipLaunchKernelGGL((k_shadow_tasks<2>), dim3(T8_TASK_BLOCKS), dim3(T8_BLOCK), 0, st, sc, sq, wc, aux);
    hipLaunchKernelGGL((k_shadow_tasks<3>), dim3(T8_TASK_BLOCKS), dim3(T8_BLOCK), 0, st, sc, sq, wc, aux);
    }
    if (sq.group) hipLaunchKernelGGL((k_resolve_shadow<true>), dim3(T8_RESOLVE_BLOCKS), dim3(256), 0, st, pool, sq, aux, 0u);
    else hipLaunchKernelGGL((k_resolve_shadow<false>), dim3(shadow_resolve_grid(count)), dim3(256), 0, st, pool, sq, aux, count);
    if (sq.group) hipLaunchKernelGGL(k_resolve_nee, dim3(grid_for(count / sq.group, 256, 4096)), dim3(256), 0, st, pool, sq, countPtr);
}
__global__ void __launch_bounds__(64) k_pass_begin(uint* __restrict__ passCounters, uint* __restrict__ nextCount, uint* __restrict__ shadowCount) {
    if (threadIdx.x < PASS_COUNTERS) passCounters[threadIdx.x] = 0u;
    if (threadIdx.x == 32u) *nextCount = 0u;
    if (threadIdx.x == 33u && shadowCount) *shadowCount = 0u;
}
void launch_pass_reset(uint* passCounters, uint* nextCount, uint* shadowCount, hipStream_t st) { static_assert(PASS_COUNTERS <= 32u, "k_pass_begin"); hipLaunchKernelGGL(k_pass_begin, dim3(1), dim3(64), 0, st, passCounters, nextCount, shadowCount); }
__global__ void __launch_bounds__(256) k_uncompact(PathPool in, PathPool out, const uint* __restrict__ countPtr) {
    const uint i = blockIdx.x * 256u + threadIdx.x;
    if (i >= *countPtr) return;
    const uint hp = in.home[i];
    out.s0[hp] = in.s0[i]; out.s1[hp] = in.s1[i]; out.s3[hp] = in.s3[i]; out.s4[hp] = in.s4[i];
}
void launch_uncompact(PathPool in, PathPool out, const uint* countPtr, uint count, hipStream_t st) {
    if (count) hipLaunchKernelGGL(k_uncompact, dim3((count + 255u) / 256u), dim3(256), 0, st, in, out, countPtr);
}
void launch_accumulate(PathPool pool, const uint* ownedPixels, uint numOwned, uint spp, float4* accum, uint accumCountBase, uint width, hipStream_t st) {
    hipLaunchKernelGGL(k_accumulate, dim3((numOwned + 255) / 256), dim3(256), 0, st, pool, ownedPixels, numOwned, spp, accum, accumCountBase, width);
}
void launch_trace_probe(const DeviceScene& sc, const float4* rays, uint n, float4* outClosest, uint* outVisible, uint* overflow, hipStream_t st) {
    hipLaunchKernelGGL(k_trace_probe, dim3(grid_for(n, T8_BLOCK, T8_MAX_BLOCKS)), dim3(T8_BLOCK), 0, st, sc, rays, n, outClosest, outVisible, overflow);
}
__global__ void __launch_bounds__(256) k_pack_feedback(const float* __restrict__ fbW, const uint* __restrict__ fbC, const float* __restrict__ depth, const uint* __restrict__ pixels, uint num, uint width, uint* __restrict__ dst) {
    uint i = blockIdx.x * 256u + threadIdx.x; if (i >= num) return;
    const uint px = pixels[i], slot = (px & 0xFFFFu) * width + (px >> 16);
    dst[3u * i] = __float_as_uint(fbW[slot]); dst[3u * i + 1u] = fbC[slot]; dst[3u * i + 2u] = depth ? __float_as_uint(depth[slot]) : 0u;
}
__global__ void __launch_bounds__(256) k_unpack_feedback(float* __restrict__ fbW, uint* __restrict__ fbC, float* __restrict__ depth, const uint* __restrict__ pixels, uint num, uint width, const uint* __restrict__ src) {
    uint i = blockIdx.x * 256u + threadIdx.x; if (i >= num) return;
    const uint px = pixels[i], slot = (px & 0xFFFFu) * width + (px >> 16);
    fbW[slot] = __uint_as_float(src[3u * i]); fbC[slot] = src[3u * i + 1u]; if (depth) depth[slot] = __uint_as_float(src[3u * i + 2u]);
}
void launch_pack_feedback(const float* fbW, const uint* fbC, const float* depth, const uint* pixels, uint num, uint width, uint* dst, hipStream_t st) {
    if (num) hipLaunchKernelGGL(k_pack_feedback, dim3((num + 255) / 256), dim3(256), 0, st, fbW, fbC, depth, pixels, num, width, dst);
}
void launch_unpack_feedback(float* fbW, uint* fbC, float* depth, const uint* pixels, uint num, uint width, const uint* src, hipStream_t st) {
    if (num) hipLaunchKernelGGL(k_unpack_feedback, dim3((num + 255) / 256), dim3(256), 0, st, fbW, fbC, depth, pixels, num, width, src);
}
void launch_pack(const float4* accum, const uint* pixels, uint num, uint width, float4* dst, hipStream_t st) {
    hipLaunchKernelGGL(k_pack, dim3((num + 255) / 256), dim3(256), 0, st, accum, pixels, num, width, dst);
}
void launch_unpack(float4* accum, const uint* pixels, uint num, uint width, const float4* src, hipStream_t st) {
    hipLaunchKernelGGL(k_unpack, dim3((num + 255) / 256), dim3(256), 0, st, accum, pixels, num, width, src);
}
void launch_env_importance(const DeviceScene& sc, uint dim, uint sx, uint sy, float4* out, hipStream_t st) {
    hipLaunchKernelGGL(k_env_importance, dim3((dim * dim + 255) / 256), dim3(256), 0, st, sc, dim, sx, sy, out);
}
__global__ void __launch_bounds__(256) k_light_weights(const PolymorphicLightInfo* __restrict__ lights, const PolymorphicLightInfoEx* __restrict__ lightsEx, uint n, float* __restrict__ w, LightFrustumBoost boost) {
    uint i = blockIdx.x * 256u + threadIdx.x; if (i >= n) return;
    PolymorphicLightInfoFull lf; lf.Base = lights[i]; lf.Extended = lightsEx[i];
    float wt = dm_pow(PolymorphicLight_GetPower(lf), 0.8f);
    if (!(wt >= 1e-8f)) wt = 0.f;
    w[i] = light_importance_frustum_boost(boost, lf, wt);
}
__global__ void __launch_bounds__(256) k_light_weight_sum(const float* __restrict__ w, uint n, float* __restrict__ sum) {
    __shared__ float stage[256];
    float s = 0.f;
    for (uint base = 0; base < n; base += 256u) {
        const uint i = base + threadIdx.x;
        stage[threadIdx.x] = (i < n) ? w[i] : 0.f;
        __syncthreads();
        if (threadIdx.x == 0) { const uint m = (n - base < 256u) ? n - base : 256u; for (uint k = 0; k < m; k++) s += stage[k]; }
        __syncthreads();
    }
    if (threadIdx.x == 0) *sum = s;
}
__global__ void __launch_bounds__(256) k_light_proxy_counts(const float* __restrict__ w, uint n, const float* __restrict__ sum, uint budget, uint uniform, uint maxPerLight, uint* __restrict__ counts,
                                                            const uint* __restrict__ usage, uint totalMaxFeedbackCount, float globalFeedbackUseWeight) {
    uint i = blockIdx.x * 256u + threadIdx.x; if (i >= n) return;
    float lightWeight = w[i];
    if (usage) lightWeight = neeat_feedback_light_weight(lightWeight, usage[i], *sum, totalMaxFeedbackCount, usage[n], globalFeedbackUseWeight);
    uint cnt = 0;
    if (lightWeight > 0) cnt = uniform ? 1u : (uint)ceilf(((float)(budget - n) * lightWeight) / *sum);
    counts[i] = cnt < maxPerLight ? cnt : maxPerLight;
}
__global__ void __launch_bounds__(256) k_neeat_boost_weights(const float* __restrict__ base, const float* __restrict__ hist, uint nHist, uint n, float mul, float* __restrict__ cur) {
    uint i = blockIdx.x * 256u + threadIdx.x; if (i >= n) return;
    cur[i] = hist ? neeat_intensity_delta_boost(base[i], i < nHist ? hist[i] : 0.f, mul) : base[i];
}
__global__ void __launch_bounds__(256) k_neeat_prefilter(NeeAtFrame F, const float* __restrict__ snapW, const uint* __restrict__ snapC) {
    uint i = blockIdx.x * 256u + threadIdx.x; if (i >= F.W * F.H) return;
    neeat_prefilter_pixel(F, snapW, snapC, (int)(i % F.W), (int)(i / F.W));
}
static const uint NEEAT_P0_TABLE = 512u;
__global__ void __launch_bounds__(1024) k_neeat_p0(NeeAtFrame F, uint totalThreads) {
    __shared__ uint hKey[NEEAT_P0_TABLE]; __shared__ uint hCnt[NEEAT_P0_TABLE];
    const uint NONE = 0xFFFFFFFFu, lane = threadIdx.x & 63u, wave = threadIdx.x >> 6;
    for (uint k = threadIdx.x; k < NEEAT_P0_TABLE; k += 1024u) { hKey[k] = NONE; hCnt[k] = 0u; }
    if (blockIdx.x == 0u && threadIdx.x == 0u && totalThreads > F.W * F.H) atomicAdd(&F.perLightCounters[F.totalLightCount], totalThreads - F.W * F.H);
    __syncthreads();
    const uint regionsX = (F.W + 31u) / 32u;
    const uint px = (blockIdx.x % regionsX) * 32u + (wave & 3u) * 8u + (lane & 7u), py = (blockIdx.x / regionsX) * 32u + (wave >> 2) * 8u + (lane >> 3);
    const uint slot = (px < F.W && py < F.H) ? neeat_p0_pixel(F, px, py) : NONE;
    unsigned long long active = __builtin_amdgcn_ballot_w64(slot != NONE);
    while (active) {
        const uint leader = (uint)__builtin_ctzll(active);
        const uint v = (uint)__builtin_amdgcn_readlane((int)slot, (int)leader);
        const unsigned long long same = __builtin_amdgcn_ballot_w64(slot == v);
        if (lane == leader) {
            const uint n = (uint)__popcll(same);
            uint h = (v * 2654435761u) >> 23; bool placed = false;
            for (uint probe = 0; probe < 16u && !placed; probe++, h = (h + 1u) & (NEEAT_P0_TABLE - 1u)) {
                const uint prev = atomicCAS(&hKey[h], NONE, v);
                if (prev == NONE || prev == v) { atomicAdd(&hCnt[h], n); placed = true; }
            }
            if (!placed) atomicAdd(&F.perLightCounters[v], n);
        }
        active &= ~same;
    }
    __syncthreads();
    for (uint k = threadIdx.x; k < NEEAT_P0_TABLE; k += 1024u) if (hKey[k] != NONE) atomicAdd(&F.perLightCounters[hKey[k]], hCnt[k]);
}
__global__ void __launch_bounds__(256) k_neeat_p1a(NeeAtFrame F) { uint i = blockIdx.x * 256u + threadIdx.x; if (i < F.BW * F.BH) neeat_p1a_pixel(F, i % F.BW, i / F.BW); }
__global__ void __launch_bounds__(256) k_neeat_p1b(NeeAtFrame F) { uint i = blockIdx.x * 256u + threadIdx.x; if (i < F.W * F.H) neeat_p1b_pixel(F, i % F.W, i / F.W); }
__global__ void __launch_bounds__(64) k_neeat_p2(NeeAtFrame F) { uint i = blockIdx.x * 64u + threadIdx.x; if (i < F.tilesX * F.tilesY) neeat_fill_tile(F, i % F.tilesX, i / F.tilesX); }
__global__ void __launch_bounds__(64) k_neeat_p3(NeeAtFrame F) {
    __shared__ uint key[RTXPT_LIGHTING_LOCAL_PROXY_COUNT];
    const uint N = RTXPT_LIGHTING_LOCAL_PROXY_COUNT, t = threadIdx.x;
    uint* tile = F.local + (size_t)blockIdx.x * N;
    key[t] = UnpackMiniListLight(tile[t]); key[t + N / 2] = UnpackMiniListLight(tile[t + N / 2]);
    __syncthreads();
    for (uint k = 2; k <= N; k <<= 1) for (uint j = k / 2; j > 0; j >>= 1) {
        const uint mask = j - 1u, hi = ((t & ~mask) << 1) | (t & mask) | j, lo = hi ^ (k == 2u * j ? k - 1u : j);
        const uint a = key[lo], b = key[hi];
        if (a > b) { key[lo] = b; key[hi] = a; }
        __syncthreads();
    }
    for (uint e = t; e < N; e += N / 2) {
        const uint v = key[e]; uint l = e, r = e;
// ... 63 lines not shown
```

### rtxpt_amd/csrc/pt_wavefront_device.h

```cpp
#pragma once
#include "pt_wavefront.h"
#include "pt_traverse8.h"

namespace ptk {

__device__ __forceinline__ uint lane_id() { return __lane_id(); }
__device__ __forceinline__ uint wave_append(bool pred, uint* counter) {
    unsigned long long mask = __ballot(pred);
    if (mask == 0ull) return 0u;
    uint lane = lane_id();
    uint leader = (uint)__ffsll((long long)mask) - 1u;
    uint base = 0;
    if (lane == leader) base = atomicAdd(counter, (uint)__popcll(mask));
    base = __shfl(base, (int)leader);
    return base + (uint)__popcll(mask & ((1ull << lane) - 1ull));
}
__device__ __forceinline__ void wave_add64(unsigned long long v, unsigned long long* counter) {
    for (int o = 32; o > 0; o >>= 1) v += __shfl_xor(v, o);
    if (lane_id() == 0 && v) atomicAdd(counter, v);
}

__device__ __forceinline__ void store_path(const PathPool& pool, uint i, const PathState& p) {
    pool.s0[i] = make_uint4(asuint(p.origin.x), asuint(p.origin.y), asuint(p.origin.z), p.id);
    pool.s1[i] = make_uint4(asuint(p.dir.x), asuint(p.dir.y), asuint(p.dir.z), asuint(p.sceneLength));
    pool.s2[i] = make_uint4(p.pack23[0], p.pack23[1], p.pack45[0], p.pack45[1]);
    pool.s3[i] = make_uint4(p.interiorList.slots[0], p.interiorList.slots[1], p.packedCounters, p.rayCone.widthSpreadAngleFP16);
    pool.s4[i] = make_uint4(p.pack0, p.pack1, p.flagsAndVertexIndex, p.sampleIndex);
}
__device__ __forceinline__ PathState load_path(const PathPool& pool, uint i) {
    PathState p;
    uint4 a = pool.s0[i], b = pool.s1[i], c = pool.s2[i], d = pool.s3[i], e = pool.s4[i];
    p.origin = make_float3(asfloat(a.x), asfloat(a.y), asfloat(a.z)); p.id = a.w;
    p.dir = make_float3(asfloat(b.x), asfloat(b.y), asfloat(b.z)); p.sceneLength = asfloat(b.w);
    p.pack23[0] = c.x; p.pack23[1] = c.y; p.pack45[0] = c.z; p.pack45[1] = c.w;
    p.interiorList.slots[0] = d.x; p.interiorList.slots[1] = d.y; p.packedCounters = d.z; p.rayCone.widthSpreadAngleFP16 = d.w;
    p.pack0 = e.x; p.pack1 = e.y; p.flagsAndVertexIndex = e.z; p.sampleIndex = e.w;
    return p;
}

struct PathPoolIO {
    static constexpr bool streams = true;
    PathPool pool; uint i;
#ifdef PT_SHADE_PHASE_PROBE
    mutable uint tk[8] = {0u, 0u, 0u, 0u, 0u, 0u, 0u, 0u};
    __device__ __forceinline__ void mark(int k) const { tk[k] = (uint)__builtin_readcyclecounter(); }
#else
    __device__ __forceinline__ void mark(int) const {}
#endif
    __device__ __forceinline__ PathState load_first() const {
        PathState p; uint4 b = pool.s1[i], d = pool.s3[i];
        p.dir = make_float3(asfloat(b.x), asfloat(b.y), asfloat(b.z)); p.sceneLength = asfloat(b.w);
        p.interiorList.slots[0] = d.x; p.interiorList.slots[1] = d.y; p.packedCounters = d.z; p.rayCone.widthSpreadAngleFP16 = d.w;
        p.flagsAndVertexIndex = reinterpret_cast<const uint*>(pool.s4)[4u * (size_t)i + 2u];
        return p;
    }
    __device__ __forceinline__ void load_rest(PathState& p) const {
        asm volatile("" ::: "memory");
        uint4 a = pool.s0[i], c = pool.s2[i], e = pool.s4[i];
        p.origin = make_float3(asfloat(a.x), asfloat(a.y), asfloat(a.z)); p.id = a.w;
        p.pack23[0] = c.x; p.pack23[1] = c.y; p.pack45[0] = c.z; p.pack45[1] = c.w;
        p.pack0 = e.x; p.pack1 = e.y; p.flagsAndVertexIndex = e.z; p.sampleIndex = e.w;
    }
    __device__ __forceinline__ void store_front(const PathState& p) const {
        pool.s0[i] = make_uint4(asuint(p.origin.x), asuint(p.origin.y), asuint(p.origin.z), p.id);
        pool.s1[i] = make_uint4(asuint(p.dir.x), asuint(p.dir.y), asuint(p.dir.z), asuint(p.sceneLength));
        pool.s2[i] = make_uint4(p.pack23[0], p.pack23[1], p.pack45[0], p.pack45[1]);
        pool.s3[i] = make_uint4(p.interiorList.slots[0], p.interiorList.slots[1], p.packedCounters, p.rayCone.widthSpreadAngleFP16);
    }
    __device__ __forceinline__ void store_back(const PathState& p) const { pool.s4[i] = make_uint4(p.pack0, p.pack1, p.flagsAndVertexIndex, p.sampleIndex); }
    __device__ __forceinline__ void store_all(const PathState& p) const { store_path(pool, i, p); }
};

struct PathCompactIO {
    static constexpr bool streams = true;
    PathPool pool; uint i, hp;
    __device__ __forceinline__ void mark(int) const {}
    __device__ __forceinline__ PathState load_first() const {
        PathState p; uint4 b = pool.s1[i], d = pool.s3[i];
        p.dir = make_float3(asfloat(b.x), asfloat(b.y), asfloat(b.z)); p.sceneLength = asfloat(b.w);
        p.interiorList.slots[0] = d.x; p.interiorList.slots[1] = d.y; p.packedCounters = d.z; p.rayCone.widthSpreadAngleFP16 = d.w;
        p.flagsAndVertexIndex = reinterpret_cast<const uint*>(pool.s4)[4u * (size_t)i + 2u];
        return p;
    }
    __device__ __forceinline__ void load_rest(PathState& p) const {
        asm volatile("" ::: "memory");
        uint4 a = pool.s0[i], c = pool.s2[hp], e = pool.s4[i];
        p.origin = make_float3(asfloat(a.x), asfloat(a.y), asfloat(a.z)); p.id = a.w;
        p.pack23[0] = c.x; p.pack23[1] = c.y; p.pack45[0] = c.z; p.pack45[1] = c.w;
        p.pack0 = e.x; p.pack1 = e.y; p.flagsAndVertexIndex = e.z; p.sampleIndex = e.w;
    }
    __device__ __forceinline__ PathState load_all() const { PathState p = load_first(); load_rest(p); return p; }
    __device__ __forceinline__ void store_front(const PathState&) const {}
    __device__ __forceinline__ void store_back(const PathState&) const {}
    __device__ __forceinline__ void store_all(const PathState&) const {}
};

__device__ __forceinline__ void t8_counters_init(Traverse8Counters& ctr) {
    ctr.nodeVisits = 0; ctr.triTests = 0; ctr.leafVisits = 0; ctr.iters = 0; ctr.leafBlocks = 0; for (int q = 0; q < 8; q++) ctr.ev[q] = 0u; ctr.cyc[0] = ctr.cyc[1] = ctr.cyc[2] = ctr.cyc[3] = 0ull;
    ctr.rayIterHist = nullptr; ctr.longRayCount = nullptr; ctr.longRays = nullptr;
}
__device__ __forceinline__ unsigned long long t8_hit_key(float t, uint prim) { return ((unsigned long long)__float_as_uint(t) << 32) | prim; }


}
```

Before: 1864 Mrays/s.

## Generate camera rays in place for first vertex instead of storing path pool

When the compact pool is in use, the generate kernel is skipped for the first bounce. The extend kernel recomputes camera rays from the pixel index, and the shade kernel rebuilds the initial path state from pixel and sample instead of reading it from the pool. Stragglers that need resolving get their rays written by a small split kernel. This removes the full pool write and read for vertex 0, in exchange for recomputing camera rays and extra kernel variants.

```diff
diff --git a/rtxpt_amd/csrc/pt_api.hip b/rtxpt_amd/csrc/pt_api.hip
--- a/rtxpt_amd/csrc/pt_api.hip
+++ b/rtxpt_amd/csrc/pt_api.hip
@@ -530,6 +530,7 @@
       if (e && !strcmp(e, "karras")) c->bvhBuilder = BVH_BUILDER_KARRAS; else if (e && !strcmp(e, "ploc")) c->bvhBuilder = BVH_BUILDER_PLOC; else if (e && !strcmp(e, "sah")) c->bvhBuilder = BVH_BUILDER_SAH; else if (e && (!strcmp(e, "ploc_opt") || !strcmp(e, "device"))) c->bvhBuilder = BVH_BUILDER_PLOC_OPT; }
     { const char* e = getenv("MI355PT_TAIL_PATHS"); if (e) c->tailBelow = (uint)strtoul(e, nullptr, 10); }
     { const char* e = getenv("MI355PT_COMPACT_POOL"); if (e) c->compactPool = atoi(e) != 0; }
+    { const char* e = getenv("MI355PT_FIRST_VERTEX_IN_PLACE"); if (e) c->firstVertexInPlace = atoi(e) != 0; }
     { const char* e = getenv("MI355PT_FUSED_TRAVERSAL"); if (e) c->fusedTraversal = (uint)strtoul(e, nullptr, 10); }
     { const char* e = getenv("MI355PT_TAIL_DEFER"); if (e) c->tailDefer = (uint)strtoul(e, nullptr, 10); }
     memset(&c->dsc, 0, sizeof(c->dsc)); memset(&c->cam, 0, sizeof(c->cam)); memset(&c->bvh, 0, sizeof(c->bvh));
diff --git a/rtxpt_amd/csrc/pt_context.h b/rtxpt_amd/csrc/pt_context.h
--- a/rtxpt_amd/csrc/pt_context.h
+++ b/rtxpt_amd/csrc/pt_context.h
@@ -65,6 +65,9 @@
 #ifndef PT_COMPACT_POOL
 #define PT_COMPACT_POOL 1
 #endif
+#ifndef PT_FIRST_VERTEX_IN_PLACE
+#define PT_FIRST_VERTEX_IN_PLACE 1
+#endif
 #ifndef PT_FREE_RUN_BELOW
 #define PT_FREE_RUN_BELOW (1u << 22)
 #endif
@@ -76,7 +79,7 @@
 struct pt_context {
     int device = 0; hipStream_t stream = nullptr; uint shardRank = 0, shardCount = 1;
     hipStream_t streams[PT_PIPELINE_BATCHES] = {}; WaveCounters* hostCounters = nullptr; bool serialKernels = false;
-    uint tailBelow = PT_TAIL_PATHS, tailDefer = 0, fusedTraversal = PT_FUSED_TRAVERSAL; bool compactPool = PT_COMPACT_POOL != 0;
+    uint tailBelow = PT_TAIL_PATHS, tailDefer = 0, fusedTraversal = PT_FUSED_TRAVERSAL; bool compactPool = PT_COMPACT_POOL != 0, firstVertexInPlace = PT_FIRST_VERTEX_IN_PLACE != 0;
     std::string lastError;
     std::vector<uint> indices; std::vector<float> positions; std::vector<ptk::float2> uvs; std::vector<uint> normals, tangents;
     std::vector<GeometryDesc> geometries; std::vector<MeshDesc> meshes; std::vector<InstanceDesc> instances;
diff --git a/rtxpt_amd/csrc/pt_frame.hip b/rtxpt_amd/csrc/pt_frame.hip
--- a/rtxpt_amd/csrc/pt_frame.hip
+++ b/rtxpt_amd/csrc/pt_frame.hip
@@ -133,6 +133,7 @@
     uint tailLaunches = 0; bool afterTail = false, inTail = false;
     uint pendingShadow = 0; TravAux auxSh;
     PathPool poolSet[2]; uint set = 0; bool compact = false;
+    bool firstInPlace = false;
     bool timed = false; Events marks; size_t t0 = 0, t1 = 0;
     struct Span { size_t a, b; int kind; uint items; }; std::vector<Span> spans;
     size_t mark() { return timed ? marks.mark(st) : 0; }
@@ -171,7 +172,10 @@
         const bool fuse = composed && (c->fusedTraversal == 1u || (c->fusedTraversal == 2u && total < PT_FUSED_BELOW));
         if (fuse) { int32_t r = enable_fused(); if (r != PT_OK) return r; }
         const bool neeatShade = c->dsc.lights.LocalSamplingBuffer != nullptr || c->dsc.lights.TemporalFeedbackRequired != 0u;
-        if (composed && c->compactPool && !neeatShade && !feedback) return enable_compact_pool();
+        if (composed && c->compactPool && !neeatShade && !feedback) {
+            int32_t r = enable_compact_pool(); if (r != PT_OK) return r;
+            if (c->firstVertexInPlace) enable_first_vertex_in_place();
+        }
         return PT_OK;
     }
     int32_t enable_fused() {
@@ -195,12 +199,18 @@
         }
         return PT_OK;
     }
+    void enable_first_vertex_in_place() {
+        for (uint b = 0; b < numBatches; b++) {
+            RenderBatch& t = B[b]; t.firstInPlace = t.compact && !(tailBelow && t.total <= tailBelow);
+            t.hwc->firstCamera.cam = t.k.cam; t.hwc->firstCamera.perPixelJitterAAScale = t.k.S.perPixelJitterAAScale;
+        }
+    }
     int32_t start() {
         for (uint b = 0; b < numBatches; b++) {
             RenderBatch& t = B[b];
             t.t0 = t.mark();
             PT_CHECK_HIP(c, hipMemcpyAsync(t.wc, t.hwc, sizeof(WaveCounters), hipMemcpyHostToDevice, t.st));
-            launch_generate(t.k, t.pool, c->dOwned.p + t.pixFirst, t.numPix, first, count, 0u, t.total, t.queue[0], nullptr, t.st);
+            if (!t.firstInPlace) launch_generate(t.k, t.pool, c->dOwned.p + t.pixFirst, t.numPix, first, count, 0u, t.total, t.queue[0], nullptr, t.st);
         }
         return PT_OK;
     }
@@ -213,14 +223,17 @@
         PathPool pin = t.pool, pout = PathPool{};
         if (t.compact) { pin = t.poolSet[t.set]; pin.home = t.queue[t.cur]; pout = t.poolSet[t.set ^ 1u]; t.set ^= 1u; }
         const uint* countIn = &t.wc->extendCount[t.cur];
-        if (t.pendingShadow) {
+        const bool vertex0 = t.firstInPlace && t.iterations == 0u;
+        const FirstVertex fv{c->dOwned.p + t.pixFirst, t.numPix, first, count};
+        if (vertex0) launch_extend_first(t.k, pin, fv, countIn, t.active, t.wc, t.aux, t.st);
+        else if (t.pendingShadow) {
             launch_trace_pair(t.sc, pin, t.queue[t.cur], countIn, t.active, t.sq, &t.wc->shadowCount, t.pendingShadow, t.wc, t.aux, t.auxSh, t.st);
             t.pendingShadow = 0;
         } else launch_extend(t.sc, pin, t.queue[t.cur], countIn, t.active, t.wc, c->countersEnabled, t.aux, t.st);
         const size_t e1 = t.mark(); t.span(e0, e1, 0, t.active);
         uint* classScratch = t.active >= PT_CLASSIFY_FROM ? reinterpret_cast<uint*>(t.aux.bestKey) : nullptr;
         launch_shade(t.k, pin, t.queue[t.cur], countIn, t.active, t.queue[nxt], &t.wc->extendCount[nxt], t.sq, t.wc, classScratch,
-                     t.aux.counts + PASS_CLASS_OFFSET, t.st, pout);
+                     t.aux.counts + PASS_CLASS_OFFSET, t.st, pout, vertex0 ? &fv : nullptr);
         const size_t e2 = t.mark(); t.span(e1, e2, 1, t.active);
         t.extendRays += t.active;
         PT_CHECK_HIP(c, hipMemcpyAsync(t.hwc, t.wc, 16, hipMemcpyDeviceToHost, t.st));
diff --git a/rtxpt_amd/csrc/pt_path.h b/rtxpt_amd/csrc/pt_path.h
--- a/rtxpt_amd/csrc/pt_path.h
+++ b/rtxpt_amd/csrc/pt_path.h
@@ -190,11 +190,12 @@
         if (S.bounceCount < vertexIndex) return true;
         return diffuseBounces > S.diffuseBounceCount;
     }
-    void computeCameraRay(uint px, uint py, uint sampleIndex, float3& o, float3& d) const {
+    void computeCameraRay(uint px, uint py, uint sampleIndex, float3& o, float3& d) const { cameraRay(cam, S.perPixelJitterAAScale, px, py, sampleIndex, o, d); }
+    static void cameraRay(const PathTracerCameraData& cam, float perPixelJitterAAScale, uint px, uint py, uint sampleIndex, float3& o, float3& d) {
         SampleGeneratorVertexBase vb = SampleGeneratorVertexBase::make((px << 16) | py, 0, sampleIndex);
         SampleSequenceGenerator sg = SampleSequenceGenerator::make(vb);
         float2 r0 = sampleNext2D(sg);
-        float2 subPixelOffset = make_float2(cam.Jitter.x + (r0.x - 0.5f) * S.perPixelJitterAAScale, cam.Jitter.y + (r0.y - 0.5f) * S.perPixelJitterAAScale);
+        float2 subPixelOffset = make_float2(cam.Jitter.x + (r0.x - 0.5f) * perPixelJitterAAScale, cam.Jitter.y + (r0.y - 0.5f) * perPixelJitterAAScale);
         float2 dof = sampleNext2D(sg);
         float2 pp = make_float2(((float)px + 0.5f + -subPixelOffset.x) / (float)cam.ViewportSize.x, ((float)py + 0.5f + subPixelOffset.y) / (float)cam.ViewportSize.y);
         float2 ndc = make_float2(2.f * pp.x + -1.f, -2.f * pp.y + 1.f);
@@ -211,7 +212,7 @@
     void ExportDepth(const PathState& path, float3 virtualWorldPos) const {
         sc.lights.DepthExport[(path.id & 0xFFFFu) * sc.lights.DepthWidth + (path.id >> 16)] = LightTable_ClipDepth(sc.lights, virtualWorldPos);
     }
-    PathState generate(uint px, uint py, uint sampleIndex) const {
+    PathState generateState(uint px, uint py, uint sampleIndex) const {
         PathState p; __builtin_memset(&p, 0, sizeof(p));
         p.id = (px << 16) | py; p.sampleIndex = sampleIndex;
         p.SetThp(make_float3(1.f));
@@ -221,22 +222,11 @@
         p.SetFireflyFilterK_BsdfScatterPdf(1.0f, 0.0f);
         p.SetPackedMISInfo_ThpRuRuCorrection(NEEBSDFMISInfo::empty().Pack16bit(), 1.0f);
         if (HasFinishedSurfaceBounces(p.getVertexIndex() + 1, p.getCounter(PC_DiffuseBounces))) p.setFlag(PF_terminateAtNextBounce);
-        SampleGeneratorVertexBase vb = SampleGeneratorVertexBase::make((px << 16) | py, 0, sampleIndex);
-        SampleSequenceGenerator sg = SampleSequenceGenerator::make(vb);
-        float2 r0 = sampleNext2D(sg);
-        float2 subPixelOffset = make_float2(cam.Jitter.x + (r0.x - 0.5f) * S.perPixelJitterAAScale, cam.Jitter.y + (r0.y - 0.5f) * S.perPixelJitterAAScale);
-        float2 dof = sampleNext2D(sg);
-        float2 pp = make_float2(((float)px + 0.5f + -subPixelOffset.x) / (float)cam.ViewportSize.x, ((float)py + 0.5f + subPixelOffset.y) / (float)cam.ViewportSize.y);
-        float2 ndc = make_float2(2.f * pp.x + -1.f, -2.f * pp.y + 1.f);
-        float3 org = cam.PosW;
-        float3 dir = (ndc.x * cam.CameraU + ndc.y * cam.CameraV) + cam.CameraW;
-        float2 ap = sample_disk(dof);
-        float3 rayTarget = org + dir;
-        org = org + cam.ApertureRadius * (ap.x * normalize(cam.CameraU) + ap.y * normalize(cam.CameraV));
-        dir = normalize(rayTarget - org);
-        float invCos = 1.f / dot(normalize(cam.CameraW), dir);
-        float tMin = cam.NearZ * invCos;
-        p.origin = org + dir * tMin; p.dir = dir;
+        return p;
+    }
+    PathState generate(uint px, uint py, uint sampleIndex) const {
+        PathState p = generateState(px, py, sampleIndex);
+        computeCameraRay(px, py, sampleIndex, p.origin, p.dir);
         return p;
     }
 
diff --git a/rtxpt_amd/csrc/pt_wavefront.h b/rtxpt_amd/csrc/pt_wavefront.h
--- a/rtxpt_amd/csrc/pt_wavefront.h
+++ b/rtxpt_amd/csrc/pt_wavefront.h
@@ -10,12 +10,15 @@
     const uint* home; };
 struct ShadowQueue { float4* q0; float4* q1; float4* q2; uint group;
     float4* q3; float* fbTotalWeight; uint* fbCandidates; uint fbWidth, fbPlane, fbSampleFirst; };
+struct FirstVertex { const uint* ownedPixels; uint numOwned, sampleFirst, spp; };
+struct FirstVertexCamera { PathTracerCameraData cam; float perPixelJitterAAScale, _pad[3]; };
 struct WaveCounters {
     uint extendCount[2]; uint shadowCount; uint overflow;
     unsigned long long hits, nodeVisitsExt, triTestsExt, nodeVisitsSh, triTestsSh, leafVisitsExt, itersExt, leafVisitsSh, itersSh, phaseCycExt[4], leafBlocksExt, eventsExt[8], itersMaxExt, rayIterHistExt[16]; uint longRayCount, _padLong; float longRays[32][8];
     unsigned long long shadowValid;
     unsigned long long tailExtendRays, tailShadowRays;
     unsigned long long tailHandedBack[3];
+    FirstVertexCamera firstCamera;
 };
 
 static const uint TRAV_COUNTERS = 5, TRAV_RESOLVE = 4, PASS_COUNTERS = 16, PASS_SHADOW_OFFSET = 5, PASS_CLASS_OFFSET = 10;
@@ -23,8 +26,10 @@
 
 void launch_generate(const PathKernelContext& k, PathPool pool, const uint* ownedPixels, uint numOwned, uint sampleFirst, uint spp, uint first, uint n, uint* queue, uint* countPtr, hipStream_t st);
 void launch_extend(const DeviceScene& sc, PathPool pool, const uint* queue, const uint* countPtr, uint count, WaveCounters* wc, bool counters, TravAux aux, hipStream_t st, bool ranged = false);
+void launch_extend_first(const PathKernelContext& k, PathPool pool, FirstVertex fv, const uint* countPtr, uint count, WaveCounters* wc, TravAux aux, hipStream_t st);
 void launch_shade(const PathKernelContext& k, PathPool pool, const uint* queueIn, const uint* countInPtr, uint countIn, uint* queueOut, uint* countOutPtr,
-                  ShadowQueue sq, WaveCounters* wc, uint* classScratch, uint* classCount, hipStream_t st, PathPool outPool = PathPool{});
+                  ShadowQueue sq, WaveCounters* wc, uint* classScratch, uint* classCount, hipStream_t st, PathPool outPool = PathPool{},
+                  const FirstVertex* fv = nullptr);
 void launch_uncompact(PathPool in, PathPool out, const uint* countPtr, uint count, hipStream_t st);
 void launch_classify(PathPool pool, const uint* queueIn, const uint* countInPtr, uint countIn, uint* classScratch, uint* classCount, hipStream_t st);
 void launch_shadow(const DeviceScene& sc, PathPool pool, ShadowQueue sq, const uint* countPtr, uint count, WaveCounters* wc, bool counters, TravAux aux, hipStream_t st);
diff --git a/rtxpt_amd/csrc/pt_wavefront.hip b/rtxpt_amd/csrc/pt_wavefront.hip
--- a/rtxpt_amd/csrc/pt_wavefront.hip
+++ b/rtxpt_amd/csrc/pt_wavefront.hip
@@ -7,9 +7,6 @@
 
 namespace ptk {
 
-#ifndef PT_SAMPLE_MINOR
-#define PT_SAMPLE_MINOR 1
-#endif
 #ifndef T8_CHUNKS_PER_WAVE_MIN
 #define T8_CHUNKS_PER_WAVE_MIN 1
 #endif
@@ -24,22 +21,27 @@
     const uint t = blockIdx.x * 256u + threadIdx.x;
     if (t >= n) return;
     const uint i = first + t;
-#if PT_SAMPLE_MINOR
-    uint kpx = i / spp, s = i - kpx * spp, px = ownedPixels[kpx];
-#else
-    uint s = i / numOwned, px = ownedPixels[i - s * numOwned];
-#endif
-    PathState p = k.generate(px >> 16, px & 0xFFFFu, sampleFirst + s);
+    uint px, sample; first_vertex_of(FirstVertex{ownedPixels, numOwned, sampleFirst, spp}, i, px, sample);
+    PathState p = k.generate(px >> 16, px & 0xFFFFu, sample);
     store_path(pool, i, p);
     queue[t] = i;
     if (countPtr && t == 0u) atomicAdd(countPtr, n);
 }
 
-template <bool COUNT, bool RANGED>
+template <bool COUNT, bool RANGED, bool FIRST = false>
 __device__ __forceinline__ void t8_extend_body(const DeviceScene& sc, const PathPool& pool, const uint* __restrict__ queue, const uint count, WaveCounters* wc, const TravAux& aux, const uint rpc,
-                                               uint2* stack, uint* rayBuf, float2* mineUV, const uint vBlock, const uint vGrid) {
+                                               uint2* stack, uint* rayBuf, float2* mineUV, const uint vBlock, const uint vGrid, const FirstVertex* fv = nullptr) {
+    static_assert(!FIRST || (!COUNT && !RANGED), "vertex 0 in place: composed frames only");
     Traverse8Counters ctr; t8_counters_init(ctr);
     auto fetch = [&](uint i, float3& o, float3& d, float& tmin, float& tmax, uint& startRef, float& bestT0, uint& bestPrim0) -> uint {
+        if (FIRST) {
+            asm volatile("" ::: "memory");
+            const FirstVertexCamera fc = wc->firstCamera;
+            uint px, sample; first_vertex_of(*fv, i, px, sample);
+            PathKernelContext::cameraRay(fc.cam, fc.perPixelJitterAAScale, px >> 16, px & 0xFFFFu, sample, o, d);
+            tmin = 0.0f; tmax = kMaxRayTravel; startRef = 0u; bestT0 = kMaxRayTravel; bestPrim0 = 0xFFFFFFFFu;
+            return i;
+        }
         uint p = pool.home ? i : queue[i];
         uint4 a = pool.s0[p], b = pool.s1[p];
         o = make_float3(asfloat(a.x), asfloat(a.y), asfloat(a.z)); d = make_float3(asfloat(b.x), asfloat(b.y), asfloat(b.z));
@@ -61,6 +63,23 @@
     __shared__ uint rayBuf[T8_RAYBUF_WORDS];
     __shared__ float2 mineUV[T8_BLOCK];
     t8_extend_body<COUNT, RANGED>(sc, pool, queue, *countPtr, wc, aux, rpc, stack, rayBuf, mineUV, blockIdx.x, gridDim.x);
+}
+
+__global__ void __launch_bounds__(T8_BLOCK, T8_EXTEND_MIN_BLOCKS) k_extend_first(DeviceScene sc, PathPool pool, FirstVertex fv, const uint* __restrict__ countPtr, WaveCounters* wc, TravAux aux, uint rpc) {
+    __shared__ uint2 stack[T8_GROUPS_PER_BLOCK * BVH8_STACK_STRIDE];
+    __shared__ uint rayBuf[T8_RAYBUF_WORDS];
+    __shared__ float2 mineUV[T8_BLOCK];
+    t8_extend_body<false, false, true>(sc, pool, nullptr, *countPtr, wc, aux, rpc, stack, rayBuf, mineUV, blockIdx.x, gridDim.x, &fv);
+}
+
+__global__ void __launch_bounds__(256) k_first_split_rays(PathKernelContext k, PathPool pool, FirstVertex fv, TravAux aux) {
+    const uint n = aux.counts[TRAV_RESOLVE];
+    for (uint i = blockIdx.x * 256u + threadIdx.x; i < n; i += gridDim.x * 256u) {
+        const uint p = aux.resolveList[i];
+        uint px, sample; first_vertex_of(fv, p, px, sample);
+        float3 o, d; k.computeCameraRay(px >> 16, px & 0xFFFFu, sample, o, d);
+        pool.s0[p] = make_uint4(asuint(o.x), asuint(o.y), asuint(o.z), px); pool.s1[p] = make_uint4(asuint(d.x), asuint(d.y), asuint(d.z), asuint(0.0f));
+    }
 }
 
 #ifndef T8_TASK_SPREAD
@@ -131,7 +150,8 @@
 #endif
 
 #define PT_CLASSIFY_ITEMS 4u
-__global__ void __launch_bounds__(1024) k_classify(PathPool pool, const uint* __restrict__ queueIn, const uint* __restrict__ countInPtr, uint* __restrict__ classQ, uint* __restrict__ classCount) {
+template <bool UNIFORM = false>
+__global__ void __launch_bounds__(1024) k_classify(PathPool pool, const uint* __restrict__ queueIn, const uint* __restrict__ countInPtr, uint* __restrict__ classQ, uint* __restrict__ classCount, uint uniformFlags) {
     __shared__ uint waveCnt[PT_CLASSIFY_ITEMS][16][3]; __shared__ uint blockBase[3];
     const uint count = *countInPtr, wave = threadIdx.x >> 6, lane = threadIdx.x & 63u;
     uint p[PT_CLASSIFY_ITEMS], cls[PT_CLASSIFY_ITEMS]; unsigned long long mine[PT_CLASSIFY_ITEMS];
@@ -141,7 +161,7 @@
         p[j] = 0u; cls[j] = 3u;
         if (i < count) {
             p[j] = pool.home ? i : queueIn[i];
-            const uint prim = reinterpret_cast<const uint*>(pool.hit)[4u * (size_t)p[j] + 1u], flags = reinterpret_cast<const uint*>(pool.s4)[4u * (size_t)p[j] + 2u];
+            const uint prim = reinterpret_cast<const uint*>(pool.hit)[4u * (size_t)p[j] + 1u], flags = UNIFORM ? uniformFlags : reinterpret_cast<const uint*>(pool.s4)[4u * (size_t)p[j] + 2u];
             cls[j] = (prim == 0xFFFFFFFFu) ? 2u : (((flags >> kVertexIndexBitCount) & PF_terminateAtNextBounce) ? 1u : 0u);
         }
         const unsigned long long m0 = __builtin_amdgcn_ballot_w64(cls[j] == 0u), m1 = __builtin_amdgcn_ballot_w64(cls[j] == 1u), m2 = __builtin_amdgcn_ballot_w64(cls[j] == 2u);
@@ -163,9 +183,10 @@
     }
 }
 
-template <bool MULTI, class PKC, bool NEEAT, bool COMPACT = false>
+template <bool MULTI, class PKC, bool NEEAT, bool COMPACT = false, bool FIRST = false>
 __global__ void __launch_bounds__(PT_SHADE_BLOCK, PT_SHADE_MIN_BLOCKS) k_shade(PKC k, PathPool pool, const uint* __restrict__ queueIn, const uint* __restrict__ countInPtr,
-                                               uint* __restrict__ queueOut, uint* countOutPtr, ShadowQueue sq, WaveCounters* wc, const uint* __restrict__ classCount, PathPool outPool) {
+                                               uint* __restrict__ queueOut, uint* countOutPtr, ShadowQueue sq, WaveCounters* wc, const uint* __restrict__ classCount, PathPool outPool, FirstVertex fv) {
+    static_assert(!FIRST || (COMPACT && !MULTI && !NEEAT), "vertex 0 in place: the compacted pool of a composed frame");
     static_assert(!COMPACT || !PT_SHADE_PROBE, "the PT_SHADE_PROBE timing builds do not know the compacted pool: take the COMPACT launch out of launch_shade and run with MI355PT_COMPACT_POOL=0");
     const uint count = *countInPtr;
     uint i = blockIdx.x * (uint)PT_SHADE_BLOCK + threadIdx.x;
@@ -179,7 +200,7 @@
             const uint nGo = classCount[0], nEnd = classCount[1];
             p = queueIn[i < nGo ? i : (i < nGo + nEnd ? count - 1u - (i - nGo) : count + (i - nGo - nEnd))];
         } else p = COMPACT ? i : queueIn[i];
-        hp = COMPACT ? pool.home[p] : p;
+        hp = (COMPACT && !FIRST) ? pool.home[p] : p;
         uint4 hr = pool.hit[p];
         HitInfo h; h.t = asfloat(hr.x); h.prim = hr.y; h.u = asfloat(hr.z); h.v = asfloat(hr.w);
 #if PT_SHADE_PROBE
@@ -192,7 +213,15 @@
         store_path(pool, p, path);
         alive = path.isActive();
 #else
-        if (COMPACT) {
+        if (COMPACT && FIRST) {
+            uint px, sample; first_vertex_of(fv, p, px, sample);
+            const PathFirstVertexIO<PKC> io{k, px, sample};
+            if (h.prim == 0xFFFFFFFFu) { cpath = io.load_all(); k.template HandleMiss<NEEAT>(cpath, cpath.dir, kMaxRayTravel); }
+            else { isHit = true; cpath = io.load_first(); k.template HandleHit<false, NEEAT>(cpath, h, req, nullptr, io); }
+            alive = cpath.isActive();
+            pool.s2[hp] = make_uint4(cpath.pack23[0], cpath.pack23[1], cpath.pack45[0], cpath.pack45[1]);
+        }
+        else if (COMPACT) {
             const PathCompactIO io{pool, p, hp};
             if (h.prim == 0xFFFFFFFFu) { cpath = io.load_all(); k.template HandleMiss<NEEAT>(cpath, cpath.dir, kMaxRayTravel); }
             else { isHit = true; cpath = io.load_first(); k.template HandleHit<false, NEEAT>(cpath, h, req, nullptr, io); }
@@ -684,6 +713,14 @@
 static const uint T8_TASK_BLOCKS = T8_TASK_BLOCKS_N, T8_RESOLVE_BLOCKS = 256;
 static const uint T8_SWEEP_BLOCKS = 2048;
 static inline uint shadow_resolve_grid(uint count) { const uint g = grid_for(count, 256u, T8_SWEEP_BLOCKS); return g < T8_RESOLVE_BLOCKS ? T8_RESOLVE_BLOCKS : g; }
+static void launch_extend_stragglers(const DeviceScene& sc, PathPool pool, uint count, WaveCounters* wc, TravAux aux, hipStream_t st);
+void launch_extend_first(const PathKernelContext& k, PathPool pool, FirstVertex fv, const uint* countPtr, uint count, WaveCounters* wc, TravAux aux, hipStream_t st) {
+    const uint rpc = rays_per_chunk(count);
+    const uint g = grid_for(count, (T8_BLOCK / 64u) * rpc * T8_CHUNKS_PER_WAVE_MIN, (aux.maxBlocks && aux.maxBlocks < T8_MAX_BLOCKS) ? aux.maxBlocks : T8_MAX_BLOCKS);
+    hipLaunchKernelGGL(k_extend_first, dim3(g), dim3(T8_BLOCK), 0, st, k.sc, pool, fv, countPtr, wc, aux, rpc);
+    hipLaunchKernelGGL(k_first_split_rays, dim3(T8_RESOLVE_BLOCKS), dim3(256), 0, st, k, pool, fv, aux);
+    launch_extend_stragglers(k.sc, pool, count, wc, aux, st);
+}
 void launch_extend(const DeviceScene& sc, PathPool pool, const uint* queue, const uint* countPtr, uint count, WaveCounters* wc, bool counters, TravAux aux, hipStream_t st, bool ranged) {
     const uint rpc = rays_per_chunk(count);
     uint g = grid_for(count, (T8_BLOCK / 64u) * rpc * T8_CHUNKS_PER_WAVE_MIN, (aux.maxBlocks && aux.maxBlocks < T8_MAX_BLOCKS) ? aux.maxBlocks : T8_MAX_BLOCKS);
@@ -691,6 +728,9 @@
                   else hipLaunchKernelGGL((k_extend<false, true>), dim3(g), dim3(T8_BLOCK), 0, st, sc, pool, queue, countPtr, wc, aux, rpc); }
     else if (counters) hipLaunchKernelGGL((k_extend<true>), dim3(g), dim3(T8_BLOCK), 0, st, sc, pool, queue, countPtr, wc, aux, rpc);
     else hipLaunchKernelGGL((k_extend<false>), dim3(g), dim3(T8_BLOCK), 0, st, sc, pool, queue, countPtr, wc, aux, rpc);
+    launch_extend_stragglers(sc, pool, count, wc, aux, st);
+}
+static void launch_extend_stragglers(const DeviceScene& sc, PathPool pool, uint count, WaveCounters* wc, TravAux aux, hipStream_t st) {
     if (count <= T8_SHORT_TAIL_BELOW) {
         hipLaunchKernelGGL((k_extend_tasks<0>), dim3(T8_TASK_BLOCKS), dim3(T8_BLOCK), 0, st, sc, pool, wc, aux);
         hipLaunchKernelGGL((k_extend_tasks<1, true>), dim3(T8_TASK_BLOCKS), dim3(T8_BLOCK), 0, st, sc, pool, wc, aux);
@@ -727,19 +767,23 @@
     hipLaunchKernelGGL(k_resolve_pair, dim3(T8_RESOLVE_BLOCKS + shadow_resolve_grid(shCount)), dim3(256), 0, st, sc, pool, sq, auxE, auxS, shCountPtr, shCount, T8_RESOLVE_BLOCKS);
 }
 void launch_classify(PathPool pool, const uint* queueIn, const uint* countInPtr, uint countIn, uint* classScratch, uint* classCount, hipStream_t st) {
-    hipLaunchKernelGGL(k_classify, dim3((countIn + 1024u * PT_CLASSIFY_ITEMS - 1u) / (1024u * PT_CLASSIFY_ITEMS)), dim3(1024), 0, st, pool, queueIn, countInPtr, classScratch, classCount);
+    hipLaunchKernelGGL((k_classify<false>), dim3((countIn + 1024u * PT_CLASSIFY_ITEMS - 1u) / (1024u * PT_CLASSIFY_ITEMS)), dim3(1024), 0, st, pool, queueIn, countInPtr, classScratch, classCount, 0u);
 }
 void launch_shade(const PathKernelContext& k, PathPool pool, const uint* queueIn, const uint* countInPtr, uint countIn, uint* queueOut, uint* countOutPtr, ShadowQueue sq, WaveCounters* wc,
-                  uint* classScratch, uint* classCount, hipStream_t st, PathPool outPool) {
+                  uint* classScratch, uint* classCount, hipStream_t st, PathPool outPool, const FirstVertex* fv) {
+    const FirstVertex fv0 = fv ? *fv : FirstVertex{nullptr, 0u, 0u, 0u};
     const dim3 g((countIn + PT_SHADE_BLOCK - 1) / PT_SHADE_BLOCK), b(PT_SHADE_BLOCK);
     if (PT_SHADE_CLASSES && classScratch) {
-        hipLaunchKernelGGL(k_classify, dim3((countIn + 1024u * PT_CLASSIFY_ITEMS - 1u) / (1024u * PT_CLASSIFY_ITEMS)), dim3(1024), 0, st, pool, queueIn, countInPtr, classScratch, classCount);
+        const dim3 cg((countIn + 1024u * PT_CLASSIFY_ITEMS - 1u) / (1024u * PT_CLASSIFY_ITEMS));
+        if (fv) hipLaunchKernelGGL((k_classify<true>), cg, dim3(1024), 0, st, pool, queueIn, countInPtr, classScratch, classCount, k.generateState(0u, 0u, 0u).flagsAndVertexIndex);
+        else hipLaunchKernelGGL((k_classify<false>), cg, dim3(1024), 0, st, pool, queueIn, countInPtr, classScratch, classCount, 0u);
         queueIn = classScratch;
     } else classCount = nullptr;
     const bool neeat = k.sc.lights.LocalSamplingBuffer != nullptr || k.sc.lights.TemporalFeedbackRequired != 0u;
-#define PT_LAUNCH_SHADE(MULTI, PKC, CTX) do { if (neeat) hipLaunchKernelGGL((k_shade<MULTI, PKC, true>), g, b, 0, st, CTX, pool, queueIn, countInPtr, queueOut, countOutPtr, sq, wc, classCount, outPool); \
-                                              else if (pool.home && !MULTI) hipLaunchKernelGGL((k_shade<false, PKC, false, true>), g, b, 0, st, CTX, pool, queueIn, countInPtr, queueOut, countOutPtr, sq, wc, classCount, outPool); \
-                                              else hipLaunchKernelGGL((k_shade<MULTI, PKC, false>), g, b, 0, st, CTX, pool, queueIn, countInPtr, queueOut, countOutPtr, sq, wc, classCount, outPool); } while (0)
+#define PT_LAUNCH_SHADE(MULTI, PKC, CTX) do { if (neeat) hipLaunchKernelGGL((k_shade<MULTI, PKC, true>), g, b, 0, st, CTX, pool, queueIn, countInPtr, queueOut, countOutPtr, sq, wc, classCount, outPool, fv0); \
+                                              else if (pool.home && !MULTI && fv) hipLaunchKernelGGL((k_shade<false, PKC, false, true, true>), g, b, 0, st, CTX, pool, queueIn, countInPtr, queueOut, countOutPtr, sq, wc, classCount, outPool, fv0); \
+                                              else if (pool.home && !MULTI) hipLaunchKernelGGL((k_shade<false, PKC, false, true>), g, b, 0, st, CTX, pool, queueIn, countInPtr, queueOut, countOutPtr, sq, wc, classCount, outPool, fv0); \
+                                              else hipLaunchKernelGGL((k_shade<MULTI, PKC, false>), g, b, 0, st, CTX, pool, queueIn, countInPtr, queueOut, countOutPtr, sq, wc, classCount, outPool, fv0); } while (0)
     if (k.S.useFp16Types) {
         static_assert(sizeof(PathKernelContextT<true>) == sizeof(PathKernelContext), "the two lp builds share one context layout");
         PathKernelContextT<true> k16; __builtin_memcpy(&k16, &k, sizeof(k16));
diff --git a/rtxpt_amd/csrc/pt_wavefront_device.h b/rtxpt_amd/csrc/pt_wavefront_device.h
--- a/rtxpt_amd/csrc/pt_wavefront_device.h
+++ b/rtxpt_amd/csrc/pt_wavefront_device.h
@@ -18,6 +18,18 @@
 __device__ __forceinline__ void wave_add64(unsigned long long v, unsigned long long* counter) {
     for (int o = 32; o > 0; o >>= 1) v += __shfl_xor(v, o);
     if (lane_id() == 0 && v) atomicAdd(counter, v);
+}
+
+#ifndef PT_SAMPLE_MINOR
+#define PT_SAMPLE_MINOR 1
+#endif
+__device__ __forceinline__ void first_vertex_of(const FirstVertex& fv, uint i, uint& px, uint& sample) {
+#if PT_SAMPLE_MINOR
+    const uint kpx = i / fv.spp, s = i - kpx * fv.spp; px = fv.ownedPixels[kpx];
+#else
+    const uint s = i / fv.numOwned; px = fv.ownedPixels[i - s * fv.numOwned];
+#endif
+    sample = fv.sampleFirst + s;
 }
 
 __device__ __forceinline__ void store_path(const PathPool& pool, uint i, const PathState& p) {
@@ -95,6 +107,28 @@
     __device__ __forceinline__ void store_all(const PathState&) const {}
 };
 
+template <class PKC> struct PathFirstVertexIO {
+    static constexpr bool streams = true;
+    const PKC& k; uint px, sample;
+    __device__ __forceinline__ void mark(int) const {}
+    __device__ __forceinline__ PathState load_first() const {
+        PathState p = k.generateState(px >> 16, px & 0xFFFFu, sample); float3 o;
+        k.computeCameraRay(px >> 16, px & 0xFFFFu, sample, o, p.dir);
+        return p;
+    }
+    __device__ __forceinline__ void load_rest(PathState& p) const {
+        uint q = px, s = sample; asm volatile("" : "+v"(q), "+v"(s) :: "memory");
+        const PathState g = k.generate(q >> 16, q & 0xFFFFu, s);
+        p.origin = g.origin; p.id = g.id;
+        p.pack23[0] = g.pack23[0]; p.pack23[1] = g.pack23[1]; p.pack45[0] = g.pack45[0]; p.pack45[1] = g.pack45[1];
+        p.pack0 = g.pack0; p.pack1 = g.pack1; p.flagsAndVertexIndex = g.flagsAndVertexIndex; p.sampleIndex = g.sampleIndex;
+    }
+    __device__ __forceinline__ PathState load_all() const { return k.generate(px >> 16, px & 0xFFFFu, sample); }
+    __device__ __forceinline__ void store_front(const PathState&) const {}
+    __device__ __forceinline__ void store_back(const PathState&) const {}
+    __device__ __forceinline__ void store_all(const PathState&) const {}
+};
+
 __device__ __forceinline__ void t8_counters_init(Traverse8Counters& ctr) {
     ctr.nodeVisits = 0; ctr.triTests = 0; ctr.leafVisits = 0; ctr.iters = 0; ctr.leafBlocks = 0; for (int q = 0; q < 8; q++) ctr.ev[q] = 0u; ctr.cyc[0] = ctr.cyc[1] = ctr.cyc[2] = ctr.cyc[3] = 0ull;
     ctr.rayIterHist = nullptr; ctr.longRayCount = nullptr; ctr.longRays = nullptr;
```

New measurement: 1883 Mrays/s, median of 6. 1.01x the previous value.
